# Nexenta/edge-fuse

Measured on NVIDIA H100. Metric: GiB/s hash+LZ4+dedup on 64 KiB chunks, higher is better.
Workload: dtype u8

## Files before the change

edge_fuse_b200/csrc/engine.cu:

```cuda
#include <algorithm>
#include <atomic>
#include <deque>
#include <mutex>
#include <set>
#include <shared_mutex>
#include <sched.h>
#include <string>
#include <new>
#include <unordered_set>
#include <stdio.h>
#include <stdlib.h>
#include <string.h>
#include <vector>
#include "../../include/cachemap_b200.h"
#include "../../include/uint128.h"
#include "kernels.h"
#include "common.cuh"
#include "streamgen.cuh"

static thread_local char g_err[512];

void cmb_set_error(const char *what, cudaError_t e, const char *file, int line) {
	snprintf(g_err, sizeof(g_err), "%s:%d: %s: %s", file, line, what, cudaGetErrorString(e));
}
static void set_error_msg(const char *msg) { snprintf(g_err, sizeof(g_err), "%s", msg); }

using namespace cmb;

struct cmb200_engine {
	int device = 0;
	int pshift = 16;
	uint32_t bsize = 65536;
	int accel = 12;
	uint64_t capacity = 0;
	uint32_t max_batch = 4096;
	uint32_t host_batch = 4096;
	uint32_t flags = 0;
	cudaStream_t st = nullptr, copy = nullptr;
	static constexpr int GET_LANES = 32;
	struct GetLane { std::atomic<int> busy{0}; cudaStream_t st = nullptr; int32_t *h_status = nullptr; cmb200_addr *h_addr = nullptr; };
	GetLane lane[GET_LANES];
	struct GetGate {
		std::atomic<int> active{0}, closed{0};
		void enter() {
			for (;;) {
				while (closed.load(std::memory_order_acquire)) sched_yield();
				active.fetch_add(1, std::memory_order_acq_rel);
				if (!closed.load(std::memory_order_acquire)) return;
				active.fetch_sub(1, std::memory_order_acq_rel);
			}
		}
		void leave() { active.fetch_sub(1, std::memory_order_acq_rel); }
		void close() {
			int open = 0;
			while (!closed.compare_exchange_weak(open, 1, std::memory_order_acq_rel)) { open = 0; sched_yield(); }
			while (active.load(std::memory_order_acquire)) sched_yield();
		}
		void reopen() { closed.store(0, std::memory_order_release); }
	} get_gate;
	struct GateClosed {
		GetGate &g;
		explicit GateClosed(GetGate &gate) : g(gate) { g.close(); }
		~GateClosed() { g.reopen(); }
	};
	std::atomic<uint32_t> lane_turn{0};
	static constexpr size_t GET_SMALL_MAX = 1024;
	const uint8_t *peer_base[GET_MAX_PEERS] = {};
	uint64_t peer_size[GET_MAX_PEERS] = {};
	std::atomic<uint64_t> small_get_requests{0}, small_get_hits{0}, small_get_launches{0};
	unsigned long long *d_recoff_out = nullptr;
	uint4 *d_scratch = nullptr;
	uint32_t *d_pool_bits = nullptr;
	uint32_t pool_n = 0, region_entries = 0;
	cudaEvent_t landed[2] = {nullptr, nullptr}, consumed[2] = {nullptr, nullptr};
	TableView table{};
	ArenaView arena{};
	unsigned long long *d_counters = nullptr;
	uint8_t *d_pages[2] = {nullptr, nullptr};
	uint8_t *d_stage = nullptr;
	uint64_t stage_stride = 0;
	unsigned long long *d_addr = nullptr, *d_ts = nullptr;
	uint8_t *d_valid = nullptr;
	uint32_t *d_slot = nullptr, *d_vlen = nullptr;
	int32_t *d_lens = nullptr, *d_status = nullptr;
	uint64_t *d_fps = nullptr, *d_recoff = nullptr;
	unsigned int *d_work = nullptr;
	uint32_t *d_order = nullptr;
	uint32_t *d_import_slot = nullptr;
	size_t import_slot_cap = 0;
	uint32_t *d_move_idx = nullptr;
	size_t move_idx_cap = 0;
	static constexpr size_t META_CAP = 1u << 18;
	uint8_t *h_meta = nullptr;
	unsigned long long seq = 1;
	unsigned long long seq_stride = 1;
	static constexpr int RING = 64;
	cudaEvent_t t0[RING] = {}, t1[RING] = {};
	cudaEvent_t p0[RING] = {}, p1[RING] = {};
	uint64_t pend_head = 0, pend_tail = 0;
	static constexpr int TICKETS = 8;
	cudaEvent_t ticket_ev[TICKETS] = {};
	uint64_t tickets = 0;
	cudaEvent_t meta_done = nullptr, meta_free[2] = {nullptr, nullptr};
	uint64_t ring_pos = 0;
	uint64_t meta_pos = 0;
	size_t meta_cap = 0;
	std::mutex mu;
	cmb200_stats stats{};
	struct HostTier {
		uint8_t *host = nullptr;
		uint8_t *dev = nullptr;
		uint64_t size = 0;
		uint64_t head = 0;
		std::deque<std::pair<uint64_t, uint32_t>> log;
		uint64_t demoted_records = 0, demoted_bytes = 0;
		uint64_t promoted_records = 0, promoted_bytes = 0;
		unsigned long long *d_ctr = nullptr;
		ulonglong2 *d_hot = nullptr;
		uint64_t hot_drained = 0;
		unsigned long long *d_retire = nullptr;
		size_t retire_cap = 0;
		DemoteEntry *d_moves = nullptr;
		PromoteEntry *d_promote = nullptr;
		HotLog hot() const { return HotLog{d_ctr ? d_ctr + 2 : nullptr, d_hot}; }
	} tier;
	std::atomic<bool> multi_gpu{false};
};

#define ENG_CHECK(expr)                                                 \
	do {                                                            \
		cudaError_t e_ = (expr);                                \
		if (e_ != cudaSuccess) {                                \
			cmb_set_error(#expr, e_, __FILE__, __LINE__);   \
			goto fail;                                      \
		}                                                       \
	} while (0)

static uint64_t next_pow2(uint64_t v) {
	uint64_t p = 1;
	while (p < v) p <<= 1;
	return p;
}

extern "C" const char *cmb200_last_error(void) { return g_err; }

extern "C" int cmb200_device_count(void) {
	int n = 0;
	cudaError_t e = cudaGetDeviceCount(&n);
	if (e != cudaSuccess) { cmb_set_error("cudaGetDeviceCount", e, __FILE__, __LINE__); return 0; }
	return n;
}

static int select_device(int device) {
	if (device >= 0) CMB_CHECK(cudaSetDevice(device));
	int n = 0;
	CMB_CHECK(cudaGetDeviceCount(&n));
	if (n == 0) { set_error_msg("no CUDA device"); return -1; }
	return 0;
}

extern "C" void cmb200_engine_destroy(cmb200_engine *e) {
	if (!e) return;
	cudaSetDevice(e->device);
	if (e->st) cudaStreamSynchronize(e->st);
	if (e->copy) cudaStreamSynchronize(e->copy);
	cudaFree(e->d_scratch); cudaFree(e->d_pool_bits); cudaFree(e->table.ckpt);
	cudaFree(e->table.slots); cudaFree(e->table.fp); cudaFree(e->arena.base); cudaFree(e->arena.seg); cudaFree(e->d_counters);
	cudaFree(e->d_pages[0]); cudaFree(e->d_pages[1]); cudaFree(e->d_stage);
	cudaFree(e->d_addr); cudaFree(e->d_ts); cudaFree(e->d_valid); cudaFree(e->d_slot); cudaFree(e->d_vlen);
	cudaFree(e->d_move_idx);
	if (e->h_meta) cudaFreeHost(e->h_meta);
	for (auto &ln : e->lane) {
		if (ln.st) { cudaStreamSynchronize(ln.st); cudaStreamDestroy(ln.st); }
		if (ln.h_status) cudaFreeHost(ln.h_status);
		if (ln.h_addr) cudaFreeHost(ln.h_addr);
	}
	cudaFree(e->d_recoff_out);
	for (int r = 0; r < GET_MAX_PEERS; r++) if (e->peer_base[r]) cudaIpcCloseMemHandle((void *)e->peer_base[r]);
	if (e->tier.host) cudaFreeHost(e->tier.host);
	cudaFree(e->tier.d_ctr); cudaFree(e->tier.d_retire); cudaFree(e->tier.d_moves);
	cudaFree(e->tier.d_promote); cudaFree(e->tier.d_hot);
	cudaFree(e->d_lens); cudaFree(e->d_status); cudaFree(e->d_fps); cudaFree(e->d_recoff); cudaFree(e->d_work); cudaFree(e->d_order); cudaFree(e->d_import_slot);
	for (int i = 0; i < 2; i++) {
		if (e->landed[i]) cudaEventDestroy(e->landed[i]);
		if (e->consumed[i]) cudaEventDestroy(e->consumed[i]);
	}
	for (int i = 0; i < cmb200_engine::RING; i++) {
		if (e->t0[i]) cudaEventDestroy(e->t0[i]);
		if (e->t1[i]) cudaEventDestroy(e->t1[i]);
		if (e->p0[i]) cudaEventDestroy(e->p0[i]);
		if (e->p1[i]) cudaEventDestroy(e->p1[i]);
	}
	for (int i = 0; i < cmb200_engine::TICKETS; i++) if (e->ticket_ev[i]) cudaEventDestroy(e->ticket_ev[i]);
	if (e->meta_done) cudaEventDestroy(e->meta_done);
	for (int i = 0; i < 2; i++) if (e->meta_free[i]) cudaEventDestroy(e->meta_free[i]);
	if (e->st) cudaStreamDestroy(e->st);
	if (e->copy) cudaStreamDestroy(e->copy);
	delete e;
}

extern "C" cmb200_engine *cmb200_engine_create(const cmb200_config *cfg) {
	if (!cfg || cfg->pshift < 6 || cfg->pshift > 20) { set_error_msg("bad config: pshift must be 6..20"); return nullptr; }
	if (select_device(cfg->device) != 0) return nullptr;
	cmb200_engine *e = new (std::nothrow) cmb200_engine();
	if (!e) return nullptr;
	cudaGetDevice(&e->device);
	e->pshift = cfg->pshift;
	e->bsize = 1u << cfg->pshift;
	e->accel = cfg->accel < 0 ? 1 : (cfg->accel > (1 << 20) ? (1 << 20) : cfg->accel);
	e->capacity = cfg->capacity;
	e->max_batch = cfg->max_batch ? cfg->max_batch : 4096;
	e->host_batch = e->max_batch < 4096u ? e->max_batch : 4096u;
	e->flags = cfg->flags;
	const uint64_t B = e->max_batch;
	{
		uint64_t slots = cfg->table_slots ? next_pow2(cfg->table_slots) : next_pow2(4 * (cfg->capacity ? cfg->capacity : 1024));
		if (slots < 1024) slots = 1024;
		if (slots > (1ull << 27)) slots = 1ull << 27;
		e->table.cap = slots;
		ENG_CHECK(cudaStreamCreateWithFlags(&e->st, cudaStreamNonBlocking));
		ENG_CHECK(cudaStreamCreateWithFlags(&e->copy, cudaStreamNonBlocking));
		for (auto &ln : e->lane) ENG_CHECK(cudaStreamCreateWithFlags(&ln.st, cudaStreamNonBlocking));
		for (int i = 0; i < 2; i++) {
			ENG_CHECK(cudaEventCreateWithFlags(&e->landed[i], cudaEventDisableTiming));
			ENG_CHECK(cudaEventCreateWithFlags(&e->consumed[i], cudaEventDisableTiming));
		}
		for (int i = 0; i < cmb200_engine::RING; i++) {
			ENG_CHECK(cudaEventCreate(&e->t0[i]));
			ENG_CHECK(cudaEventCreate(&e->t1[i]));
			ENG_CHECK(cudaEventCreate(&e->p0[i]));
			ENG_CHECK(cudaEventCreate(&e->p1[i]));
		}
		for (int i = 0; i < cmb200_engine::TICKETS; i++)
			ENG_CHECK(cudaEventCreateWithFlags(&e->ticket_ev[i], cudaEventDisableTiming));
		ENG_CHECK(cudaEventCreateWithFlags(&e->meta_done, cudaEventDisableTiming));
		ENG_CHECK(cudaEventCreateWithFlags(&e->meta_free[0], cudaEventDisableTiming));
		ENG_CHECK(cudaEventCreateWithFlags(&e->meta_free[1], cudaEventDisableTiming));
		ENG_CHECK(cudaMalloc(&e->table.slots, (slots + 2) * sizeof(Slot)));
		ENG_CHECK(cudaMemsetAsync(e->table.slots, 0, (slots + 2) * sizeof(Slot), e->st));
		if (e->flags & CMB200_FINGERPRINT) {
			ENG_CHECK(cudaMalloc(&e->table.fp, (slots + 2) * 16));
			ENG_CHECK(cudaMemsetAsync(e->table.fp, 0, (slots + 2) * 16, e->st));
		}
		if (get_small_supports(e->bsize)) {
			const char *ck = getenv("CMB200_CKPT");
			if (!ck || atoi(ck) != 0) {
				ENG_CHECK(cudaMalloc(&e->table.ckpt, (slots + 2) * CKPT_WORDS * 4));
				ENG_CHECK(cudaMemsetAsync(e->table.ckpt, 0, (slots + 2) * CKPT_WORDS * 4, e->st));
			}
			const int resident = get_small_residency(e->bsize);
			if (resident <= 0) { set_error_msg("k_get_small does not fit this device"); goto fail; }
			e->pool_n = (uint32_t)resident;
			e->region_entries = get_small_region_entries(e->bsize);
			ENG_CHECK(cudaMalloc(&e->d_scratch, (size_t)e->pool_n * e->region_entries * sizeof(uint4)));
			ENG_CHECK(cudaMalloc(&e->d_pool_bits, ((size_t)e->pool_n + 31) / 32 * 4));
			ENG_CHECK(cudaMemsetAsync(e->d_pool_bits, 0, ((size_t)e->pool_n + 31) / 32 * 4, e->st));
		}
		ENG_CHECK(cudaMalloc(&e->d_counters, 8 * sizeof(unsigned long long)));
		ENG_CHECK(cudaMemsetAsync(e->d_counters, 0, 8 * sizeof(unsigned long long), e->st));
		e->table.entries = e->d_counters + 0;
		e->table.tombs = e->d_counters + 1;
		e->arena.head = e->d_counters + 2;
		e->arena.garbage = e->d_counters + 3;
		e->arena.dropped = e->d_counters + 4;
		e->table.remote = e->d_counters + 5;
		e->arena.tier = e->d_counters + 6;

		{
			const uint64_t bound = (uint64_t)e->bsize + e->bsize / 255 + 16;
			const uint64_t row = (uint64_t)e->bsize + 1024 > bound ? (uint64_t)e->bsize + 1024 : bound;
			e->stage_stride = (row + 15) & ~15ull;
		}
		ENG_CHECK(cudaMalloc(&e->d_pages[0], (uint64_t)e->host_batch * e->bsize + 256));
		ENG_CHECK(cudaMalloc(&e->d_pages[1], (uint64_t)e->host_batch * e->bsize + 256));
		ENG_CHECK(cudaMalloc(&e->d_stage, (uint64_t)16384 * e->stage_stride + 256));
		const uint64_t M = cmb200_engine::META_CAP > B ? cmb200_engine::META_CAP : B;
		e->meta_cap = M;
		ENG_CHECK(cudaMalloc(&e->d_addr, 2 * M * 16));
		ENG_CHECK(cudaMalloc(&e->d_ts, 2 * M * 8));
		ENG_CHECK(cudaMalloc(&e->d_valid, 2 * M));
		ENG_CHECK(cudaMalloc(&e->d_slot, B * 4));
		ENG_CHECK(cudaMalloc(&e->d_vlen, B * 4));
		ENG_CHECK(cudaMalloc(&e->d_lens, M * 4));
		ENG_CHECK(cudaMalloc(&e->d_status, M * 4));
		ENG_CHECK(cudaMalloc(&e->d_fps, B * 16));
		ENG_CHECK(cudaMalloc(&e->d_recoff, B * 8));
		ENG_CHECK(cudaMalloc(&e->d_work, 64));
		ENG_CHECK(cudaMalloc(&e->d_order, encode_order_words((uint32_t)B) * 4));
		ENG_CHECK(cudaMallocHost(&e->h_meta, cmb200_engine::META_CAP * 33));
		for (auto &ln : e->lane) {
			ENG_CHECK(cudaMallocHost(&ln.h_status, cmb200_engine::GET_SMALL_MAX * 4));
			ENG_CHECK(cudaMallocHost(&ln.h_addr, cmb200_engine::GET_SMALL_MAX * 16));
		}
		ENG_CHECK(cudaMalloc(&e->d_recoff_out, M * 8));

		uint64_t arena = cfg->arena_bytes;
		if (!arena) {
			size_t free_b = 0, total_b = 0;
			ENG_CHECK(cudaMemGetInfo(&free_b, &total_b));
			uint64_t want = (cfg->capacity ? cfg->capacity : 1024) * (e->stage_stride + 32);
			want += want / 8;
			uint64_t lim = (uint64_t)(free_b * 0.8);
			arena = want < lim ? want : lim;
		}
		arena = (arena + 255) & ~255ull;
		ENG_CHECK(cudaMalloc(&e->arena.base, arena + 256));
		e->arena.size = arena;
		{
			const uint64_t worst = (24 + e->stage_stride + 15) & ~15ull;
			uint64_t seg = arena / (8ull * 2072ull);
			if (seg > (2ull << 20)) seg = 2ull << 20;
			if (seg < 4 * worst) seg = 0;
			const char *kb = getenv("CMB200_SEG_KB");
			if (kb && *kb) { seg = strtoull(kb, nullptr, 10) << 10; if (seg && seg < worst) seg = worst; }
			seg = (seg + 255) & ~255ull;
			e->arena.seg_bytes = (uint32_t)seg;
			ENG_CHECK(cudaMalloc(&e->arena.seg, ARENA_SEG_SLOTS * 2 * sizeof(unsigned long long)));
			ENG_CHECK(cudaMemsetAsync(e->arena.seg, 0, ARENA_SEG_SLOTS * 2 * sizeof(unsigned long long), e->st));
		}
		ENG_CHECK(cudaStreamSynchronize(e->st));
	}
	return e;
fail:
	cmb200_engine_destroy(e);
	return nullptr;
}

extern "C" void *cmb200_host_alloc(size_t bytes) {
	void *p = nullptr;
	cudaError_t er = cudaMallocHost(&p, bytes);
	if (er != cudaSuccess) { cmb_set_error("cudaMallocHost", er, __FILE__, __LINE__); return nullptr; }
	return p;
}
extern "C" void cmb200_host_free(void *p) { if (p) cudaFreeHost(p); }
extern "C" void *cmb200_dev_alloc(cmb200_engine *e, size_t bytes) {
	void *p = nullptr;
	if (e) cudaSetDevice(e->device);
	cudaError_t er = cudaMalloc(&p, bytes + 256);
	if (er != cudaSuccess) { cmb_set_error("cudaMalloc", er, __FILE__, __LINE__); return nullptr; }
	return p;
}
extern "C" void cmb200_dev_free(cmb200_engine *e, void *p) { if (e) cudaSetDevice(e->device); if (p) cudaFree(p); }
extern "C" int cmb200_memcpy_h2d(cmb200_engine *e, void *dev, const void *host, size_t bytes) {
	cudaSetDevice(e->device);
	CMB_CHECK(cudaMemcpyAsync(dev, host, bytes, cudaMemcpyHostToDevice, e->st));
	CMB_CHECK(cudaStreamSynchronize(e->st));
	return 0;
}
extern "C" int cmb200_memcpy_d2h(cmb200_engine *e, void *host, const void *dev, size_t bytes) {
	cudaSetDevice(e->device);
	CMB_CHECK(cudaMemcpyAsync(host, dev, bytes, cudaMemcpyDeviceToHost, e->st));
	CMB_CHECK(cudaStreamSynchronize(e->st));
	return 0;
}
extern "C" void *cmb200_stream(cmb200_engine *e) { return (void *)e->st; }
extern "C" int cmb200_sync(cmb200_engine *e) {
	cudaSetDevice(e->device);
	CMB_CHECK(cudaStreamSynchronize(e->copy));
	CMB_CHECK(cudaStreamSynchronize(e->st));
	return 0;
}


static void harvest_pending(cmb200_engine *e, bool wait) {
	while (e->pend_tail < e->pend_head) {
		const int k = (int)(e->pend_tail % cmb200_engine::RING);
		if (wait) cudaEventSynchronize(e->p1[k]);
		else if (cudaEventQuery(e->p1[k]) != cudaSuccess) { (void)cudaGetLastError(); break; }
		float ms = 0;
		if (cudaEventElapsedTime(&ms, e->p0[k], e->p1[k]) == cudaSuccess) {
			e->stats.encode_kernel_ns += (uint64_t)(ms * 1e6);
			e->stats.encode_kernel_launches++;
		}
		e->pend_tail++;
	}
}

struct StepRecords { uint32_t rank; unsigned long long *out; bool keep_pages; };

static int put_slice(cmb200_engine *e, size_t n, const cmb200_addr *addr, const uint8_t *valid,
    const uint8_t *pages, bool pages_on_dev, const uint64_t *ts, int32_t *lens_out, uint64_t *ticket,
    const StepRecords *recs = nullptr) {
	const size_t B = pages_on_dev ? e->max_batch : e->host_batch;
	const bool deferred = ticket != nullptr;
	const bool copy_meta = !pages_on_dev || deferred;
	const unsigned long long seq_first = e->seq;
	cmb200_addr *h_addr = (cmb200_addr *)e->h_meta;
	uint64_t *h_ts = (uint64_t *)(e->h_meta + cmb200_engine::META_CAP * 16);
	int32_t *h_lens = (int32_t *)(e->h_meta + cmb200_engine::META_CAP * 24);
	uint8_t *h_valid = e->h_meta + cmb200_engine::META_CAP * 32;
	harvest_pending(e, !deferred);
	memcpy(h_addr, addr, n * 16);
	if (ts) memcpy(h_ts, ts, n * 8);
	if (valid) memcpy(h_valid, valid, n);
	const int mb = copy_meta ? (int)(e->meta_pos++ & 1) : 0;
	unsigned long long *d_addr = e->d_addr + (size_t)mb * e->meta_cap * 2;
	unsigned long long *d_ts = e->d_ts + (size_t)mb * e->meta_cap;
	uint8_t *d_valid = e->d_valid + (size_t)mb * e->meta_cap;
	cudaStream_t ms = copy_meta ? e->copy : e->st;
	if (copy_meta) CMB_CHECK(cudaStreamWaitEvent(e->copy, e->meta_free[mb], 0));
	CMB_CHECK(cudaMemcpyAsync(d_addr, h_addr, n * 16, cudaMemcpyHostToDevice, ms));
	if (valid) CMB_CHECK(cudaMemcpyAsync(d_valid, h_valid, n, cudaMemcpyHostToDevice, ms));
	if (ts) CMB_CHECK(cudaMemcpyAsync(d_ts, h_ts, n * 8, cudaMemcpyHostToDevice, ms));
	if (copy_meta) {
		CMB_CHECK(cudaEventRecord(e->meta_done, e->copy));
		CMB_CHECK(cudaStreamWaitEvent(e->st, e->meta_done, 0));
	}
	size_t nb = 0;
	int last_buf = 0;
	for (size_t at = 0; at < n; at += B, nb++) {
		const uint32_t m = (uint32_t)((n - at < B) ? n - at : B);
		const int buf = (int)(e->ring_pos & 1);
		const uint8_t *d_in;
		if (pages_on_dev) {
			d_in = pages + at * e->bsize;
		} else {
			e->ring_pos++;
			last_buf = buf;
			CMB_CHECK(cudaStreamWaitEvent(e->copy, e->consumed[buf], 0));
			CMB_CHECK(cudaMemcpyAsync(e->d_pages[buf], pages + at * e->bsize, (size_t)m * e->bsize,
			    cudaMemcpyHostToDevice, e->copy));
			CMB_CHECK(cudaEventRecord(e->landed[buf], e->copy));
			CMB_CHECK(cudaStreamWaitEvent(e->st, e->landed[buf], 0));
			d_in = e->d_pages[buf];
		}
		if (launch_upsert(e->table, d_addr + 2 * at, valid ? d_valid + at : nullptr, m, e->seq, e->seq_stride, e->d_slot, e->st)) return -1;
		EncodeJob job{};
		job.pages = d_in; job.page_stride = e->bsize; job.nbytes = e->bsize; job.n = m;
		job.accel = (uint32_t)e->accel;
		job.stage = e->d_stage; job.stage_stride = e->stage_stride;
		job.lens = e->d_lens + at;
		job.rec_out = e->d_recoff_out + at;
		job.fps = (e->flags & CMB200_FINGERPRINT) ? e->d_fps : nullptr;
		job.work = e->d_work;
		job.order = e->d_order;
		job.slot_idx = e->d_slot;
		job.addr = d_addr + 2 * at;
		job.ts = ts ? d_ts + at : nullptr;
		job.seq0 = e->seq; job.seq_stride = e->seq_stride;
		job.table = e->table; job.arena = e->arena;
		cudaEvent_t ev0, ev1;
		if (deferred) {
			if (e->pend_head - e->pend_tail >= (uint64_t)cmb200_engine::RING) harvest_pending(e, true);
			ev0 = e->p0[e->pend_head % cmb200_engine::RING]; ev1 = e->p1[e->pend_head % cmb200_engine::RING];
			e->pend_head++;
		} else {
			ev0 = e->t0[nb % e->RING]; ev1 = e->t1[nb % e->RING];
		}
		CMB_CHECK(cudaEventRecord(ev0, e->st));
		const int encode_kernels = launch_encode(job, e->st);
		if (encode_kernels < 0) return -1;
		CMB_CHECK(cudaEventRecord(ev1, e->st));
		if (!pages_on_dev) CMB_CHECK(cudaEventRecord(e->consumed[buf], e->st));
		e->seq += (unsigned long long)m * e->seq_stride;
		e->stats.kernel_launches += 1 + encode_kernels;
	}
	e->stats.put_chunks += n;
	if (recs && recs->out) {
		if (launch_pack_records(d_addr, e->d_lens, e->d_recoff_out, (uint32_t)n, seq_first, e->seq_stride, recs->rank, recs->out, e->st)) return -1;
		e->stats.kernel_launches++;
	}
	if (copy_meta) CMB_CHECK(cudaEventRecord(e->meta_free[mb], e->st));
	if (deferred) {
		if (lens_out) CMB_CHECK(cudaMemcpyAsync(lens_out, e->d_lens, n * 4, cudaMemcpyDeviceToHost, e->st));
		CMB_CHECK(cudaEventRecord(e->ticket_ev[e->tickets % cmb200_engine::TICKETS], e->st));
		*ticket = ++e->tickets;
		CMB_CHECK(cudaEventSynchronize(e->meta_done));
		if (nb && !pages_on_dev && !(recs && recs->keep_pages)) CMB_CHECK(cudaEventSynchronize(e->landed[last_buf]));
		harvest_pending(e, false);
		return 0;
	}
	if (lens_out) CMB_CHECK(cudaMemcpyAsync(h_lens, e->d_lens, n * 4, cudaMemcpyDeviceToHost, e->st));
	CMB_CHECK(cudaStreamSynchronize(e->st));
	if (lens_out) memcpy(lens_out, h_lens, n * 4);
	for (size_t k = 0; k < nb && k < (size_t)e->RING; k++) {
		float ms = 0;
		CMB_CHECK(cudaEventElapsedTime(&ms, e->t0[k], e->t1[k]));
		e->stats.encode_kernel_ns += (uint64_t)(ms * 1e6);
		e->stats.encode_kernel_launches++;
	}
	return 0;
}

static int check_dev_pages(const void *pages, const char *what) {
	if (reinterpret_cast<uintptr_t>(pages) & 15u) {
		snprintf(g_err, sizeof(g_err), "%s: device pages must be 16-byte aligned", what);
		return -1;
	}
	return 0;
}

static int multi_gpu_call(cmb200_engine *e, const char *what) {
	if (e->tier.host) {
		snprintf(g_err, sizeof(g_err), "%s: not available on an engine with a host tier", what);
		return -1;
	}
	e->multi_gpu = true;
	return 0;
}

static int put_impl(cmb200_engine *e, size_t n, const cmb200_addr *addr, const uint8_t *valid,
    const uint8_t *pages, bool pages_on_dev, const uint64_t *ts, int32_t *lens_out, uint64_t *ticket) {
	std::lock_guard<std::mutex> g(e->mu);
	CMB_CHECK(cudaSetDevice(e->device));
	if (ticket) *ticket = e->tickets;
	for (size_t at = 0; at < n; at += cmb200_engine::META_CAP) {
		size_t m = n - at < cmb200_engine::META_CAP ? n - at : cmb200_engine::META_CAP;
		const bool last = at + m == n;
		if (put_slice(e, m, addr + at, valid ? valid + at : nullptr, pages + at * e->bsize, pages_on_dev,
			ts ? ts + at : nullptr, lens_out ? lens_out + at : nullptr, last ? ticket : nullptr)) return -1;
	}
	return 0;
}

extern "C" int cmb200_put_batch(cmb200_engine *e, size_t n, const cmb200_addr *addr, const uint8_t *valid,
    const void *pages_host, const uint64_t *ts, int32_t *lens_out) {
	return put_impl(e, n, addr, valid, (const uint8_t *)pages_host, false, ts, lens_out, nullptr);
}
extern "C" int cmb200_put_batch_async(cmb200_engine *e, size_t n, const cmb200_addr *addr, const uint8_t *valid,
    const void *pages_host, const uint64_t *ts, int32_t *lens_out, uint64_t *ticket) {
	uint64_t t = 0;
	const int rc = put_impl(e, n, addr, valid, (const uint8_t *)pages_host, false, ts, lens_out, &t);
	if (ticket) *ticket = t;
	return rc;
}
extern "C" int cmb200_put_step(cmb200_engine *e, size_t n, const cmb200_addr *addr, const uint8_t *valid,
    const void *pages, int pages_on_dev, const uint64_t *ts, uint32_t rank, void *records_dev_out,
    int32_t *lens_out, uint64_t *ticket) {
	if (multi_gpu_call(e, "cmb200_put_step")) return -1;
	if (n > cmb200_engine::META_CAP) { set_error_msg("cmb200_put_step: more than 262144 chunks in one step"); return -1; }
	if (pages_on_dev == 1 && check_dev_pages(pages, "cmb200_put_step")) return -1;
	std::lock_guard<std::mutex> g(e->mu);
	CMB_CHECK(cudaSetDevice(e->device));
	uint64_t t = e->tickets;
	StepRecords r{rank, (unsigned long long *)records_dev_out, pages_on_dev == 2};
	const int rc = n ? put_slice(e, n, addr, valid, (const uint8_t *)pages, pages_on_dev == 1, ts, lens_out, &t, &r) : 0;
	if (ticket) *ticket = t;
	return rc;
}

extern "C" int cmb200_import_records_dev(cmb200_engine *e, size_t n_total, const void *records_dev, uint32_t my_rank) {
	std::lock_guard<std::mutex> g(e->mu);
	if (multi_gpu_call(e, "cmb200_import_records_dev")) return -1;
	CMB_CHECK(cudaSetDevice(e->device));
	if (n_total == 0) return 0;
	if (n_total > 0xffffffffull) { set_error_msg("cmb200_import_records_dev: too many records"); return -1; }
	if (n_total > e->import_slot_cap) {
		CMB_CHECK(cudaStreamSynchronize(e->st));
		if (e->d_import_slot) cudaFree(e->d_import_slot);
		e->d_import_slot = nullptr; e->import_slot_cap = 0;
		CMB_CHECK(cudaMalloc(&e->d_import_slot, n_total * sizeof(uint32_t)));
		e->import_slot_cap = n_total;
	}
	if (launch_import_records(e->table, e->arena, (const unsigned long long *)records_dev, (uint32_t)n_total, my_rank,
		e->d_import_slot, e->st)) return -1;
	e->stats.kernel_launches += 2;
	return 0;
}

extern "C" int cmb200_wait(cmb200_engine *e, uint64_t ticket) {
	cudaEvent_t ev = nullptr;
	{
		std::lock_guard<std::mutex> g(e->mu);
		if (ticket == 0 || ticket > e->tickets) return 0;
		ev = e->ticket_ev[(ticket - 1) % cmb200_engine::TICKETS];
		if (cudaSetDevice(e->device) != cudaSuccess) return -1;
	}
	CMB_CHECK(cudaEventSynchronize(ev));
	return 0;
}
extern "C" int cmb200_put_batch_dev(cmb200_engine *e, size_t n, const cmb200_addr *addr, const uint8_t *valid,
    const void *pages_dev, const uint64_t *ts, int32_t *lens_out) {
	if (check_dev_pages(pages_dev, "cmb200_put_batch_dev")) return -1;
	return put_impl(e, n, addr, valid, (const uint8_t *)pages_dev, true, ts, lens_out, nullptr);
}


static int get_slice(cmb200_engine *e, size_t n, const cmb200_addr *addr, const uint8_t *valid,
    uint8_t *pages_out, bool out_on_dev, int32_t *status_out) {
	const size_t B = out_on_dev ? e->max_batch : e->host_batch;
	cmb200_addr *h_addr = (cmb200_addr *)e->h_meta;
	int32_t *h_status = (int32_t *)(e->h_meta + cmb200_engine::META_CAP * 28);
	uint8_t *h_valid = e->h_meta + cmb200_engine::META_CAP * 32;
	memcpy(h_addr, addr, n * 16);
	if (valid) memcpy(h_valid, valid, n);
	CMB_CHECK(cudaMemcpyAsync(e->d_addr, h_addr, n * 16, cudaMemcpyHostToDevice, e->st));
	if (valid) CMB_CHECK(cudaMemcpyAsync(e->d_valid, h_valid, n, cudaMemcpyHostToDevice, e->st));
	size_t nb = 0;
	for (size_t at = 0; at < n; at += B, nb++) {
		const uint32_t m = (uint32_t)((n - at < B) ? n - at : B);
		const int buf = (int)(nb & 1);
		uint8_t *d_out = out_on_dev ? pages_out + at * e->bsize : e->d_pages[buf];
		if (!out_on_dev) CMB_CHECK(cudaStreamWaitEvent(e->st, e->consumed[buf], 0));
		if (launch_lookup(e->table, e->d_addr + 2 * at, valid ? e->d_valid + at : nullptr, m, e->d_status + at, e->d_recoff,
			e->d_vlen, nullptr, e->st)) return -1;
		DecodeJob job{};
		job.n = m; job.nbytes = e->bsize; job.pages = d_out; job.status = e->d_status + at;
		job.rec_off = e->d_recoff; job.vlen = e->d_vlen; job.arena = e->arena.base;
		job.host = e->tier.dev; job.host_hits = e->tier.d_ctr + 1;
		job.hot = e->tier.hot(); job.addr = e->d_addr + 2 * at;
		CMB_CHECK(cudaEventRecord(e->t0[nb % e->RING], e->st));
		if (launch_decode(job, e->st)) return -1;
		CMB_CHECK(cudaEventRecord(e->t1[nb % e->RING], e->st));
		if (!out_on_dev) {
			CMB_CHECK(cudaEventRecord(e->landed[buf], e->st));
			CMB_CHECK(cudaStreamWaitEvent(e->copy, e->landed[buf], 0));
			CMB_CHECK(cudaMemcpyAsync(pages_out + at * e->bsize, d_out, (size_t)m * e->bsize,
			    cudaMemcpyDeviceToHost, e->copy));
			CMB_CHECK(cudaEventRecord(e->consumed[buf], e->copy));
		}
		e->stats.kernel_launches += 2;
	}
	CMB_CHECK(cudaMemcpyAsync(h_status, e->d_status, n * 4, cudaMemcpyDeviceToHost, e->st));
	CMB_CHECK(cudaStreamSynchronize(e->st));
	CMB_CHECK(cudaStreamSynchronize(e->copy));
	memcpy(status_out, h_status, n * 4);
	for (size_t k = 0; k < nb && k < (size_t)e->RING; k++) {
		float ms = 0;
		CMB_CHECK(cudaEventElapsedTime(&ms, e->t0[k], e->t1[k]));
		e->stats.decode_kernel_ns += (uint64_t)(ms * 1e6);
		e->stats.decode_kernel_launches++;
	}
	for (size_t i = 0; i < n; i++) {
		if (status_out[i] != CMB200_INVALID) e->stats.get_requests++;
		if (status_out[i] == CMB200_HIT) e->stats.get_hits++;
	}
	return 0;
}

static int get_impl(cmb200_engine *e, size_t n, const cmb200_addr *addr, const uint8_t *valid,
    uint8_t *pages_out, bool out_on_dev, int32_t *status_out) {
	std::lock_guard<std::mutex> g(e->mu);
	CMB_CHECK(cudaSetDevice(e->device));
	for (size_t at = 0; at < n; at += cmb200_engine::META_CAP) {
		size_t m = n - at < cmb200_engine::META_CAP ? n - at : cmb200_engine::META_CAP;
		if (get_slice(e, m, addr + at, valid ? valid + at : nullptr, pages_out + at * e->bsize, out_on_dev,
			status_out + at)) return -1;
	}
	return 0;
}

extern "C" int cmb200_get_batch(cmb200_engine *e, size_t n, const cmb200_addr *addr, const uint8_t *valid,
    void *pages_out_host, int32_t *status_out) {
	return get_impl(e, n, addr, valid, (uint8_t *)pages_out_host, false, status_out);
}
static int lookup_chunk(cmb200_engine *e, const cmb200_addr *addr, uint32_t m, int32_t *status, uint64_t *loc,
    uint32_t *vlen) {
	CMB_CHECK(cudaMemcpyAsync(e->d_addr, addr, (size_t)m * 16, cudaMemcpyHostToDevice, e->st));
	if (launch_lookup(e->table, e->d_addr, nullptr, m, e->d_status, e->d_recoff, e->d_vlen, nullptr, e->st)) return -1;
	CMB_CHECK(cudaMemcpyAsync(status, e->d_status, (size_t)m * 4, cudaMemcpyDeviceToHost, e->st));
	CMB_CHECK(cudaMemcpyAsync(loc, e->d_recoff, (size_t)m * 8, cudaMemcpyDeviceToHost, e->st));
	if (vlen) CMB_CHECK(cudaMemcpyAsync(vlen, e->d_vlen, (size_t)m * 4, cudaMemcpyDeviceToHost, e->st));
	CMB_CHECK(cudaStreamSynchronize(e->st));
	return 0;
}

extern "C" int cmb200_locate_batch(cmb200_engine *e, size_t n, const cmb200_addr *addr, int32_t *status_out,
    uint64_t *owner_out) {
	std::lock_guard<std::mutex> g(e->mu);
	CMB_CHECK(cudaSetDevice(e->device));
	for (size_t at = 0; at < n; at += e->max_batch) {
		uint32_t m = (uint32_t)((n - at < e->max_batch) ? n - at : e->max_batch);
		if (lookup_chunk(e, addr + at, m, status_out + at, owner_out + at, nullptr)) return -1;
		e->stats.kernel_launches++;
	}
	return 0;
}
extern "C" int cmb200_get_batch_dev(cmb200_engine *e, size_t n, const cmb200_addr *addr, const uint8_t *valid,
    void *pages_out_dev, int32_t *status_out) {
	return get_impl(e, n, addr, valid, (uint8_t *)pages_out_dev, true, status_out);
}


extern "C" int cmb200_set_stream_order(cmb200_engine *e, uint64_t next_seq, uint64_t stride) {
	std::lock_guard<std::mutex> g(e->mu);
	if (multi_gpu_call(e, "cmb200_set_stream_order")) return -1;
	if (stride == 0) { set_error_msg("stream order: stride must be >= 1"); return -1; }
	e->seq = next_seq; e->seq_stride = stride;
	return 0;
}


static const int32_t SMALL_PENDING = -1;

extern "C" int cmb200_get_small_begin(cmb200_engine *e, size_t n, const cmb200_addr *addr, void *pages_out, cmb200_small_ticket *t) {
	if (!t) return -1;
	t->lane = -1; t->n = 0; t->status = nullptr;
	if (n == 0) return 0;
	if (n > cmb200_engine::GET_SMALL_MAX) { set_error_msg("cmb200_get_small_begin: more than 1024 requests"); return -1; }
	if (!get_small_supports(e->bsize)) { set_error_msg("cmb200_get_small: page size not supported by the fused kernel"); return -2; }
	e->get_gate.enter();
	cmb200_engine::GetLane *ln = nullptr;
	int li = -1;
	const uint32_t first = e->lane_turn.fetch_add(1, std::memory_order_relaxed);
	for (uint64_t spins = 0; !ln; spins++) {
		for (int k = 0; k < cmb200_engine::GET_LANES && !ln; k++) {
			const int c = (int)((first + k) % cmb200_engine::GET_LANES);
			int idle = 0;
			if (e->lane[c].busy.compare_exchange_strong(idle, 1, std::memory_order_acq_rel)) { ln = &e->lane[c]; li = c; }
		}
		if (!ln) sched_yield();
	}
	if (cudaSetDevice(e->device) != cudaSuccess) { ln->busy.store(0, std::memory_order_release); e->get_gate.leave(); return -1; }
	memcpy(ln->h_addr, addr, n * 16);
	volatile int32_t *hs = ln->h_status;
	for (size_t i = 0; i < n; i++) hs[i] = SMALL_PENDING;
	GetJob job{};
	job.table = e->table; job.arena = e->arena.base; job.arena_size = e->arena.size;
	job.host = e->tier.dev; job.host_size = e->tier.size; job.host_hits = e->tier.d_ctr + 1;
	job.addr = (const unsigned long long *)ln->h_addr; job.valid = nullptr; job.n = (uint32_t)n; job.nbytes = e->bsize;
	job.out = (uint8_t *)pages_out;
	job.status = ln->h_status;
	for (int r = 0; r < GET_MAX_PEERS; r++) { job.peer[r] = e->peer_base[r]; job.peer_size[r] = e->peer_size[r]; }
	job.scratch = e->d_scratch; job.region_entries = e->region_entries; job.pool_bits = e->d_pool_bits; job.pool_n = e->pool_n;
	job.hot = e->tier.hot();
	if (launch_get_small(job, e->device, ln->st)) { ln->busy.store(0, std::memory_order_release); e->get_gate.leave(); return -1; }
	t->lane = li; t->n = (uint32_t)n; t->status = ln->h_status;
	return 0;
}

extern "C" int cmb200_get_small_end(cmb200_engine *e, cmb200_small_ticket *t, int32_t *status_out) {
	if (!t || t->lane < 0) return 0;
	cmb200_engine::GetLane *ln = &e->lane[t->lane];
	volatile int32_t *hs = ln->h_status;
	int rc = 0;
	uint32_t done = 0;
	for (uint64_t spins = 0; done < t->n;) {
		if (hs[done] != SMALL_PENDING) { done++; continue; }
#if defined(__x86_64__)
		__builtin_ia32_pause();
#endif
		if (++spins > 20000) {
			if (cudaSetDevice(e->device) != cudaSuccess || cudaStreamSynchronize(ln->st) != cudaSuccess) {
				cmb_set_error("cudaStreamSynchronize(small get)", cudaGetLastError(), __FILE__, __LINE__);
				rc = -1; break;
			}
			spins = 0;
			if (hs[done] == SMALL_PENDING) { set_error_msg("cmb200_get_small: kernel finished without an answer"); rc = -1; break; }
		}
	}
	__atomic_thread_fence(__ATOMIC_ACQUIRE);
	if (rc == 0) {
		uint64_t rq = 0, ht = 0;
		for (uint32_t i = 0; i < t->n; i++) {
			const int32_t st = hs[i];
			if (status_out) status_out[i] = st;
			if (st != CMB200_INVALID) rq++;
			if (st == CMB200_HIT) ht++;
		}
		e->small_get_launches++;
		e->small_get_requests += rq; e->small_get_hits += ht;
	}
	t->lane = -1;
	ln->busy.store(0, std::memory_order_release);
	e->get_gate.leave();
	return rc;
}

extern "C" int cmb200_get_small(cmb200_engine *e, size_t n, const cmb200_addr *addr, void *pages_out, int32_t *status_out) {
	for (size_t at = 0; at < n; at += cmb200_engine::GET_SMALL_MAX) {
		const size_t m = n - at < cmb200_engine::GET_SMALL_MAX ? n - at : cmb200_engine::GET_SMALL_MAX;
		cmb200_small_ticket t;
		const int rc = cmb200_get_small_begin(e, m, addr + at, (uint8_t *)pages_out + at * e->bsize, &t);
		if (rc) return rc;
		if (cmb200_get_small_end(e, &t, status_out + at)) return -1;
	}
	return 0;
}


extern "C" int cmb200_close_peers(cmb200_engine *e) {
	cmb200_engine::GateClosed g(e->get_gate);
	CMB_CHECK(cudaSetDevice(e->device));
	for (int r = 0; r < GET_MAX_PEERS; r++) {
		if (e->peer_base[r]) cudaIpcCloseMemHandle((void *)e->peer_base[r]);
		e->peer_base[r] = nullptr; e->peer_size[r] = 0;
	}
	return 0;
}

extern "C" int cmb200_arena_ipc_handle(cmb200_engine *e, void *handle64, uint64_t *arena_bytes_out) {
	{
		std::lock_guard<std::mutex> g(e->mu);
		if (multi_gpu_call(e, "cmb200_arena_ipc_handle")) return -1;
	}
	CMB_CHECK(cudaSetDevice(e->device));
	cudaIpcMemHandle_t h;
	static_assert(sizeof(h) == 64, "cudaIpcMemHandle_t is 64 bytes");
	CMB_CHECK(cudaIpcGetMemHandle(&h, e->arena.base));
	memcpy(handle64, &h, 64);
	if (arena_bytes_out) *arena_bytes_out = e->arena.size;
	return 0;
}

extern "C" int cmb200_open_peer(cmb200_engine *e, uint32_t rank, const void *handle64, uint64_t arena_bytes) {
	{
		std::lock_guard<std::mutex> g(e->mu);
		if (multi_gpu_call(e, "cmb200_open_peer")) return -1;
	}
	if (rank >= GET_MAX_PEERS) { set_error_msg("cmb200_open_peer: rank out of range"); return -1; }
	cmb200_engine::GateClosed g(e->get_gate);
	CMB_CHECK(cudaSetDevice(e->device));
	cudaIpcMemHandle_t h;
	memcpy(&h, handle64, 64);
	void *p = nullptr;
	CMB_CHECK(cudaIpcOpenMemHandle(&p, h, cudaIpcMemLazyEnablePeerAccess));
	if (e->peer_base[rank]) cudaIpcCloseMemHandle((void *)e->peer_base[rank]);
	e->peer_base[rank] = (const uint8_t *)p;
	e->peer_size[rank] = arena_bytes;
	return 0;
}


extern "C" int cmb200_unset_batch(cmb200_engine *e, size_t n, const cmb200_addr *addr) {
	std::lock_guard<std::mutex> g(e->mu);
	CMB_CHECK(cudaSetDevice(e->device));
	for (size_t at = 0; at < n; at += e->max_batch) {
		uint32_t m = (uint32_t)((n - at < e->max_batch) ? n - at : e->max_batch);
		CMB_CHECK(cudaMemcpyAsync(e->d_addr, addr + at, (size_t)m * 16, cudaMemcpyHostToDevice, e->st));
		if (launch_unset(e->table, e->arena, e->d_addr, m, e->st)) return -1;
		e->stats.kernel_launches++;
	}
	CMB_CHECK(cudaStreamSynchronize(e->st));
	return 0;
}

static int read_counters(cmb200_engine *e, unsigned long long out[8]) {
	CMB_CHECK(cudaSetDevice(e->device));
	CMB_CHECK(cudaMemcpyAsync(out, e->d_counters, 8 * sizeof(unsigned long long), cudaMemcpyDeviceToHost, e->st));
	CMB_CHECK(cudaStreamSynchronize(e->st));
	return 0;
}

extern "C" uint64_t cmb200_entries(cmb200_engine *e) {
	std::lock_guard<std::mutex> g(e->mu);
	unsigned long long c[8];
	if (read_counters(e, c)) return 0;
	return c[0];
}

extern "C" int cmb200_get_stats(cmb200_engine *e, cmb200_stats *out) {
	std::lock_guard<std::mutex> g(e->mu);
	unsigned long long c[8];
	if (read_counters(e, c)) return -1;
	harvest_pending(e, true);
	*out = e->stats;
	out->get_requests += e->small_get_requests.load(); out->get_hits += e->small_get_hits.load();
	out->kernel_launches += e->small_get_launches.load();
	out->entries = c[0]; out->tombstones = c[1];
	out->arena_used = c[2] < e->arena.size ? c[2] : e->arena.size;
	out->arena_garbage = c[3];
	out->dropped_puts = c[4]; out->remote_entries = c[5];
	out->table_slots = e->table.cap; out->arena_bytes = e->arena.size;
	return 0;
}

extern "C" int cmb200_sample(cmb200_engine *e, size_t n, const uint64_t *r, cmb200_addr *addr_out,
    uint64_t *ts_out, int32_t *ok_out) {
	std::lock_guard<std::mutex> g(e->mu);
	CMB_CHECK(cudaSetDevice(e->device));
	for (size_t at = 0; at < n; at += e->max_batch) {
		const uint32_t m = (uint32_t)((n - at < e->max_batch) ? n - at : e->max_batch);
		CMB_CHECK(cudaMemcpyAsync(e->d_recoff, r + at, (size_t)m * 8, cudaMemcpyHostToDevice, e->st));
		if (launch_sample(e->table, (const unsigned long long *)e->d_recoff, m, e->d_addr, e->d_ts, e->d_status, e->st)) return -1;
		CMB_CHECK(cudaMemcpyAsync(addr_out + at, e->d_addr, (size_t)m * 16, cudaMemcpyDeviceToHost, e->st));
		CMB_CHECK(cudaMemcpyAsync(ts_out + at, e->d_ts, (size_t)m * 8, cudaMemcpyDeviceToHost, e->st));
		CMB_CHECK(cudaMemcpyAsync(ok_out + at, e->d_status, (size_t)m * 4, cudaMemcpyDeviceToHost, e->st));
		CMB_CHECK(cudaStreamSynchronize(e->st));
		e->stats.kernel_launches++;
	}
	return 0;
}

extern "C" int cmb200_read_records(cmb200_engine *e, size_t n, const cmb200_addr *addr, void *out_host,
    size_t stride, int32_t *len_out) {
	std::lock_guard<std::mutex> g(e->mu);
	CMB_CHECK(cudaSetDevice(e->device));
	std::vector<int32_t> st(e->max_batch);
	std::vector<uint64_t> off(e->max_batch);
	std::vector<uint32_t> vl(e->max_batch);
	for (size_t at = 0; at < n; at += e->max_batch) {
		uint32_t m = (uint32_t)((n - at < e->max_batch) ? n - at : e->max_batch);
		if (lookup_chunk(e, addr + at, m, st.data(), off.data(), vl.data())) return -1;
		for (uint32_t i = 0; i < m; i++) {
			if (st[i] != ST_HIT) { len_out[at + i] = -1; continue; }
			uint32_t clen = vl[i] - 1;
			size_t total = 24 + (clen ? clen : e->bsize);
			if (total > stride) { set_error_msg("cmb200_read_records: stride too small"); return -1; }
			if (off[i] & REC_HOST) memcpy((uint8_t *)out_host + (at + i) * stride, e->tier.host + (off[i] & ~REC_HOST), total);
			else CMB_CHECK(cudaMemcpyAsync((uint8_t *)out_host + (at + i) * stride, e->arena.base + off[i], total,
			    cudaMemcpyDeviceToHost, e->st));
			len_out[at + i] = (int32_t)total;
		}
		CMB_CHECK(cudaStreamSynchronize(e->st));
	}
	return 0;
}

extern "C" int cmb200_read_fingerprints(cmb200_engine *e, size_t n, const cmb200_addr *addr, uint64_t *fp_out,
    int32_t *ok_out) {
	std::lock_guard<std::mutex> g(e->mu);
	CMB_CHECK(cudaSetDevice(e->device));
	if (!e->table.fp) { set_error_msg("engine created without CMB200_FINGERPRINT"); return -1; }
	for (size_t at = 0; at < n; at += e->max_batch) {
		uint32_t m = (uint32_t)((n - at < e->max_batch) ? n - at : e->max_batch);
		CMB_CHECK(cudaMemcpyAsync(e->d_addr, addr + at, (size_t)m * 16, cudaMemcpyHostToDevice, e->st));
		if (launch_read_fp(e->table, e->d_addr, m, e->d_fps, e->d_status, e->st)) return -1;
		CMB_CHECK(cudaMemcpyAsync(fp_out + 2 * at, e->d_fps, (size_t)m * 16, cudaMemcpyDeviceToHost, e->st));
		CMB_CHECK(cudaMemcpyAsync(ok_out + at, e->d_status, (size_t)m * 4, cudaMemcpyDeviceToHost, e->st));
		CMB_CHECK(cudaStreamSynchronize(e->st));
	}
	return 0;
}

struct DevBuf {
	void *p = nullptr;
	~DevBuf() { if (p) cudaFree(p); }
	int alloc(size_t bytes) { CMB_CHECK(cudaMalloc(&p, bytes + 256)); return 0; }
	template <class T> T *as() { return (T *)p; }
};

extern "C" int cmb200_read_checkpoints(cmb200_engine *e, size_t n, const cmb200_addr *addr, uint32_t *words_out,
    int32_t *ok_out) {
	std::lock_guard<std::mutex> g(e->mu);
	CMB_CHECK(cudaSetDevice(e->device));
	if (!e->table.ckpt) {
		memset(words_out, 0, n * CKPT_WORDS * 4);
		for (size_t i = 0; i < n; i++) ok_out[i] = -1;
		return 0;
	}
	DevBuf d_words;
	if (n && d_words.alloc((size_t)e->max_batch * CKPT_WORDS * 4)) return -1;
	for (size_t at = 0; at < n; at += e->max_batch) {
		uint32_t m = (uint32_t)((n - at < e->max_batch) ? n - at : e->max_batch);
		CMB_CHECK(cudaMemcpyAsync(e->d_addr, addr + at, (size_t)m * 16, cudaMemcpyHostToDevice, e->st));
		if (launch_read_ckpt(e->table, e->d_addr, m, d_words.as<uint32_t>(), e->d_status, e->st)) return -1;
		CMB_CHECK(cudaMemcpyAsync(words_out + at * CKPT_WORDS, d_words.p, (size_t)m * CKPT_WORDS * 4, cudaMemcpyDeviceToHost, e->st));
		CMB_CHECK(cudaMemcpyAsync(ok_out + at, e->d_status, (size_t)m * 4, cudaMemcpyDeviceToHost, e->st));
		CMB_CHECK(cudaStreamSynchronize(e->st));
	}
	return 0;
}

static int live_records(cmb200_engine *e, bool arena_only, std::vector<ExportEntry> &list, unsigned long long c[8]) {
	if (read_counters(e, c)) return -1;
	const unsigned long long cap_out = c[0] + 16;
	DevBuf d_list, d_count;
	if (d_list.alloc(cap_out * sizeof(ExportEntry)) || d_count.alloc(8)) return -1;
	CMB_CHECK(cudaMemsetAsync(d_count.p, 0, 8, e->st));
	if (launch_export_list(e->table, e->bsize, d_list.as<ExportEntry>(), d_count.as<unsigned long long>(), cap_out,
		arena_only, e->st)) return -1;
	unsigned long long count = 0;
	CMB_CHECK(cudaMemcpyAsync(&count, d_count.p, 8, cudaMemcpyDeviceToHost, e->st));
	CMB_CHECK(cudaStreamSynchronize(e->st));
	const int over = count > cap_out;
	if (over) count = cap_out;
	list.resize(count);
	if (count) CMB_CHECK(cudaMemcpy(list.data(), d_list.p, count * sizeof(ExportEntry), cudaMemcpyDeviceToHost));
	std::sort(list.begin(), list.end(), [](const ExportEntry &a, const ExportEntry &b) { return a.rec_off < b.rec_off; });
	return over;
}

struct SnapHeader {
	char magic[8];
	uint32_t version, pshift;
	uint64_t records, bytes;
	uint32_t flags, pad[7];
};
static_assert(sizeof(SnapHeader) == 64, "snapshot header");
struct SnapRecord { uint64_t ts, fp_hi, fp_lo; uint32_t len, zero; };
static_assert(sizeof(SnapRecord) == 32, "snapshot record header");
static const size_t SNAP_WINDOW = 64u << 20;

static int save_engine(cmb200_engine *e, FILE *f, uint8_t *win, uint64_t *records, uint64_t *bytes) {
	unsigned long long c[8];
	std::vector<ExportEntry> list;
	if (live_records(e, false, list, c) < 0) return -1;
	*records += list.size();
	for (const ExportEntry &x : list) *bytes += x.len;

	bool ok = true;
	static const uint8_t zeros[16] = {0};
	size_t k = 0;
	while (ok && k < list.size()) {
		if (list[k].rec_off & REC_HOST) {
			const ExportEntry &x = list[k++];
			SnapRecord r{x.ts, x.fp_hi, x.fp_lo, x.len, 0};
			const size_t padn = (16 - (x.len & 15)) & 15;
			ok = fwrite(&r, sizeof(r), 1, f) == 1 && fwrite(e->tier.host + (x.rec_off & ~REC_HOST), x.len, 1, f) == 1 &&
			    (padn == 0 || fwrite(zeros, padn, 1, f) == 1);
			continue;
		}
		const unsigned long long w0 = list[k].rec_off;
		unsigned long long w1 = w0 + SNAP_WINDOW;
		if (w1 > e->arena.size + 256) w1 = e->arena.size + 256;
		if (cudaMemcpyAsync(win, e->arena.base + w0, (size_t)(w1 - w0), cudaMemcpyDeviceToHost, e->st) != cudaSuccess ||
		    cudaStreamSynchronize(e->st) != cudaSuccess) { ok = false; break; }
		for (; k < list.size() && list[k].rec_off + list[k].len <= w1; k++) {
			const ExportEntry &x = list[k];
			SnapRecord r{x.ts, x.fp_hi, x.fp_lo, x.len, 0};
			const size_t padn = (16 - (x.len & 15)) & 15;
			ok = ok && fwrite(&r, sizeof(r), 1, f) == 1 && fwrite(win + (x.rec_off - w0), x.len, 1, f) == 1 &&
			    (padn == 0 || fwrite(zeros, padn, 1, f) == 1);
		}
	}
	return ok ? 0 : -2;
}

extern "C" int cmb200_save_set(cmb200_engine *const *engines, int g, const char *path, uint64_t *records_out) {
	if (g < 1 || !engines) { set_error_msg("cmb200_save_set: no engines"); return -1; }
	for (int i = 1; i < g; i++)
		if (engines[i]->pshift != engines[0]->pshift) { set_error_msg("cmb200_save_set: engines of different page sizes"); return -1; }
	std::string tmp = std::string(path) + ".tmp";
	FILE *f = fopen(tmp.c_str(), "wb");
	if (!f) { set_error_msg("cmb200_save: cannot create the snapshot file"); return -1; }
	uint8_t *win = nullptr;
	if (cudaMallocHost(&win, SNAP_WINDOW) != cudaSuccess) { fclose(f); remove(tmp.c_str()); set_error_msg("cmb200_save: no page-locked window"); return -1; }
	SnapHeader h{};
	memcpy(h.magic, "CMB200S1", 8);
	h.version = 1; h.pshift = (uint32_t)engines[0]->pshift; h.flags = engines[0]->table.fp ? 1u : 0u;
	bool ok = fwrite(&h, sizeof(h), 1, f) == 1;
	int rc = 0;
	for (int i = 0; i < g && ok && rc == 0; i++) {
		std::lock_guard<std::mutex> lk(engines[i]->mu);
		rc = save_engine(engines[i], f, win, &h.records, &h.bytes);
	}
	cudaFreeHost(win);
	ok = ok && rc != -2 && fseek(f, 0, SEEK_SET) == 0 && fwrite(&h, sizeof(h), 1, f) == 1;
	ok = ok && fflush(f) == 0;
	ok = (fclose(f) == 0) && ok;
	if (rc == -1 || !ok || rename(tmp.c_str(), path) != 0) {
		remove(tmp.c_str());
		if (rc != -1) set_error_msg("cmb200_save: write failed");
		return -1;
	}
	if (records_out) *records_out = h.records;
	return 0;
}

extern "C" int cmb200_save(cmb200_engine *e, const char *path, uint64_t *records_out) {
	return cmb200_save_set(&e, 1, path, records_out);
}

static int demote_arena_all(cmb200_engine *e);

struct LoadBatch {
	cmb200_engine *e = nullptr;
	uint8_t *blob = nullptr;
	size_t cap = 0, B = 0, used = 0, m = 0;
	std::vector<unsigned long long> off, ts, fps;
	std::vector<cmb200_addr> addr;
	unsigned long long *d_off = nullptr;
	uint64_t *d_fp = nullptr;
	int setup(cmb200_engine *eng) {
		e = eng;
		CMB_CHECK(cudaSetDevice(e->device));
		cap = (size_t)e->host_batch * e->bsize;
		B = e->max_batch < cmb200_engine::META_CAP ? e->max_batch : cmb200_engine::META_CAP;
		off.resize(B); ts.resize(B); fps.resize(2 * B); addr.resize(B);
		CMB_CHECK(cudaMallocHost(&blob, cap));
		CMB_CHECK(cudaMalloc(&d_off, B * 8));
		CMB_CHECK(cudaMalloc(&d_fp, B * 16));
		return 0;
	}
	void release() {
		if (!e) return;
		cudaSetDevice(e->device);
		if (blob) cudaFreeHost(blob);
		if (d_off) cudaFree(d_off);
		if (d_fp) cudaFree(d_fp);
	}
};

static long long load_flush(LoadBatch &b, bool with_fp) {
	if (b.m == 0) return 0;
	cmb200_engine *e = b.e;
	std::lock_guard<std::mutex> g(e->mu);
	CMB_CHECK(cudaSetDevice(e->device));
	const size_t m = b.m;
	if (e->tier.host) {
		unsigned long long c[8];
		if (read_counters(e, c)) return -1;
		if (c[2] + b.used > e->arena.size && demote_arena_all(e)) return -1;
	}
	CMB_CHECK(cudaMemcpyAsync(e->d_pages[0], b.blob, b.used, cudaMemcpyHostToDevice, e->st));
	CMB_CHECK(cudaMemcpyAsync(e->d_addr, b.addr.data(), m * 16, cudaMemcpyHostToDevice, e->st));
	CMB_CHECK(cudaMemcpyAsync(e->d_ts, b.ts.data(), m * 8, cudaMemcpyHostToDevice, e->st));
	CMB_CHECK(cudaMemcpyAsync(b.d_off, b.off.data(), m * 8, cudaMemcpyHostToDevice, e->st));
	CMB_CHECK(cudaMemcpyAsync(b.d_fp, b.fps.data(), m * 16, cudaMemcpyHostToDevice, e->st));
	if (launch_upsert(e->table, e->d_addr, nullptr, (uint32_t)m, e->seq, e->seq_stride, e->d_slot, e->st)) return -1;
	EncodeJob job{};
	job.n = (uint32_t)m; job.nbytes = e->bsize;
	job.slot_idx = e->d_slot; job.addr = e->d_addr; job.ts = e->d_ts;
	job.seq0 = e->seq; job.seq_stride = e->seq_stride;
	job.table = e->table; job.arena = e->arena;
	if (launch_restore(job, e->d_pages[0], b.d_off, with_fp ? b.d_fp : nullptr, e->bsize, e->st)) return -1;
	CMB_CHECK(cudaStreamSynchronize(e->st));
	e->seq += (unsigned long long)m * e->seq_stride;
	e->stats.kernel_launches += 2;
	b.m = 0; b.used = 0;
	return (long long)m;
}

extern "C" int cmb200_load_set(cmb200_engine *const *engines, int g, const char *path, uint64_t *records_out) {
	if (records_out) *records_out = 0;
	if (g < 1 || !engines) { set_error_msg("cmb200_load_set: no engines"); return -1; }
	FILE *f = fopen(path, "rb");
	if (!f) { set_error_msg("cmb200_load: no snapshot file"); return -1; }
	SnapHeader h{};
	if (fread(&h, sizeof(h), 1, f) != 1 || memcmp(h.magic, "CMB200S1", 8) != 0 || h.version != 1) {
		fclose(f); set_error_msg("cmb200_load: not a snapshot of this library"); return -1;
	}
	for (int i = 0; i < g; i++)
		if ((int)h.pshift != engines[i]->pshift) { fclose(f); set_error_msg("cmb200_load: snapshot has another page size"); return -1; }
	const uint32_t bsize = engines[0]->bsize;
	std::vector<LoadBatch> bs(g);
	int rc = 0;
	for (int i = 0; i < g && rc == 0; i++)
		if (bs[i].setup(engines[i])) { rc = -1; set_error_msg("cmb200_load: no staging buffers"); }
	uint64_t done = 0, loaded = 0;
	while (rc == 0 && done < h.records) {
		SnapRecord r;
		cmb200_addr a;
		if (fread(&r, sizeof(r), 1, f) != 1 || r.len < 24 || r.len > 24u + bsize + 1024u || fread(&a, 16, 1, f) != 1) {
			rc = -1; set_error_msg("cmb200_load: truncated or corrupt snapshot"); break;
		}
		uint64_t key;
		FNV_hash(&a, 16, &key);
		LoadBatch &b = bs[cmb200_owner(key, g)];
		const size_t padded = ((size_t)r.len + 15) & ~(size_t)15;
		if (padded > b.cap) { rc = -1; set_error_msg("cmb200_load: record larger than the staging buffer"); break; }
		if (b.m == b.B || b.used + padded > b.cap) {
			const long long got = load_flush(b, h.flags & 1u);
			if (got < 0) { rc = -1; break; }
			loaded += (uint64_t)got;
		}
		uint8_t *rec = b.blob + b.used;
		memcpy(rec, &a, 16);
		if (fread(rec + 16, padded - 16, 1, f) != 1) { rc = -1; set_error_msg("cmb200_load: truncated or corrupt snapshot"); break; }
		{
			int32_t clen;
			memcpy(&clen, rec + 16, 4);
			if (clen < 0 || (uint32_t)clen > bsize + 1024u || r.len != 24u + (clen ? (uint32_t)clen : bsize)) {
				rc = -1; set_error_msg("cmb200_load: truncated or corrupt snapshot"); break;
			}
		}
		b.addr[b.m] = a;
		b.off[b.m] = b.used; b.ts[b.m] = r.ts; b.fps[2 * b.m] = r.fp_hi; b.fps[2 * b.m + 1] = r.fp_lo;
		b.used += padded; b.m++;
		done++;
	}
	for (int i = 0; i < g && rc == 0; i++) {
		const long long got = load_flush(bs[i], h.flags & 1u);
		if (got < 0) rc = -1;
		else loaded += (uint64_t)got;
	}
	for (LoadBatch &b : bs) b.release();
	fclose(f);
	if (records_out) *records_out = loaded;
	return rc;
}

extern "C" int cmb200_load(cmb200_engine *e, const char *path, uint64_t *records_out) {
	return cmb200_load_set(&e, 1, path, records_out);
}


extern "C" int cmb200_move_pages(cmb200_engine *e, size_t n, void *dst_dev, const uint32_t *dst_idx, const void *src_dev,
    const uint32_t *src_idx) {
	if (n == 0) return 0;
	if (check_dev_pages(dst_dev, "cmb200_move_pages") || check_dev_pages(src_dev, "cmb200_move_pages")) return -1;
	if (n > 0xffffffffu) { set_error_msg("cmb200_move_pages: too many pages"); return -1; }
	std::lock_guard<std::mutex> g(e->mu);
	CMB_CHECK(cudaSetDevice(e->device));
	if ((dst_idx || src_idx) && n > e->move_idx_cap) {
		CMB_CHECK(cudaStreamSynchronize(e->st));
		cudaFree(e->d_move_idx);
		e->d_move_idx = nullptr;
		e->move_idx_cap = 0;
		CMB_CHECK(cudaMalloc(&e->d_move_idx, n * 8));
		e->move_idx_cap = n;
	}
	uint32_t *d_dst_idx = dst_idx ? e->d_move_idx : nullptr;
	uint32_t *d_src_idx = src_idx ? e->d_move_idx + e->move_idx_cap : nullptr;
	if (dst_idx) CMB_CHECK(cudaMemcpyAsync(d_dst_idx, dst_idx, n * 4, cudaMemcpyHostToDevice, e->st));
	if (src_idx) CMB_CHECK(cudaMemcpyAsync(d_src_idx, src_idx, n * 4, cudaMemcpyHostToDevice, e->st));
	if (launch_move_pages(dst_dev, d_dst_idx, src_dev, d_src_idx, (uint32_t)n, e->bsize, e->st)) return -1;
	e->stats.kernel_launches++;
	CMB_CHECK(cudaStreamSynchronize(e->st));
	return 0;
}

extern "C" int cmb200_copy_peer(cmb200_engine *dst_e, void *dst_dev, cmb200_engine *src_e, const void *src_dev, size_t bytes) {
	if (bytes == 0) return 0;
	std::lock_guard<std::mutex> g(src_e->mu);
	CMB_CHECK(cudaSetDevice(src_e->device));
	CMB_CHECK(cudaMemcpyPeerAsync(dst_dev, dst_e->device, src_dev, src_e->device, bytes, src_e->st));
	CMB_CHECK(cudaStreamSynchronize(src_e->st));
	return 0;
}

static int compact_locked(cmb200_engine *e, uint64_t *reclaimed_out) {
	cmb200_engine::GateClosed gg(e->get_gate);
	harvest_pending(e, true);
	unsigned long long c[8];
	std::vector<ExportEntry> list;
	const int listed = live_records(e, true, list, c);
	if (listed < 0) return -1;
	if (listed > 0) { set_error_msg("cmb200_compact: the store changed under the compaction"); return -1; }
	const unsigned long long head_before = c[2];
	const size_t count = list.size();
	DevBuf d_moves;
	std::vector<MoveEntry> moves(count);
	unsigned long long at = 0;
	for (size_t i = 0; i < count; i++) {
		moves[i] = MoveEntry{list[i].rec_off, at, list[i].len, list[i].slot};
		at += ((unsigned long long)list[i].len + 15ull) & ~15ull;
	}
	if (count && d_moves.alloc(count * sizeof(MoveEntry))) return -1;
	if (count) CMB_CHECK(cudaMemcpyAsync(d_moves.p, moves.data(), count * sizeof(MoveEntry), cudaMemcpyHostToDevice, e->st));
	const unsigned long long bounce_cap = (unsigned long long)e->host_batch * e->bsize;
	size_t k = 0;
	while (k < count) {
		size_t j = k;
		while (j < count && moves[j].new_off + (((unsigned long long)moves[j].len + 15ull) & ~15ull) - moves[k].new_off <= bounce_cap) j++;
		if (j == k) { set_error_msg("cmb200_compact: record larger than the bounce buffer"); return -1; }
		if (launch_compact_window(e->table, e->arena, d_moves.as<MoveEntry>() + k, (uint32_t)(j - k), e->d_pages[0], e->st)) return -1;
		e->stats.kernel_launches += 2;
		k = j;
	}
	unsigned long long fresh[2] = {at, 0};
	CMB_CHECK(cudaMemcpyAsync(e->d_counters + 2, fresh, 16, cudaMemcpyHostToDevice, e->st));
	CMB_CHECK(cudaMemsetAsync(e->arena.seg, 0, ARENA_SEG_SLOTS * 2 * sizeof(unsigned long long), e->st));
	CMB_CHECK(cudaStreamSynchronize(e->st));
	if (reclaimed_out) *reclaimed_out = head_before > at ? head_before - at : 0;
	if (c[1] > e->table.cap / 8) {
		TableView fresh = e->table;
		fresh.slots = nullptr; fresh.fp = nullptr; fresh.ckpt = nullptr;
		if (cudaMalloc(&fresh.slots, (e->table.cap + 2) * sizeof(Slot)) == cudaSuccess &&
		    (!e->table.fp || cudaMalloc(&fresh.fp, (e->table.cap + 2) * 16) == cudaSuccess)) {
			CMB_CHECK(cudaMemsetAsync(fresh.slots, 0, (e->table.cap + 2) * sizeof(Slot), e->st));
			if (fresh.fp) CMB_CHECK(cudaMemsetAsync(fresh.fp, 0, (e->table.cap + 2) * 16, e->st));
			const size_t ck_bytes = (e->table.cap + 2) * CKPT_WORDS * 4;
			if (e->table.ckpt && cudaMalloc(&fresh.ckpt, ck_bytes) != cudaSuccess) {
				(void)cudaGetLastError();
				fresh.ckpt = nullptr;
			}
			if (fresh.ckpt) CMB_CHECK(cudaMemsetAsync(fresh.ckpt, 0, ck_bytes, e->st));
			if (launch_rehash(e->table, fresh, e->st)) return -1;
			if (e->table.ckpt && !fresh.ckpt) CMB_CHECK(cudaMemsetAsync(e->table.ckpt, 0, ck_bytes, e->st));
			CMB_CHECK(cudaMemsetAsync(e->d_counters + 1, 0, sizeof(unsigned long long), e->st));
			CMB_CHECK(cudaStreamSynchronize(e->st));
			cudaFree(e->table.slots); cudaFree(e->table.fp);
			e->table.slots = fresh.slots; e->table.fp = fresh.fp;
			if (fresh.ckpt) { cudaFree(e->table.ckpt); e->table.ckpt = fresh.ckpt; }
			e->stats.kernel_launches++;
		} else {
			(void)cudaGetLastError();
			cudaFree(fresh.slots);
		}
	}
	return 0;
}

extern "C" int cmb200_compact(cmb200_engine *e, uint64_t *reclaimed_out) {
	std::lock_guard<std::mutex> g(e->mu);
	return compact_locked(e, reclaimed_out);
}


extern "C" int cmb200_host_tier_enable(cmb200_engine *e, uint64_t bytes) {
	std::lock_guard<std::mutex> g(e->mu);
	if (e->tier.host) { set_error_msg("cmb200_host_tier_enable: the engine already has a host tier"); return -1; }
	if (e->multi_gpu) { set_error_msg("cmb200_host_tier_enable: not available after a multi-GPU call"); return -1; }
	if (e->seq != 1) { set_error_msg("cmb200_host_tier_enable: must be called before the first put"); return -1; }
	bytes = (bytes + 4095) & ~4095ull;
	if (bytes < 4ull * e->stage_stride) { set_error_msg("cmb200_host_tier_enable: fewer bytes than four worst-case records"); return -1; }
	CMB_CHECK(cudaSetDevice(e->device));
	cmb200_engine::HostTier &t = e->tier;
	if (cudaMalloc(&t.d_ctr, 3 * sizeof(unsigned long long)) != cudaSuccess ||
	    cudaMalloc(&t.d_moves, (size_t)e->max_batch * sizeof(DemoteEntry)) != cudaSuccess ||
	    cudaMalloc(&t.d_promote, (size_t)e->max_batch * sizeof(PromoteEntry)) != cudaSuccess ||
	    cudaMalloc(&t.d_hot, HOT_LOG_N * sizeof(ulonglong2)) != cudaSuccess ||
	    cudaMemset(t.d_ctr, 0, 3 * sizeof(unsigned long long)) != cudaSuccess ||
	    cudaMemset(t.d_hot, 0, HOT_LOG_N * sizeof(ulonglong2)) != cudaSuccess ||
	    cudaHostAlloc(&t.host, bytes, cudaHostAllocMapped) != cudaSuccess ||
	    cudaHostGetDevicePointer(&t.dev, t.host, 0) != cudaSuccess) {
		cmb_set_error("cmb200_host_tier_enable", cudaGetLastError(), __FILE__, __LINE__);
		if (t.host) cudaFreeHost(t.host);
		cudaFree(t.d_ctr); cudaFree(t.d_moves); cudaFree(t.d_promote); cudaFree(t.d_hot);
		t = cmb200_engine::HostTier{};
		return -1;
	}
	t.size = bytes;
	return 0;
}

static int demote_group(cmb200_engine *e, const std::vector<DemoteEntry> &grp,
    const std::vector<std::pair<uint64_t, uint32_t>> &placed, uint64_t start, uint64_t end) {
	cmb200_engine::HostTier &t = e->tier;
	uint8_t *bounce = e->d_pages[0];
	const uint32_t n = (uint32_t)grp.size();
	CMB_CHECK(cudaMemcpyAsync(t.d_moves, grp.data(), n * sizeof(DemoteEntry), cudaMemcpyHostToDevice, e->st));
	if (launch_demote_gather(e->arena, t.d_moves, n, bounce, e->st)) return -1;
	std::vector<unsigned long long> ret;
	while (!t.log.empty() && t.log.front().first + t.size < end) {
		const uint64_t p = t.log.front().first, at = p % t.size;
		const unsigned long long *pre = reinterpret_cast<const unsigned long long *>(t.host + at);
		ret.insert(ret.end(), {pre[0], pre[1], REC_HOST | at, t.log.front().second});
		t.log.pop_front();
	}
	const bool overwrite = end > t.size;
	if (overwrite) e->get_gate.close();
	int rc = 0;
	const size_t nr = ret.size() / 4;
	if (nr > t.retire_cap) {
		if (cudaStreamSynchronize(e->st) != cudaSuccess) rc = -1;
		cudaFree(t.d_retire);
		t.d_retire = nullptr; t.retire_cap = 0;
		if (rc == 0 && cudaMalloc(&t.d_retire, nr * 32) == cudaSuccess) t.retire_cap = nr;
		else rc = -1;
	}
	const uint64_t a0 = start % t.size, bytes = end - start, first = std::min(bytes, t.size - a0);
	if (rc == 0 && nr) {
		rc = cudaMemcpyAsync(t.d_retire, ret.data(), nr * 32, cudaMemcpyHostToDevice, e->st) != cudaSuccess ||
		    launch_tier_retire(e->table, e->arena, t.d_retire, (uint32_t)nr, t.d_ctr, e->st) ? -1 : 0;
		e->stats.kernel_launches++;
	}
	if (rc == 0 && (cudaMemcpyAsync(t.host + a0, bounce, first, cudaMemcpyDeviceToHost, e->st) != cudaSuccess ||
	    (bytes > first && cudaMemcpyAsync(t.host, bounce + first, bytes - first, cudaMemcpyDeviceToHost, e->st) != cudaSuccess)))
		rc = -1;
	if (rc == 0 && launch_demote_publish(e->table, e->arena, t.d_moves, n, e->st)) rc = -1;
	if (cudaStreamSynchronize(e->st) != cudaSuccess) rc = -1;
	if (overwrite) e->get_gate.reopen();
	if (rc) { cmb_set_error("host tier demotion", cudaGetLastError(), __FILE__, __LINE__); return -1; }
	t.log.insert(t.log.end(), placed.begin(), placed.end());
	t.head = end;
	t.demoted_records += n;
	for (const DemoteEntry &d : grp) t.demoted_bytes += d.len;
	e->stats.kernel_launches += 2;
	return 0;
}

static int demote_records(cmb200_engine *e, const std::vector<std::pair<unsigned long long, uint32_t>> &recs) {
	cmb200_engine::HostTier &t = e->tier;
	const uint64_t cap = std::min<uint64_t>(t.size, (uint64_t)e->host_batch * e->bsize);
	size_t k = 0;
	std::vector<DemoteEntry> grp;
	std::vector<std::pair<uint64_t, uint32_t>> placed;
	while (k < recs.size()) {
		grp.clear(); placed.clear();
		const uint64_t start = t.head;
		uint64_t pos = start;
		while (k < recs.size() && grp.size() < e->max_batch) {
			const uint32_t len = recs[k].second, need = (len + 15u) & ~15u;
			uint64_t p = pos;
			if (p % t.size + need > t.size) p += t.size - p % t.size;
			if (p + need - start > cap) break;
			grp.push_back(DemoteEntry{recs[k].first, p % t.size, p - start, len, 0});
			placed.emplace_back(p, need);
			pos = p + need;
			k++;
		}
		if (grp.empty()) { set_error_msg("cmb200_demote_batch: record larger than the bounce buffer"); return -1; }
		if (demote_group(e, grp, placed, start, pos)) return -1;
	}
	return 0;
}

extern "C" int cmb200_demote_batch(cmb200_engine *e, size_t n, const cmb200_addr *addr, uint64_t *demoted_out) {
	std::lock_guard<std::mutex> g(e->mu);
	if (demoted_out) *demoted_out = 0;
	if (!e->tier.host) { set_error_msg("cmb200_demote_batch: the engine has no host tier"); return -1; }
	CMB_CHECK(cudaSetDevice(e->device));
	harvest_pending(e, true);
	std::vector<int32_t> st(e->max_batch);
	std::vector<uint64_t> off(e->max_batch);
	std::vector<uint32_t> vl(e->max_batch);
	std::vector<std::pair<unsigned long long, uint32_t>> recs;
	uint64_t done = 0;
	for (size_t at = 0; at < n; at += e->max_batch) {
		const uint32_t m = (uint32_t)((n - at < e->max_batch) ? n - at : e->max_batch);
		if (lookup_chunk(e, addr + at, m, st.data(), off.data(), vl.data())) return -1;
		e->stats.kernel_launches++;
		recs.clear();
		std::unordered_set<uint64_t> seen;
		for (uint32_t i = 0; i < m; i++) {
			if (st[i] != ST_HIT || (off[i] & REC_HOST) || !seen.insert(off[i]).second) continue;
			const uint32_t clen = vl[i] - 1u;
			recs.emplace_back(off[i], 24u + (clen ? clen : e->bsize));
		}
		if (demote_records(e, recs)) return -1;
		done += recs.size();
	}
	if (demoted_out) *demoted_out = done;
	return 0;
}

static int demote_arena_all(cmb200_engine *e) {
	unsigned long long c[8];
	std::vector<ExportEntry> list;
	if (live_records(e, true, list, c) < 0) return -1;
	std::vector<std::pair<unsigned long long, uint32_t>> recs;
	for (const ExportEntry &x : list) recs.emplace_back(x.rec_off, x.len);
	if (demote_records(e, recs)) return -1;
	return compact_locked(e, nullptr);
}

extern "C" int cmb200_promote_batch(cmb200_engine *e, size_t n, const cmb200_addr *addr, uint64_t *promoted_out) {
	std::lock_guard<std::mutex> g(e->mu);
	if (promoted_out) *promoted_out = 0;
	cmb200_engine::HostTier &t = e->tier;
	if (!t.host) { set_error_msg("cmb200_promote_batch: the engine has no host tier"); return -1; }
	CMB_CHECK(cudaSetDevice(e->device));
	harvest_pending(e, true);
	unsigned long long c[8];
	if (read_counters(e, c)) return -1;
	unsigned long long head = c[2];
	std::vector<int32_t> st(e->max_batch);
	std::vector<uint64_t> off(e->max_batch);
	std::vector<uint32_t> vl(e->max_batch);
	std::vector<PromoteEntry> plan;
	uint64_t done = 0;
	bool full = false;
	for (size_t at = 0; at < n && !full; at += e->max_batch) {
		const uint32_t m = (uint32_t)((n - at < e->max_batch) ? n - at : e->max_batch);
		if (lookup_chunk(e, addr + at, m, st.data(), off.data(), vl.data())) return -1;
		e->stats.kernel_launches++;
		plan.clear();
		std::unordered_set<uint64_t> seen;
		for (uint32_t i = 0; i < m; i++) {
			if (st[i] != ST_HIT || !(off[i] & REC_HOST) || !seen.insert(off[i]).second) continue;
			const uint32_t clen = vl[i] - 1u, len = 24u + (clen ? clen : e->bsize), need = (len + 15u) & ~15u;
			if (head + need > e->arena.size) { full = true; break; }
			plan.push_back(PromoteEntry{off[i] & ~REC_HOST, head, len, 0});
			head += need;
		}
		if (plan.empty()) continue;
		CMB_CHECK(cudaMemcpyAsync(e->d_counters + 2, &head, 8, cudaMemcpyHostToDevice, e->st));
		CMB_CHECK(cudaMemcpyAsync(t.d_promote, plan.data(), plan.size() * sizeof(PromoteEntry), cudaMemcpyHostToDevice, e->st));
		if (launch_promote(e->table, e->arena, t.d_promote, (uint32_t)plan.size(), t.dev, e->st)) return -1;
		CMB_CHECK(cudaStreamSynchronize(e->st));
		e->stats.kernel_launches++;
		done += plan.size();
		t.promoted_records += plan.size();
		for (const PromoteEntry &p : plan) t.promoted_bytes += p.len;
	}
	if (promoted_out) *promoted_out = done;
	return 0;
}

extern "C" int cmb200_host_tier_hot(cmb200_engine *e, size_t max, cmb200_addr *addr_out, size_t *n_out, uint64_t *lost_out) {
	std::lock_guard<std::mutex> g(e->mu);
	*n_out = 0;
	if (lost_out) *lost_out = 0;
	cmb200_engine::HostTier &t = e->tier;
	if (!t.host) return 0;
	CMB_CHECK(cudaSetDevice(e->device));
	unsigned long long head = 0;
	std::vector<ulonglong2> ring(HOT_LOG_N);
	CMB_CHECK(cudaMemcpyAsync(&head, t.d_ctr + 2, 8, cudaMemcpyDeviceToHost, e->st));
	CMB_CHECK(cudaMemcpyAsync(ring.data(), t.d_hot, HOT_LOG_N * sizeof(ulonglong2), cudaMemcpyDeviceToHost, e->st));
	CMB_CHECK(cudaStreamSynchronize(e->st));
	const uint64_t since = head - t.hot_drained;
	const uint64_t from = since > HOT_LOG_N ? head - HOT_LOG_N : t.hot_drained;
	if (lost_out) *lost_out = since > HOT_LOG_N ? since - HOT_LOG_N : 0;
	t.hot_drained = head;
	std::set<std::pair<uint64_t, uint64_t>> seen;
	size_t k = 0;
	for (uint64_t p = head; p > from && k < max; p--) {
		const ulonglong2 a = ring[(p - 1) % HOT_LOG_N];
		if (!seen.insert({a.x, a.y}).second) continue;
		addr_out[k].u = a.x; addr_out[k].l = a.y;
		k++;
	}
	*n_out = k;
	return 0;
}

extern "C" int cmb200_host_tier_stats(cmb200_engine *e, struct cmb200_host_tier_stats *out) {
	std::lock_guard<std::mutex> g(e->mu);
	memset(out, 0, sizeof(*out));
	const cmb200_engine::HostTier &t = e->tier;
	if (!t.host) return 0;
	unsigned long long c[8], d[2];
	if (read_counters(e, c)) return -1;
	CMB_CHECK(cudaMemcpy(d, t.d_ctr, sizeof(d), cudaMemcpyDeviceToHost));
	out->bytes = t.size;
	out->used = t.log.empty() ? 0 : t.head - t.log.front().first;
	out->records = c[7]; out->garbage = c[6];
	out->demoted_records = t.demoted_records; out->demoted_bytes = t.demoted_bytes;
	out->retired_records = d[0]; out->hits = d[1];
	out->promoted_records = t.promoted_records; out->promoted_bytes = t.promoted_bytes;
	return 0;
}


extern "C" int cmb200_compose_keys(int device, size_t n, const uint64_t *offset, const uint64_t *nhid,
    const uint32_t *genid, int pshift, cmb200_addr *addr_out, uint8_t *valid_out, uint64_t *key_out) {
	if (select_device(device)) return -1;
	DevBuf d_off, d_nh, d_g, d_addr, d_valid, d_key;
	if (d_off.alloc(n * 8) || d_nh.alloc(n * 8) || d_g.alloc(n * 4) || d_addr.alloc(n * 16) || d_valid.alloc(n) || d_key.alloc(n * 8)) return -1;
	CMB_CHECK(cudaMemcpy(d_off.p, offset, n * 8, cudaMemcpyHostToDevice));
	CMB_CHECK(cudaMemcpy(d_nh.p, nhid, n * 8, cudaMemcpyHostToDevice));
	CMB_CHECK(cudaMemcpy(d_g.p, genid, n * 4, cudaMemcpyHostToDevice));
	if (launch_compose(d_off.as<uint64_t>(), d_nh.as<uint64_t>(), d_g.as<uint32_t>(), pshift, (uint32_t)n,
		d_addr.as<unsigned long long>(), d_valid.as<uint8_t>(), d_key.as<unsigned long long>(), 0)) return -1;
	CMB_CHECK(cudaMemcpy(addr_out, d_addr.p, n * 16, cudaMemcpyDeviceToHost));
	CMB_CHECK(cudaMemcpy(valid_out, d_valid.p, n, cudaMemcpyDeviceToHost));
	CMB_CHECK(cudaMemcpy(key_out, d_key.p, n * 8, cudaMemcpyDeviceToHost));
	return 0;
}

extern "C" int cmb200_lz4_encode_batch(int device, const void *pages_host, size_t n, uint32_t nbytes,
    size_t stride, int accel, void *blocks_out_host, size_t out_stride, int32_t *lens_out, uint64_t *fp_out) {
	if (select_device(device)) return -1;
	if (stride % 16 || stride < nbytes) { set_error_msg("encode_batch: stride must be a multiple of 16 and >= nbytes"); return -1; }
	size_t bound = (size_t)nbytes + nbytes / 255 + 16;
	size_t sstride = (bound + 15) & ~(size_t)15;
	if (out_stride < bound) { set_error_msg("encode_batch: out_stride below LZ4_compressBound"); return -1; }
	DevBuf d_in, d_stage, d_lens, d_fps, d_work, d_order;
	if (d_in.alloc(n * stride) || d_stage.alloc(n * sstride) || d_lens.alloc(n * 4) || d_fps.alloc(n * 16) || d_work.alloc(64) ||
	    d_order.alloc(encode_order_words((uint32_t)n) * 4)) return -1;
	CMB_CHECK(cudaMemcpy(d_in.p, pages_host, n * stride, cudaMemcpyHostToDevice));
	EncodeJob job{};
	job.pages = d_in.as<uint8_t>(); job.page_stride = stride; job.nbytes = nbytes; job.n = (uint32_t)n;
	job.accel = accel < 0 ? 1u : (uint32_t)(accel > (1 << 20) ? (1 << 20) : accel);
	if (accel == 0) job.accel = 1;
	job.stage = d_stage.as<uint8_t>(); job.stage_stride = sstride;
	job.lens = d_lens.as<int32_t>();
	job.fps = fp_out ? d_fps.as<uint64_t>() : nullptr;
	job.work = d_work.as<unsigned int>();
	job.order = d_order.as<uint32_t>();
	if (launch_encode(job, 0) < 0) return -1;
	CMB_CHECK(cudaMemcpy(lens_out, d_lens.p, n * 4, cudaMemcpyDeviceToHost));
	if (fp_out) CMB_CHECK(cudaMemcpy(fp_out, d_fps.p, n * 16, cudaMemcpyDeviceToHost));
	CMB_CHECK(cudaMemcpy2D(blocks_out_host, out_stride, d_stage.p, sstride, bound < out_stride ? bound : out_stride, n,
	    cudaMemcpyDeviceToHost));
	return 0;
}

extern "C" int cmb200_lz4_decode_batch(int device, const void *blocks_host, size_t in_stride, const int32_t *lens,
    size_t n, uint32_t nbytes, void *pages_out_host, int32_t *consumed_out) {
	if (select_device(device)) return -1;
	DevBuf d_blk, d_lens, d_out, d_used;
	if (d_blk.alloc(n * in_stride) || d_lens.alloc(n * 4) || d_out.alloc(n * (size_t)nbytes) || d_used.alloc(n * 4)) return -1;
	CMB_CHECK(cudaMemcpy(d_blk.p, blocks_host, n * in_stride, cudaMemcpyHostToDevice));
	CMB_CHECK(cudaMemcpy(d_lens.p, lens, n * 4, cudaMemcpyHostToDevice));
	CMB_CHECK(cudaMemset(d_out.p, 0, n * (size_t)nbytes));
	DecodeJob job{};
	job.n = (uint32_t)n; job.nbytes = nbytes; job.pages = d_out.as<uint8_t>(); job.status = d_used.as<int32_t>();
	job.blocks = d_blk.as<uint8_t>(); job.block_stride = in_stride; job.lens = d_lens.as<int32_t>();
	if (launch_decode(job, 0)) return -1;
	CMB_CHECK(cudaMemcpy(consumed_out, d_used.p, n * 4, cudaMemcpyDeviceToHost));
	CMB_CHECK(cudaMemcpy(pages_out_host, d_out.p, n * (size_t)nbytes, cudaMemcpyDeviceToHost));
	return 0;
}

extern "C" int cmb200_fingerprint_batch(int device, const void *pages_host, size_t n, uint32_t nbytes,
    size_t stride, uint64_t *fp_out) {
	if (select_device(device)) return -1;
	if (stride % 16) { set_error_msg("fingerprint_batch: stride must be a multiple of 16"); return -1; }
	DevBuf d_in, d_fps;
	if (d_in.alloc(n * stride) || d_fps.alloc(n * 16)) return -1;
	CMB_CHECK(cudaMemcpy(d_in.p, pages_host, n * stride, cudaMemcpyHostToDevice));
	if (launch_fingerprint(d_in.as<uint8_t>(), stride, nbytes, (uint32_t)n, d_fps.as<uint64_t>(), 0)) return -1;
	CMB_CHECK(cudaMemcpy(fp_out, d_fps.p, n * 16, cudaMemcpyDeviceToHost));
	return 0;
}

extern "C" int cmb200_fingerprint_dev(cmb200_engine *e, size_t n, const void *pages_dev, uint64_t *fp_out_host) {
	std::lock_guard<std::mutex> g(e->mu);
	CMB_CHECK(cudaSetDevice(e->device));
	DevBuf d_fps;
	if (d_fps.alloc(n * 16)) return -1;
	CMB_CHECK(cudaEventRecord(e->t0[0], e->st));
	if (launch_fingerprint((const uint8_t *)pages_dev, e->bsize, e->bsize, (uint32_t)n, d_fps.as<uint64_t>(), e->st)) return -1;
	CMB_CHECK(cudaEventRecord(e->t1[0], e->st));
	CMB_CHECK(cudaMemcpyAsync(fp_out_host, d_fps.p, n * 16, cudaMemcpyDeviceToHost, e->st));
	CMB_CHECK(cudaStreamSynchronize(e->st));
	float ms = 0;
	CMB_CHECK(cudaEventElapsedTime(&ms, e->t0[0], e->t1[0]));
	e->stats.fingerprint_kernel_ns += (uint64_t)(ms * 1e6);
	e->stats.kernel_launches++;
	return 0;
}


extern "C" void cmb200_gen_chunk_host(uint64_t seed, uint64_t cid, uint32_t bsize, void *out) {
	uint64_t *w = (uint64_t *)out;
	for (uint32_t i = 0; i < bsize / 8; i++) w[i] = sg_chunk_word(seed, cid, bsize, i);
}

extern "C" int cmb200_gen_chunks_dev(cmb200_engine *e, uint64_t seed, const uint64_t *cids_host, size_t n, void *out_dev) {
	std::lock_guard<std::mutex> g(e->mu);
	CMB_CHECK(cudaSetDevice(e->device));
	DevBuf d_c;
	if (d_c.alloc(n * 8)) return -1;
	CMB_CHECK(cudaMemcpyAsync(d_c.p, cids_host, n * 8, cudaMemcpyHostToDevice, e->st));
	if (launch_streamgen(d_c.as<uint64_t>(), (uint32_t)n, seed, e->bsize, (uint8_t *)out_dev, e->st)) return -1;
	CMB_CHECK(cudaStreamSynchronize(e->st));
	return 0;
}

extern "C" uint64_t cmb200_gen_stream_ids(uint64_t seed2, size_t n, double dup, uint64_t first_cid, uint64_t *cid_out) {
	uint64_t state = seed2, distinct = 0;
	for (size_t k = 0; k < n; k++) {
		state += SG_GOLDEN;
		uint64_t r = sg_mix(state);
		bool repeat = distinct > 0 && (double)(r >> 11) * (1.0 / 9007199254740992.0) < dup;
		if (repeat) {
			state += SG_GOLDEN;
			cid_out[k] = first_cid + sg_mix(state) % distinct;
		} else {
			cid_out[k] = first_cid + distinct++;
		}
	}
	return distinct;
}

extern "C" void cmb200_gen_addr(uint64_t seed, uint64_t cid, int pshift, uint64_t *offset_out, uint64_t *nhid_out) {
	*offset_out = sg_offset(cid, pshift);
	*nhid_out = sg_nhid(seed, cid);
}
```

edge_fuse_b200/csrc/kernels.cu:

```cuda
#include "kernels.h"
#include "common.cuh"
#include "fingerprint.cuh"
#include "lz4_encode.cuh"
#include "lz4_encode_ring.cuh"
#include <type_traits>
#include "lz4_decode.cuh"
#include "lz4_decode_cta.cuh"
#include "streamgen.cuh"

namespace cmb {


__host__ __device__ __forceinline__ unsigned long long fnv_addr(unsigned long long u, unsigned long long l) {
	unsigned long long h = 14695981039346656037ULL;
#pragma unroll
	for (int i = 0; i < 8; i++) { h = (h ^ ((u >> (8 * i)) & 0xFF)) * 0x100000001b3ULL; }
#pragma unroll
	for (int i = 0; i < 8; i++) { h = (h ^ ((l >> (8 * i)) & 0xFF)) * 0x100000001b3ULL; }
	return h;
}

__device__ __forceinline__ uint64_t home_slot(unsigned long long key, uint64_t cap) {
	unsigned long long z = key;
	z = (z ^ (z >> 32)) * 0xD6E8FEB86659FD93ULL;
	z ^= z >> 32;
	return z & (cap - 1);
}

__device__ __forceinline__ unsigned long long ld_key(const Slot *s) {
	return *reinterpret_cast<const volatile unsigned long long *>(&s->key);
}

__device__ uint32_t table_find_or_claim(const TableView &t, unsigned long long key) {
	if (key == KEY_EMPTY) return (uint32_t)t.cap;
	if (key == KEY_TOMB) return (uint32_t)t.cap + 1;
	for (int attempt = 0; attempt < 64; attempt++) {
		uint64_t i = home_slot(key, t.cap);
		uint64_t tomb = ~0ull;
		bool retry = false;
		for (uint64_t n = 0; n < t.cap; n++, i = (i + 1) & (t.cap - 1)) {
			unsigned long long cur = ld_key(&t.slots[i]);
			if (cur == key) return (uint32_t)i;
			if (cur == KEY_TOMB) { if (tomb == ~0ull) tomb = i; continue; }
			if (cur == KEY_EMPTY) {
				if (tomb != ~0ull) {
					unsigned long long old = atomicCAS(&t.slots[tomb].key, KEY_TOMB, key);
					if (old == KEY_TOMB) { atomicAdd(t.tombs, (unsigned long long)-1ll); return (uint32_t)tomb; }
					if (old == key) return (uint32_t)tomb;
					retry = true;
					break;
				}
				unsigned long long old = atomicCAS(&t.slots[i].key, KEY_EMPTY, key);
				if (old == KEY_EMPTY || old == key) return (uint32_t)i;
			}
		}
		if (retry) continue;
		if (tomb != ~0ull) {
			unsigned long long old = atomicCAS(&t.slots[tomb].key, KEY_TOMB, key);
			if (old == KEY_TOMB) { atomicAdd(t.tombs, (unsigned long long)-1ll); return (uint32_t)tomb; }
			if (old == key) return (uint32_t)tomb;
			continue;
		}
		break;
	}
	return 0xffffffffu;
}

__device__ uint32_t table_find(const TableView &t, unsigned long long key) {
	if (key == KEY_EMPTY) return (uint32_t)t.cap;
	if (key == KEY_TOMB) return (uint32_t)t.cap + 1;
	uint64_t i = home_slot(key, t.cap);
	for (uint64_t n = 0; n < t.cap; n++, i = (i + 1) & (t.cap - 1)) {
		unsigned long long cur = ld_key(&t.slots[i]);
		if (cur == key) return (uint32_t)i;
		if (cur == KEY_EMPTY) break;
	}
	return 0xffffffffu;
}

__global__ void k_compose(const uint64_t *offset, const uint64_t *nhid, const uint32_t *genid, int pshift,
    uint32_t n, unsigned long long *addr, uint8_t *valid, unsigned long long *key) {
	uint32_t i = blockIdx.x * blockDim.x + threadIdx.x;
	if (i >= n) return;
	unsigned long long page = offset[i] >> pshift;
	bool ok = (page >> 44) == 0;
	unsigned long long l = page | ((unsigned long long)genid[i] << 44);
	unsigned long long u = nhid[i];
	addr[2 * i] = u;
	addr[2 * i + 1] = l;
	valid[i] = ok;
	if (key) key[i] = fnv_addr(u, l);
}

__global__ void k_upsert(TableView t, const unsigned long long *addr, const uint8_t *valid, uint32_t n,
    unsigned long long seq0, unsigned long long seq_stride, uint32_t *slot_idx) {
	uint32_t i = blockIdx.x * blockDim.x + threadIdx.x;
	if (i >= n) return;
	uint32_t idx = 0xffffffffu;
	if (!valid || valid[i]) {
		unsigned long long key = fnv_addr(addr[2 * i], addr[2 * i + 1]);
		idx = table_find_or_claim(t, key);
		if (idx != 0xffffffffu) atomicMax(&t.slots[idx].seq, seq0 + seq_stride * i);
	}
	slot_idx[i] = idx;
}

__global__ void k_lookup(TableView t, const unsigned long long *addr, const uint8_t *valid, uint32_t n,
    int32_t *status, uint64_t *rec_off, uint32_t *vlen, unsigned long long *ts_out) {
	uint32_t i = blockIdx.x * blockDim.x + threadIdx.x;
	if (i >= n) return;
	int32_t st = ST_MISS;
	uint64_t off = 0;
	uint32_t vl = 0;
	unsigned long long ts = 0;
	if (valid && !valid[i]) {
		st = ST_INVALID;
	} else {
		unsigned long long u = addr[2 * i], l = addr[2 * i + 1];
		uint32_t idx = table_find(t, fnv_addr(u, l));
		if (idx != 0xffffffffu) {
			const Slot &s = t.slots[idx];
			if (s.vlen != 0) {
				if (s.addr_u == u && s.addr_l == l) {
					st = ST_HIT; off = s.rec_off; vl = s.vlen; ts = s.ts;
				} else {
					st = ST_BAD_ENTRY;
				}
			} else if (s.owner != 0 && s.addr_u == u && s.addr_l == l) {
				st = ST_REMOTE; off = s.owner - 1;
			}
		}
	}
	status[i] = st;
	if (rec_off) rec_off[i] = off;
	if (vlen) vlen[i] = vl;
	if (ts_out) ts_out[i] = ts;
}

__device__ __forceinline__ void slot_release(const ArenaView &a, const Slot &s) {
	if (s.rec_off & REC_HOST) {
		atomicAdd(a.tier, (unsigned long long)s.alloc);
		atomicAdd(a.tier + 1, (unsigned long long)-1ll);
	} else {
		atomicAdd(a.garbage, (unsigned long long)s.alloc);
	}
}

__device__ __forceinline__ void hot_log(const HotLog &h, unsigned long long u, unsigned long long l) {
	const unsigned long long k = atomicAdd(h.head, 1ull);
	h.ring[k % HOT_LOG_N] = make_ulonglong2(u, l);
}

__global__ void k_unset(TableView t, ArenaView a, const unsigned long long *addr, uint32_t n) {
	uint32_t i = blockIdx.x * blockDim.x + threadIdx.x;
	if (i >= n) return;
	uint32_t idx = table_find(t, fnv_addr(addr[2 * i], addr[2 * i + 1]));
	if (idx == 0xffffffffu) return;
	Slot &s = t.slots[idx];
	uint32_t old = atomicExch(&s.vlen, 0u);
	if (old == 0) return;
	atomicAdd(t.entries, (unsigned long long)-1ll);
	slot_release(a, s);
	s.alloc = 0;
	s.owner = 0;
	if (idx < t.cap) {
		s.key = KEY_TOMB;
		atomicAdd(t.tombs, 1ull);
	}
}

constexpr uint32_t SAMPLE_WALK = 128, SAMPLE_REDRAWS = 8;
__device__ __forceinline__ bool slot_live(const Slot &s) { return s.vlen != 0; }
__global__ void k_sample(TableView t, const unsigned long long *r, uint32_t n, unsigned long long *addr_out,
    unsigned long long *ts_out, int32_t *ok) {
	uint32_t i = blockIdx.x * blockDim.x + threadIdx.x;
	if (i >= n) return;
	unsigned long long draw = r[i];
	int32_t found = -1;
	for (uint32_t a = 0; a < SAMPLE_REDRAWS && found < 0; a++) {
		const uint64_t start = home_slot(draw, t.cap);
		for (uint32_t k = 0; k < SAMPLE_WALK; k++) {
			const uint64_t j = (start + k) % (t.cap + 2);
			const Slot &s = t.slots[j];
			if (slot_live(s)) {
				addr_out[2 * i] = s.addr_u; addr_out[2 * i + 1] = s.addr_l; ts_out[i] = s.ts;
				found = 1;
				break;
			}
		}
		draw = draw * 0x9E3779B97F4A7C15ULL + 0xD1B54A32D192ED03ULL;
	}
	ok[i] = found;
}
__global__ void __launch_bounds__(256) k_sample_scan(TableView t, const unsigned long long *r, uint32_t n,
    unsigned long long *addr_out, unsigned long long *ts_out, int32_t *ok) {
	__shared__ unsigned long long first;
	for (uint32_t i = blockIdx.x; i < n; i += gridDim.x) {
		if (ok[i] >= 0) continue;
		const uint64_t total = t.cap + 2, start = home_slot(r[i], t.cap);
		if (threadIdx.x == 0) first = ~0ull;
		__syncthreads();
		for (uint64_t base = 0; base < total; base += blockDim.x) {
			const uint64_t k = base + threadIdx.x;
			if (k < total && slot_live(t.slots[(start + k) % total])) atomicMin(&first, (unsigned long long)k);
			__syncthreads();
			if (first != ~0ull) break;
			__syncthreads();
		}
		if (threadIdx.x == 0) {
			if (first != ~0ull) {
				const Slot &s = t.slots[(start + first) % total];
				addr_out[2 * i] = s.addr_u; addr_out[2 * i + 1] = s.addr_l; ts_out[i] = s.ts;
				ok[i] = 1;
			} else {
				ok[i] = 0;
			}
		}
		__syncthreads();
	}
}


__device__ __forceinline__ void slot_publish(const EncodeJob &job, Slot &s, uint32_t i, uint32_t idx, unsigned long long off,
    uint32_t need, uint32_t clen, unsigned long long au, unsigned long long al, uint64_t fp_hi, uint64_t fp_lo) {
	if (job.table.ckpt) *reinterpret_cast<volatile uint32_t *>(&job.table.ckpt[(size_t)idx * CKPT_WORDS]) = 0u;
	if (s.owner) { atomicAdd(job.table.remote, (unsigned long long)-1ll); s.owner = 0; }
	else if (s.alloc) slot_release(job.arena, s);
	s.addr_u = au; s.addr_l = al;
	s.ts = job.ts ? job.ts[i] : 0;
	if (job.table.fp) { job.table.fp[2 * (size_t)idx] = fp_hi; job.table.fp[2 * (size_t)idx + 1] = fp_lo; }
	s.alloc = need;
	*reinterpret_cast<volatile unsigned long long *>(&s.rec_off) = off;
	__threadfence();
	if (s.vlen == 0) atomicAdd(job.table.entries, 1ull);
	*reinterpret_cast<volatile uint32_t *>(&s.vlen) = clen + 1u;
	if (job.rec_out) job.rec_out[i] = off;
}

__device__ __forceinline__ void ckpt_store(const EncodeJob &job, uint32_t idx, unsigned long long off, uint32_t clen,
    uint32_t ck, int lane) {
	if (!job.table.ckpt) return;
	uint32_t *w = job.table.ckpt + (size_t)idx * CKPT_WORDS;
	__syncwarp();
	if (lane >= 1 && lane < (int)CKPT_WORDS) *reinterpret_cast<volatile uint32_t *>(w + lane) = ck;
	__threadfence();
	__syncwarp();
	if (lane == 0) *reinterpret_cast<volatile uint32_t *>(w) = ckpt_tag(off, clen);
}

__device__ __forceinline__ void ckpt_retag(const TableView &t, uint32_t idx, unsigned long long old_loc,
    unsigned long long new_loc, uint32_t clen) {
	if (!t.ckpt) return;
	uint32_t *w = t.ckpt + (size_t)idx * CKPT_WORDS;
	if (*reinterpret_cast<volatile uint32_t *>(w) == ckpt_tag(old_loc, clen)) {
		__threadfence();
		*reinterpret_cast<volatile uint32_t *>(w) = ckpt_tag(new_loc, clen);
	}
}

__device__ unsigned long long commit_record(const EncodeJob &job, uint32_t i, uint32_t idx, const uint8_t *payload,
    uint32_t plen, int32_t clen, bool payload_ro, uint64_t fp_hi, uint64_t fp_lo, int lane) {
	Slot &s = job.table.slots[idx];
	const uint32_t need = (24u + plen + 15u) & ~15u;
	unsigned long long off = 0;
	int ok = 1;
	if (lane == 0) {
		off = atomicAdd(job.arena.head, (unsigned long long)need);
		if (off + need > job.arena.size) {
			atomicAdd(job.arena.dropped, 1ull);
			ok = 0;
		}
	}
	ok = __shfl_sync(CMB_FULL, ok, 0);
	if (!ok) { if (lane == 0 && job.rec_out) job.rec_out[i] = ~0ull; return ~0ull; }
	off = __shfl_sync(CMB_FULL, off, 0);
	uint8_t *rec = job.arena.base + off;
	const unsigned long long au = job.addr[2 * i], al = job.addr[2 * i + 1];
	if (lane < 6) {
		uint32_t w;
		switch (lane) {
		case 0: w = (uint32_t)au; break;
		case 1: w = (uint32_t)(au >> 32); break;
		case 2: w = (uint32_t)al; break;
		case 3: w = (uint32_t)(al >> 32); break;
		case 4: w = (uint32_t)clen; break;
		default: w = 0; break;
		}
		reinterpret_cast<uint32_t *>(rec)[lane] = w;
	}
	if (payload_ro) warp_copy_ro(rec + 24, payload, plen, lane);
	else warp_copy_rw(rec + 24, payload, plen, lane);
	__threadfence();
	__syncwarp();
	if (lane == 0) slot_publish(job, s, i, idx, off, need, (uint32_t)clen, au, al, fp_hi, fp_lo);
	return off;
}

__device__ uint32_t commit_direct(const EncodeJob &job, uint32_t i, uint32_t idx, unsigned long long base,
    uint32_t clen, uint64_t fp_hi, uint64_t fp_lo, int lane) {
	Slot &s = job.table.slots[idx];
	const uint32_t need = (24u + clen + 15u) & ~15u;
	uint8_t *r = job.arena.base + base;
	const unsigned long long au = job.addr[2 * i], al = job.addr[2 * i + 1];
	if (lane < 6) {
		const uint32_t w = lane == 0 ? (uint32_t)au : lane == 1 ? (uint32_t)(au >> 32) : lane == 2 ? (uint32_t)al
		    : lane == 3 ? (uint32_t)(al >> 32) : lane == 4 ? clen : 0u;
		reinterpret_cast<uint32_t *>(r)[lane] = w;
	}
	__threadfence();
	__syncwarp();
	if (lane == 0) slot_publish(job, s, i, idx, base, need, clen, au, al, fp_hi, fp_lo);
	return need;
}

constexpr uint32_t COST_WARPS = 8, COST_TAB = 2048, COST_POS = 125;
constexpr float COST_LIT = 1.0f / 14.0f;
constexpr float COST_FULL = 160.0f;
#ifdef CMB_ENC_TIMELINE
__device__ unsigned long long *g_enc_timeline;
__device__ __forceinline__ unsigned long long enc_clock() {
	unsigned long long t;
	asm volatile("mov.u64 %0, %%globaltimer;" : "=l"(t));
	return t;
}
#endif
__global__ void __launch_bounds__(COST_WARPS * 32, 4) k_cost(EncodeJob job) {
	__shared__ __align__(16) uint32_t smp[COST_WARPS][256 + 4];
	__shared__ uint16_t tab[COST_WARPS][COST_TAB];
	const int lane = threadIdx.x & 31, warp = threadIdx.x >> 5;
	uint32_t *s = smp[warp];
	uint16_t *h = tab[warp];
	const uint8_t *sb = reinterpret_cast<const uint8_t *>(s);
	const uint32_t o0 = ((uint32_t)lane & 3u) * 32u;
	const uint32_t win_stride = (job.nbytes / 8u) & ~15u;
	for (uint32_t i = blockIdx.x * COST_WARPS + warp; i < job.n; i += gridDim.x * COST_WARPS) {
		const uint4 *src = reinterpret_cast<const uint4 *>(job.pages + (size_t)i * job.page_stride + (lane >> 2) * win_stride + o0);
		const uint4 a = __ldg(src), c = __ldg(src + 1);
		bool live = true;
		if (job.slot_idx) {
			const uint32_t idx = job.slot_idx[i];
			live = idx != 0xffffffffu && job.table.slots[idx].seq == job.seq0 + job.seq_stride * i;
		}
		uint32_t bucket = 0;
		[[maybe_unused]] uint32_t est = 0;
		if (live) {
			const uint32_t w[9] = {a.x, a.y, a.z, a.w, c.x, c.y, c.z, c.w, __shfl_down_sync(CMB_FULL, a.x, 1)};
			__syncwarp();
			reinterpret_cast<uint4 *>(s)[2 * lane] = a;
			reinterpret_cast<uint4 *>(s)[2 * lane + 1] = c;
#pragma unroll
			for (uint32_t k = 0; k < 32; k++) {
				if (o0 + k >= COST_POS) break;
				const uint32_t g = __funnelshift_r(w[k >> 2], w[(k >> 2) + 1], (k & 3u) * 8u);
				h[(g * 2654435761u) >> 21] = (uint16_t)((uint32_t)lane * 32u + k);
			}
			__syncwarp();
			uint32_t starts = 0, lits = 0;
#pragma unroll
			for (uint32_t k = 0; k < 32; k++) {
				if (o0 + k >= COST_POS) break;
				const uint32_t p = (uint32_t)lane * 32u + k;
				const uint32_t g = __funnelshift_r(w[k >> 2], w[(k >> 2) + 1], (k & 3u) * 8u);
				const uint32_t q = h[(g * 2654435761u) >> 21] & 1023u;
				const bool m = q != p && (q & 127u) < COST_POS && __funnelshift_r(s[q >> 2], s[(q >> 2) + 1], (q & 3u) * 8u) == g;
				const bool cont = m && o0 + k > 0u && (q & 127u) > 0u && sb[p - 1] == sb[q - 1];
				starts += m && !cont;
				lits += !m;
			}
#pragma unroll
			for (int d = 16; d > 0; d >>= 1) {
				starts += __shfl_xor_sync(CMB_FULL, starts, d);
				lits += __shfl_xor_sync(CMB_FULL, lits, d);
			}
			const float cost = (float)starts + COST_LIT * (float)lits / (float)job.accel;
			bucket = min(ENC_BUCKETS - 1u, (uint32_t)(cost * ((float)ENC_BUCKETS / COST_FULL)));
			est = starts << 16 | lits;
		}
		if (lane == 0) {
			const uint32_t pos = atomicAdd(&job.work[1 + bucket], 1u);
			job.order[(size_t)bucket * job.n + pos] = i;
#ifdef CMB_ENC_TIMELINE
			if (g_enc_timeline) g_enc_timeline[4 * (size_t)i + 3] = (unsigned long long)bucket << 32 | est;
#endif
		}
	}
}

__device__ __noinline__ uint32_t enc_ticket_chunk(const unsigned int *work, const uint32_t *order, uint32_t n, uint32_t t, int lane) {
	uint32_t cum = lane < (int)ENC_BUCKETS ? work[ENC_BUCKETS - lane] : 0u;
#pragma unroll
	for (int d = 1; d < (int)ENC_BUCKETS; d <<= 1) {
		const uint32_t v = __shfl_up_sync(CMB_FULL, cum, d);
		if (lane >= d) cum += v;
	}
	const int k = __ffs(__ballot_sync(CMB_FULL, lane < (int)ENC_BUCKETS && t < cum)) - 1;
	const uint32_t before = __shfl_sync(CMB_FULL, cum, (k + 31) & 31);
	return order[(size_t)(ENC_BUCKETS - 1 - k) * n + (t - (k ? before : 0u))];
}

constexpr int ENC_PLAIN_WARPS = 7, ENC_PLAIN_CTAS = 2, ENC_RING_WARPS = 13;
template <bool WIDE, int ENC>
__global__ void __launch_bounds__(ENC == 1 ? ENC_RING_WARPS * 32 : ENC_PLAIN_WARPS * 32, ENC == 1 ? 1 : ENC_PLAIN_CTAS) k_encode(EncodeJob job) {
	extern __shared__ __align__(128) uint8_t smem[];
	const int lane = threadIdx.x & 31, warp = threadIdx.x >> 5;
	const uint32_t nwarps = blockDim.x >> 5;
	uint8_t *wsm = smem + (size_t)warp * LZ4_TABLE_BYTES;
	PageRing ring;
	if (ENC == 1)
		ring_setup(ring, smem + (size_t)nwarps * LZ4_TABLE_BYTES + (size_t)warp * RING_ALLOC,
		    smem + (size_t)nwarps * (LZ4_TABLE_BYTES + RING_ALLOC) + (size_t)warp * RING_MBAR_BYTES, lane);
	const uint32_t gw = blockIdx.x * (blockDim.x >> 5) + warp;
	const bool direct = job.slot_idx != nullptr && job.arena.seg_bytes != 0u && job.accel != 0u && gw < ARENA_SEG_SLOTS;
	const uint32_t worst = (uint32_t)((24u + job.stage_stride + 15u) & ~15ull);
	unsigned long long seg_cur = 0, seg_end = 0;
	if (direct && lane == 0) { seg_cur = job.arena.seg[2 * gw]; seg_end = job.arena.seg[2 * gw + 1]; }
#ifdef CMB_ENC_TIMELINE
	uint32_t prev = ~0u;
#endif
	for (;;) {
		uint32_t i = 0;
		if (lane == 0) i = atomicAdd(job.work, 1u);
		i = __shfl_sync(CMB_FULL, i, 0);
		if (i < job.n && job.order) i = enc_ticket_chunk(job.work, job.order, job.n, i, lane);
#ifdef CMB_ENC_TIMELINE
		if (lane == 0 && g_enc_timeline) {
			const unsigned long long t = enc_clock();
			if (prev != ~0u) g_enc_timeline[4 * (size_t)prev + 2] = t;
			if (i < job.n) { g_enc_timeline[4 * (size_t)i] = gw; g_enc_timeline[4 * (size_t)i + 1] = t; }
			prev = i;
		}
#endif
		if (i >= job.n) break;
		const bool store = job.slot_idx != nullptr;
		uint32_t idx = 0;
		if (store) {
			idx = job.slot_idx[i];
			bool live = idx != 0xffffffffu && job.table.slots[idx].seq == job.seq0 + job.seq_stride * i;
			if (!live) { if (lane == 0) job.lens[i] = -1; continue; }
		}
		const uint8_t *src = job.pages + (size_t)i * job.page_stride;
		uint64_t fp_hi = 0, fp_lo = 0;
		if (job.accel == 0) {
			if (job.fps) {
				warp_fingerprint128(src, job.nbytes, lane, fp_hi, fp_lo);
				if (lane == 0) { job.fps[2 * (size_t)i] = fp_hi; job.fps[2 * (size_t)i + 1] = fp_lo; }
			}
			if (lane == 0) job.lens[i] = 0;
			if (store) commit_record(job, i, idx, src, job.nbytes, 0, true, fp_hi, fp_lo, lane);
			continue;
		}
		uint8_t *dst = job.stage + (size_t)(store ? gw : i) * job.stage_stride;
		unsigned long long base = 0;
		int in_arena = 0;
		if (direct) {
			if (lane == 0) {
				if (seg_cur + worst > seg_end) {
					if (seg_end > seg_cur) atomicAdd(job.arena.garbage, seg_end - seg_cur);
					const unsigned long long off = atomicAdd(job.arena.head, (unsigned long long)job.arena.seg_bytes);
					if (off + job.arena.seg_bytes <= job.arena.size) { seg_cur = off; seg_end = off + job.arena.seg_bytes; }
					else { seg_cur = seg_end = 0; }
				}
				in_arena = seg_cur + worst <= seg_end;
				base = seg_cur;
			}
			in_arena = __shfl_sync(CMB_FULL, in_arena, 0);
			base = __shfl_sync(CMB_FULL, base, 0);
			if (in_arena) dst = job.arena.base + base + 24;
		}
		uint32_t clen, ck = 0xffffffffu;
#ifdef CMB_ENC_PHASES
		if (lane == 0) s_enc_phase_row[warp] = g_enc_phases && gw % 4u == 0u ? g_enc_phases + 2u * ENC_PH_N * (size_t)i : nullptr;
		__syncwarp();
#endif
		if (job.fps) {
			clen = lz4_encode_lean<WIDE, true, ENC == 1>(src, job.nbytes, dst, job.accel, wsm, ring, lane, fp_hi, fp_lo, ck);
			if (lane == 0) { job.fps[2 * (size_t)i] = fp_hi; job.fps[2 * (size_t)i + 1] = fp_lo; }
		} else {
			clen = lz4_encode_lean<WIDE, false, ENC == 1>(src, job.nbytes, dst, job.accel, wsm, ring, lane, fp_hi, fp_lo, ck);
		}
		const bool raw = store && clen > job.nbytes + 1024u;
		if (lane == 0) job.lens[i] = raw ? 0 : (int32_t)clen;
		if (raw) {
			__syncwarp();
			commit_record(job, i, idx, src, job.nbytes, 0, true, fp_hi, fp_lo, lane);
		} else if (store) {
			__syncwarp();
			if (in_arena) {
				const uint32_t used = commit_direct(job, i, idx, base, clen, fp_hi, fp_lo, lane);
				if (lane == 0) seg_cur += used;
				ckpt_store(job, idx, base, clen, ck, lane);
			} else {
				const unsigned long long at = commit_record(job, i, idx, dst, clen, (int32_t)clen, false, fp_hi, fp_lo, lane);
				if (at != ~0ull) ckpt_store(job, idx, at, clen, ck, lane);
			}
		}
	}
	if (direct && lane == 0) { job.arena.seg[2 * gw] = seg_cur; job.arena.seg[2 * gw + 1] = seg_end; }
}

static int g_sm_count = 0;
int sm_count() {
	if (!g_sm_count) {
		int dev = 0;
		cudaGetDevice(&dev);
		cudaDeviceGetAttribute(&g_sm_count, cudaDevAttrMultiProcessorCount, dev);
		if (g_sm_count <= 0) g_sm_count = 132;
	}
	return g_sm_count;
}

static int launch_encode_kernel(const EncodeJob &job, bool ring, cudaStream_t st) {
	const bool wide = job.nbytes >= LZ4_NARROW_LIMIT;
	void (*const kern)(EncodeJob) = ring ? (wide ? k_encode<true, 1> : k_encode<false, 1>)
	                                     : (wide ? k_encode<true, 0> : k_encode<false, 0>);
	const int warps = ring ? ENC_RING_WARPS : ENC_PLAIN_WARPS, ctas_per_sm = ring ? 1 : ENC_PLAIN_CTAS;
	const size_t smem = (size_t)warps * (ring ? RING_WARP_SMEM : LZ4_TABLE_BYTES);
	CMB_CHECK(cudaFuncSetAttribute(kern, cudaFuncAttributeMaxDynamicSharedMemorySize, (int)smem));
	uint32_t grid = (uint32_t)(sm_count() * ctas_per_sm);
	uint32_t need = (job.n + warps - 1) / warps;
	if (grid > need) grid = need;
	kern<<<grid, warps * 32, smem, st>>>(job);
	CMB_CHECK(cudaGetLastError());
	return 0;
}

int launch_encode(const EncodeJob &job_in, cudaStream_t st) {
	if (job_in.n == 0) return 0;
	EncodeJob job = job_in;
	const bool ring = job.accel >= 1 && job.accel <= RING_MAX_ACCEL && job.nbytes < (1u << 24);
	const uint32_t resident = (uint32_t)sm_count() * (ring ? ENC_RING_WARPS : ENC_PLAIN_CTAS * ENC_PLAIN_WARPS);
	if (job.n <= resident || job.accel == 0 || job.nbytes < 1024u) job.order = nullptr;
	CMB_CHECK(cudaMemsetAsync(job.work, 0, (job.order ? 1 + ENC_BUCKETS : 1) * sizeof(unsigned int), st));
	if (job.order) {
		k_cost<<<(job.n + COST_WARPS - 1) / COST_WARPS, COST_WARPS * 32, 0, st>>>(job);
		CMB_CHECK(cudaGetLastError());
	}
	if (launch_encode_kernel(job, ring, st) != 0) return -1;
	return job.order ? 2 : 1;
}

#ifdef CMB_ENC_TIMELINE
extern "C" int cmb200_enc_timeline(void *buf) {
	return cudaMemcpyToSymbol(g_enc_timeline, &buf, sizeof(buf)) == cudaSuccess ? 0 : -1;
}
#endif
#ifdef CMB_ENC_PHASES
extern "C" int cmb200_enc_phases(void *buf, uint32_t *nphases) {
	if (nphases) *nphases = ENC_PH_N;
	return cudaMemcpyToSymbol(g_enc_phases, &buf, sizeof(buf)) == cudaSuccess ? 0 : -1;
}
#endif


__global__ void __launch_bounds__(256, 8) k_decode(DecodeJob job) {
	const int lane = threadIdx.x & 31;
	const uint32_t i = blockIdx.x * (blockDim.x >> 5) + (threadIdx.x >> 5);
	if (i >= job.n) return;
	uint8_t *out = job.pages + (size_t)i * job.nbytes;
	if (job.rec_off) {
		if (job.status[i] != ST_HIT) return;
		const unsigned long long off = job.rec_off[i];
		const uint8_t *rec = (off & REC_HOST) ? job.host + (off & ~REC_HOST) : job.arena + off;
		if ((off & REC_HOST) && lane == 0) {
			atomicAdd(job.host_hits, 1ull);
			hot_log(job.hot, job.addr[2 * (size_t)i], job.addr[2 * (size_t)i + 1]);
		}
		uint32_t clen = job.vlen[i] - 1u;
		if (clen == 0) {
			warp_copy_ro(out, rec + 24, job.nbytes, lane);
			return;
		}
		int used = lz4_decode_warp(rec + 24, clen, out, job.nbytes, lane);
		if (used != (int)clen && lane == 0) job.status[i] = ST_BAD_DECODE;
	} else {
		int used = lz4_decode_warp(job.blocks + (size_t)i * job.block_stride, (uint32_t)job.lens[i], out,
		    job.nbytes, lane);
		if (lane == 0) job.status[i] = used;
	}
}

int launch_decode(const DecodeJob &job, cudaStream_t st) {
	if (job.n == 0) return 0;
	const int warps = 8;
	k_decode<<<(job.n + warps - 1) / warps, warps * 32, 0, st>>>(job);
	CMB_CHECK(cudaGetLastError());
	return 0;
}


constexpr uint32_t GS_THREADS = DC_THREADS;
constexpr uint32_t GS_CTRL = 128 + 1152;
static_assert(sizeof(DecodeCta) <= 1152, "decoder state fits its slot");
constexpr uint32_t GS_MAX_PAGE = 65536;
constexpr uint32_t GS_PAIR_MAX_PAGE = 131072;
struct GetShared {
	unsigned long long bar;
	unsigned long long off;
	int32_t st;
	uint32_t clen;
	uint32_t owner;
	uint32_t idx;
	uint32_t region;
	uint32_t sections;
	uint32_t ck[CKPT_WORDS];
};
static_assert(sizeof(GetShared) <= 128, "control block");
__host__ __device__ inline uint32_t gs_recbuf(uint32_t nbytes) { return (24u + nbytes + 1024u + 31u) & ~15u; }
bool get_small_supports(uint32_t nbytes) { return nbytes >= 64u && nbytes <= GS_PAIR_MAX_PAGE && (nbytes & 15u) == 0; }
size_t get_small_smem(uint32_t nbytes) {
	return nbytes > GS_MAX_PAGE ? GS_CTRL + gs_recbuf(nbytes) : GS_CTRL + gs_recbuf(nbytes) + nbytes;
}
uint32_t get_small_region_entries(uint32_t nbytes) { return dc_region(nbytes); }

__device__ __forceinline__ unsigned long long ldv64(const unsigned long long *p) { return *reinterpret_cast<const volatile unsigned long long *>(p); }
__device__ __forceinline__ uint32_t ldv32(const uint32_t *p) { return *reinterpret_cast<const volatile uint32_t *>(p); }

__device__ void gs_lookup(const GetJob &job, unsigned long long u, unsigned long long l, GetShared *sh) {
	int32_t st = ST_MISS;
	uint32_t clen = 0, owner = 0;
	unsigned long long off = 0;
	const uint32_t idx = table_find(job.table, fnv_addr(u, l));
	if (idx != 0xffffffffu) {
		const Slot *s = &job.table.slots[idx];
		const uint32_t vlen = ldv32(&s->vlen);
		const unsigned long long au = ldv64(&s->addr_u), al = ldv64(&s->addr_l);
		if (vlen != 0u) {
			if (au == u && al == l) { st = ST_HIT; __threadfence(); off = ldv64(&s->rec_off); clen = vlen - 1u; }
			else st = ST_BAD_ENTRY;
		} else {
			const unsigned long long ow = ldv64(&s->owner);
			if (ow != 0ull && au == u && al == l) {
				st = ST_REMOTE; owner = (uint32_t)ow;
				__threadfence();
				off = ldv64(&s->rec_off);
				const uint32_t len1 = ldv32(&s->alloc);
				clen = len1 ? len1 - 1u : 0xffffffffu;
			}
		}
	}
	sh->st = st; sh->clen = clen; sh->off = off; sh->owner = owner; sh->idx = idx;
}

__device__ uint32_t gs_region_take(const GetJob &job) {
	uint32_t smid;
	asm volatile("mov.u32 %0, %%smid;" : "=r"(smid));
	const uint32_t words = (job.pool_n + 31u) / 32u;
	for (uint32_t probe = 0; probe < (1u << 22); probe++) {
		const uint32_t w = (smid + probe) % words;
		const uint32_t live = w + 1u == words && (job.pool_n & 31u) ? (1u << (job.pool_n & 31u)) - 1u : 0xffffffffu;
		const uint32_t vacant = ~ldv32(&job.pool_bits[w]) & live;
		if (!vacant) continue;
		const uint32_t b = (uint32_t)__ffs(vacant) - 1u;
		if (!((atomicOr(&job.pool_bits[w], 1u << b) >> b) & 1u)) return w * 32u + b;
	}
	return 0xffffffffu;
}
__device__ void gs_region_give(const GetJob &job, uint32_t r) { atomicAnd(&job.pool_bits[r / 32u], ~(1u << (r & 31u))); }

__device__ void gs_sections(const GetJob &job, GetShared *sh, DecodeCta *dc, uint32_t clen, bool local) {
	const uint32_t n = job.nbytes, S = n / DC_CHAINS;
	bool use = false;
	if (local && job.table.ckpt) {
		const uint32_t *ck = job.table.ckpt + (size_t)sh->idx * CKPT_WORDS;
		const uint32_t want = ckpt_tag(sh->off, clen);
		if (ldv32(ck) == want) {
			__threadfence();
			for (uint32_t k = 1; k < CKPT_WORDS; k++) sh->ck[k] = ldv32(ck + k);
			__threadfence();
			use = ldv32(ck) == want;
		}
	}
	for (uint32_t c = 0; c < DC_CHAINS; c++) { dc->ip0[c] = 0xffffffffu; dc->op0[c] = 0; dc->op_end[c] = 0; dc->cnt[c] = 0; dc->ip1[c] = 0; dc->op1[c] = 0; }
	dc->err = 0;
	dc->ip0[0] = 0; dc->op0[0] = 0;
	uint32_t prev = 0;
	if (use) {
		for (uint32_t k = 1; k < DC_CHAINS; k++) {
			const uint32_t v = sh->ck[k];
			if (v == 0xffffffffu) continue;
			const uint32_t ip = v >> CKPT_POS_BITS, op = k * S + (v & ((1u << CKPT_POS_BITS) - 1u));
			if (ip >= clen || op >= n || op >= (k + 1u) * S || ip <= dc->ip0[prev]) { use = false; break; }
			dc->ip0[k] = ip; dc->op0[k] = op;
			dc->op_end[prev] = op;
			prev = k;
		}
	}
	if (!use) {
		for (uint32_t c = 1; c < DC_CHAINS; c++) dc->ip0[c] = 0xffffffffu;
		prev = 0;
	}
	dc->op_end[prev] = n;
// ... 289 lines not shown
	if (job.n == 0) return 0;
	const size_t smem = get_small_smem(job.nbytes);
	constexpr int MAX_DEV = 64;
	const int dev = device >= 0 && device < MAX_DEV ? device : 0;
	if (job.nbytes > GS_MAX_PAGE) {
		static size_t configured_pair[MAX_DEV] = {};
		if (smem > configured_pair[dev]) {
			CMB_CHECK(cudaFuncSetAttribute(k_get_small_pair, cudaFuncAttributeMaxDynamicSharedMemorySize, (int)smem));
			configured_pair[dev] = smem;
		}
		k_get_small_pair<<<2u * job.n, GS_THREADS, smem, st>>>(job);
		CMB_CHECK(cudaGetLastError());
		return 0;
	}
	static size_t configured[MAX_DEV] = {};
	if (smem > configured[dev]) {
		CMB_CHECK(cudaFuncSetAttribute(k_get_small, cudaFuncAttributeMaxDynamicSharedMemorySize, (int)smem));
		configured[dev] = smem;
	}
	k_get_small<<<job.n, GS_THREADS, smem, st>>>(job);
	CMB_CHECK(cudaGetLastError());
	return 0;
}

int get_small_residency(uint32_t nbytes) {
	const size_t smem = get_small_smem(nbytes);
	if (nbytes > GS_MAX_PAGE) {
		if (cudaFuncSetAttribute(k_get_small_pair, cudaFuncAttributeMaxDynamicSharedMemorySize, (int)smem) != cudaSuccess) return -1;
		cudaLaunchConfig_t cfg = {};
		cfg.gridDim = dim3(2u * (uint32_t)sm_count());
		cfg.blockDim = dim3(GS_THREADS);
		cfg.dynamicSmemBytes = smem;
		int clusters = 0;
		if (cudaOccupancyMaxActiveClusters(&clusters, k_get_small_pair, &cfg) != cudaSuccess) return -1;
		return clusters;
	}
	if (cudaFuncSetAttribute(k_get_small, cudaFuncAttributeMaxDynamicSharedMemorySize, (int)smem) != cudaSuccess) return -1;
	int per_sm = 0;
	if (cudaOccupancyMaxActiveBlocksPerMultiprocessor(&per_sm, k_get_small, (int)GS_THREADS, smem) != cudaSuccess) return -1;
	return per_sm * sm_count();
}


__global__ void __launch_bounds__(256) k_fingerprint(const uint8_t *pages, uint64_t stride, uint32_t nbytes,
    uint32_t n, uint64_t *fps) {
	const int lane = threadIdx.x & 31;
	const uint32_t i = blockIdx.x * (blockDim.x >> 5) + (threadIdx.x >> 5);
	if (i >= n) return;
	uint64_t hi, lo;
	warp_fingerprint128(pages + (size_t)i * stride, nbytes, lane, hi, lo);
	if (lane == 0) { fps[2 * (size_t)i] = hi; fps[2 * (size_t)i + 1] = lo; }
}

int launch_fingerprint(const uint8_t *pages, uint64_t stride, uint32_t nbytes, uint32_t n, uint64_t *fps,
    cudaStream_t st) {
	if (n == 0) return 0;
	const int warps = 8;
	k_fingerprint<<<(n + warps - 1) / warps, warps * 32, 0, st>>>(pages, stride, nbytes, n, fps);
	CMB_CHECK(cudaGetLastError());
	return 0;
}

__global__ void k_streamgen(const uint64_t *cids, uint32_t n, uint64_t seed, uint32_t bsize, uint8_t *out) {
	const uint32_t words = bsize / 8;
	const uint64_t total = (uint64_t)n * words;
	for (uint64_t g = (uint64_t)blockIdx.x * blockDim.x + threadIdx.x; g < total;
	     g += (uint64_t)gridDim.x * blockDim.x) {
		uint32_t c = (uint32_t)(g / words), w = (uint32_t)(g % words);
		reinterpret_cast<uint64_t *>(out)[g] = sg_chunk_word(seed, cids[c], bsize, w);
	}
}

int launch_streamgen(const uint64_t *cids, uint32_t n, uint64_t seed, uint32_t bsize, uint8_t *out,
    cudaStream_t st) {
	if (n == 0) return 0;
	k_streamgen<<<sm_count() * 8, 256, 0, st>>>(cids, n, seed, bsize, out);
	CMB_CHECK(cudaGetLastError());
	return 0;
}

#define GRID1D(n) (((n) + 255u) / 256u), 256

int launch_compose(const uint64_t *offset, const uint64_t *nhid, const uint32_t *genid, int pshift,
    uint32_t n, unsigned long long *addr, uint8_t *valid, unsigned long long *key, cudaStream_t st) {
	if (n == 0) return 0;
	k_compose<<<GRID1D(n), 0, st>>>(offset, nhid, genid, pshift, n, addr, valid, key);
	CMB_CHECK(cudaGetLastError());
	return 0;
}
__global__ void k_pack_records(const unsigned long long *addr, const int32_t *lens, const unsigned long long *rec_off,
    uint32_t n, unsigned long long seq0, unsigned long long stride, uint32_t rank, unsigned long long *out) {
	uint32_t i = blockIdx.x * blockDim.x + threadIdx.x;
	if (i >= n) return;
	ulonglong2 a = *reinterpret_cast<const ulonglong2 *>(addr + 2 * (size_t)i);
	ulonglong2 b;
	b.x = seq0 + stride * i;
	int32_t len = lens[i];
	unsigned long long off = (len >= 0 && rec_off) ? rec_off[i] : 0ull;
	if (off == ~0ull) { len = -1; off = 0; }
	b.y = xrec_tail(rank, off, len);
	reinterpret_cast<ulonglong2 *>(out)[2 * (size_t)i] = a;
	reinterpret_cast<ulonglong2 *>(out)[2 * (size_t)i + 1] = b;
}
int launch_pack_records(const unsigned long long *addr, const int32_t *lens, const unsigned long long *rec_off, uint32_t n,
    unsigned long long seq0, unsigned long long stride, uint32_t rank, unsigned long long *out, cudaStream_t st) {
	if (n == 0) return 0;
	k_pack_records<<<GRID1D(n), 0, st>>>(addr, lens, rec_off, n, seq0, stride, rank, out);
	CMB_CHECK(cudaGetLastError());
	return 0;
}
__global__ void k_import_claim_rec(TableView t, const unsigned long long *rec, uint32_t n, uint32_t my_rank,
    uint32_t *slot_idx) {
	uint32_t i = blockIdx.x * blockDim.x + threadIdx.x;
	if (i >= n) return;
	const unsigned long long tail = rec[4 * (size_t)i + 3];
	uint32_t idx = 0xffffffffu;
	if (xrec_owner(tail) != my_rank && xrec_len1(tail) != 0u) {
		idx = table_find_or_claim(t, fnv_addr(rec[4 * (size_t)i], rec[4 * (size_t)i + 1]));
		if (idx != 0xffffffffu) atomicMax(&t.slots[idx].seq, rec[4 * (size_t)i + 2]);
	}
	slot_idx[i] = idx;
}
__global__ void k_import_apply_rec(TableView t, ArenaView a, const unsigned long long *rec, uint32_t n,
    const uint32_t *slot_idx) {
	uint32_t i = blockIdx.x * blockDim.x + threadIdx.x;
	if (i >= n) return;
	uint32_t idx = slot_idx[i];
	if (idx == 0xffffffffu) return;
	Slot &s = t.slots[idx];
	if (s.seq != rec[4 * (size_t)i + 2]) return;
	if (s.vlen) {
		atomicAdd(t.entries, (unsigned long long)-1ll);
		atomicAdd(a.garbage, (unsigned long long)s.alloc);
		s.vlen = 0; s.alloc = 0;
	}
	if (s.owner == 0) atomicAdd(t.remote, 1ull);
	const unsigned long long tail = rec[4 * (size_t)i + 3];
	s.addr_u = rec[4 * (size_t)i]; s.addr_l = rec[4 * (size_t)i + 1];
	s.rec_off = xrec_off(tail); s.alloc = xrec_len1(tail);
	__threadfence();
	s.owner = (unsigned long long)xrec_owner(tail) + 1;
}
int launch_import_records(TableView t, ArenaView a, const unsigned long long *rec, uint32_t n, uint32_t my_rank,
    uint32_t *slot_idx, cudaStream_t st) {
	if (n == 0) return 0;
	k_import_claim_rec<<<GRID1D(n), 0, st>>>(t, rec, n, my_rank, slot_idx);
	CMB_CHECK(cudaGetLastError());
	k_import_apply_rec<<<GRID1D(n), 0, st>>>(t, a, rec, n, slot_idx);
	CMB_CHECK(cudaGetLastError());
	return 0;
}

int launch_upsert(TableView t, const unsigned long long *addr, const uint8_t *valid, uint32_t n,
    unsigned long long seq0, unsigned long long seq_stride, uint32_t *slot_idx, cudaStream_t st) {
	if (n == 0) return 0;
	k_upsert<<<GRID1D(n), 0, st>>>(t, addr, valid, n, seq0, seq_stride, slot_idx);
	CMB_CHECK(cudaGetLastError());
	return 0;
}
int launch_lookup(TableView t, const unsigned long long *addr, const uint8_t *valid, uint32_t n,
    int32_t *status, uint64_t *rec_off, uint32_t *vlen, unsigned long long *ts_out, cudaStream_t st) {
	if (n == 0) return 0;
	k_lookup<<<GRID1D(n), 0, st>>>(t, addr, valid, n, status, rec_off, vlen, ts_out);
	CMB_CHECK(cudaGetLastError());
	return 0;
}
int launch_unset(TableView t, ArenaView a, const unsigned long long *addr, uint32_t n, cudaStream_t st) {
	if (n == 0) return 0;
	k_unset<<<GRID1D(n), 0, st>>>(t, a, addr, n);
	CMB_CHECK(cudaGetLastError());
	return 0;
}
__global__ void k_read_fp(TableView t, const unsigned long long *addr, uint32_t n, uint64_t *fp_out, int32_t *ok) {
	uint32_t i = blockIdx.x * blockDim.x + threadIdx.x;
	if (i >= n) return;
	unsigned long long u = addr[2 * i], l = addr[2 * i + 1];
	uint32_t idx = table_find(t, fnv_addr(u, l));
	int32_t found = 0;
	if (idx != 0xffffffffu && t.slots[idx].vlen != 0 && t.slots[idx].addr_u == u && t.slots[idx].addr_l == l) {
		fp_out[2 * i] = t.fp[2 * (size_t)idx]; fp_out[2 * i + 1] = t.fp[2 * (size_t)idx + 1];
		found = 1;
	}
	ok[i] = found;
}
int launch_read_fp(TableView t, const unsigned long long *addr, uint32_t n, uint64_t *fp_out, int32_t *ok,
    cudaStream_t st) {
	if (n == 0) return 0;
	k_read_fp<<<GRID1D(n), 0, st>>>(t, addr, n, fp_out, ok);
	CMB_CHECK(cudaGetLastError());
	return 0;
}
__global__ void k_read_ckpt(TableView t, const unsigned long long *addr, uint32_t n, uint32_t *words_out, int32_t *ok) {
	uint32_t i = blockIdx.x * blockDim.x + threadIdx.x;
	if (i >= n) return;
	unsigned long long u = addr[2 * i], l = addr[2 * i + 1];
	uint32_t idx = table_find(t, fnv_addr(u, l));
	int32_t found = -1;
	uint32_t *w = words_out + (size_t)i * CKPT_WORDS;
	for (uint32_t k = 0; k < CKPT_WORDS; k++) w[k] = 0;
	if (idx != 0xffffffffu) {
		const Slot &s = t.slots[idx];
		if (s.vlen != 0 && s.owner == 0 && s.addr_u == u && s.addr_l == l) {
			for (uint32_t k = 0; k < CKPT_WORDS; k++) w[k] = t.ckpt[(size_t)idx * CKPT_WORDS + k];
			found = w[0] == ckpt_tag(s.rec_off, s.vlen - 1u) ? 1 : 0;
		}
	}
	ok[i] = found;
}
int launch_read_ckpt(TableView t, const unsigned long long *addr, uint32_t n, uint32_t *words_out, int32_t *ok,
    cudaStream_t st) {
	if (n == 0) return 0;
	k_read_ckpt<<<GRID1D(n), 0, st>>>(t, addr, n, words_out, ok);
	CMB_CHECK(cudaGetLastError());
	return 0;
}
__global__ void k_export_list(TableView t, uint32_t bsize, ExportEntry *out, unsigned long long *count,
    unsigned long long max_out, bool arena_only) {
	const uint64_t i = (uint64_t)blockIdx.x * blockDim.x + threadIdx.x;
	if (i >= t.cap + 2) return;
	const Slot &s = t.slots[i];
	if (s.vlen == 0 || s.owner != 0) return;
	if (arena_only && (s.rec_off & REC_HOST)) return;
	if (i < t.cap && (s.key == KEY_EMPTY || s.key == KEY_TOMB)) return;
	const unsigned long long j = atomicAdd(count, 1ull);
	if (j >= max_out) return;
	ExportEntry e;
	e.rec_off = s.rec_off; e.ts = s.ts;
	e.fp_hi = t.fp ? t.fp[2 * i] : 0ull; e.fp_lo = t.fp ? t.fp[2 * i + 1] : 0ull;
	e.len = 24u + (s.vlen > 1u ? s.vlen - 1u : bsize);
	e.slot = (uint32_t)i;
	out[j] = e;
}
int launch_export_list(TableView t, uint32_t bsize, ExportEntry *out, unsigned long long *count,
    unsigned long long max_out, bool arena_only, cudaStream_t st) {
	const uint64_t n = t.cap + 2;
	k_export_list<<<(unsigned)((n + 255) / 256), 256, 0, st>>>(t, bsize, out, count, max_out, arena_only);
	CMB_CHECK(cudaGetLastError());
	return 0;
}

constexpr uint32_t RESTORE_WARPS = 8, RESTORE_WIN = 1024;
__device__ bool restore_ckpt_walk(const uint8_t *blk, uint32_t clen, uint32_t n, uint8_t *win, int lane, uint32_t &ck) {
	const uint32_t S = n / CKPT_WORDS;
	uint32_t ip = 0, op = 0, k = 1, wb = 0, we = 0;
	ck = 0xffffffffu;
	auto at = [&](uint32_t p) -> uint32_t {
		if (p >= we) {
			__syncwarp();
			wb = p; we = min(p + RESTORE_WIN, clen);
			for (uint32_t q = wb + (uint32_t)lane; q < we; q += 32u) win[q - wb] = blk[q];
			__syncwarp();
		}
		return win[p - wb];
	};
	for (;;) {
		for (; k < CKPT_WORDS && op >= k * S; k++)
			if ((uint32_t)lane == k) ck = op - k * S < S ? (ip << CKPT_POS_BITS) | (op - k * S) : 0xffffffffu;
		if (ip >= clen) return false;
		const uint32_t tok = at(ip++);
		uint32_t lit = tok >> 4;
		if (lit == 15u) {
			uint32_t b;
			do {
				if (ip >= clen) return false;
				b = at(ip++);
				lit += b;
			} while (b == 255u && lit <= n);
		}
		if (lit > n - op || lit > clen - ip) return false;
		ip += lit; op += lit;
		if (ip == clen) break;
		if (clen - ip < 2u) return false;
		ip += 2;
		uint32_t mlen = tok & 15u;
		if (mlen == 15u) {
			uint32_t b;
			do {
				if (ip >= clen) return false;
				b = at(ip++);
				mlen += b;
			} while (b == 255u && mlen <= n);
		}
		if (mlen + 4u > n - op) return false;
		op += mlen + 4u;
	}
	if (op != n) return false;
	for (; k < CKPT_WORDS; k++) if ((uint32_t)lane == k) ck = 0xffffffffu;
	return true;
}

__global__ void __launch_bounds__(RESTORE_WARPS * 32) k_restore(EncodeJob job, const uint8_t *blob, const unsigned long long *off,
    const uint64_t *fps, uint32_t bsize) {
	__shared__ uint8_t win[RESTORE_WARPS][RESTORE_WIN];
	const int lane = threadIdx.x & 31;
	const uint32_t i = (blockIdx.x * blockDim.x + threadIdx.x) >> 5;
	if (i >= job.n) return;
	const uint32_t idx = job.slot_idx[i];
	if (idx == 0xffffffffu || job.table.slots[idx].seq != job.seq0 + job.seq_stride * i) return;
	const uint8_t *rec = blob + off[i];
	const int32_t clen = *reinterpret_cast<const int32_t *>(rec + 16);
	const uint32_t plen = clen > 0 ? (uint32_t)clen : bsize;
	const unsigned long long at =
	    commit_record(job, i, idx, rec + 24, plen, clen, true, fps ? fps[2 * i] : 0ull, fps ? fps[2 * i + 1] : 0ull, lane);
	if (at == ~0ull || clen <= 0 || !job.table.ckpt) return;
	uint32_t ck;
	if (restore_ckpt_walk(rec + 24, (uint32_t)clen, bsize, win[threadIdx.x >> 5], lane, ck))
		ckpt_store(job, idx, at, (uint32_t)clen, ck, lane);
}
int launch_restore(const EncodeJob &job, const uint8_t *blob, const unsigned long long *off,
// ... 197 lines not shown
```

edge_fuse_b200/csrc/kernels.h:

```cpp
#pragma once
#include <cuda_runtime.h>
#include <stdint.h>

namespace cmb {

struct Slot {
	unsigned long long key;
	unsigned long long addr_u;
	unsigned long long addr_l;
	unsigned long long rec_off;
	uint32_t vlen;
	uint32_t alloc;
	unsigned long long ts;
	unsigned long long seq;
	unsigned long long owner;
};
static_assert(sizeof(Slot) == 64, "slot layout");

constexpr unsigned long long KEY_EMPTY = 0ull;
constexpr unsigned long long KEY_TOMB = ~0ull;

constexpr unsigned long long REC_HOST = 1ull << 63;

constexpr uint32_t HOT_LOG_N = 4096;
struct HotLog {
	unsigned long long *head;
	ulonglong2 *ring;
};

struct TableView {
	Slot *slots;
	uint64_t cap;
	unsigned long long *entries;
	unsigned long long *tombs;
	unsigned long long *remote;
	uint64_t *fp;
	uint32_t *ckpt;
};

constexpr uint32_t CKPT_WORDS = 16;
constexpr uint32_t CKPT_POS_BITS = 13;
__host__ __device__ inline uint32_t ckpt_tag(unsigned long long rec_off, uint32_t clen) {
	return 0x80000000u | ((uint32_t)(rec_off >> 33) & 0x40000000u) |
	    (((uint32_t)(rec_off >> 4) ^ (clen * 0x9E3779B1u)) & 0x3fffffffu);
}

#define ARENA_SEG_SLOTS 4096u

struct ArenaView {
	uint8_t *base;
	uint64_t size;
	unsigned long long *head;
	unsigned long long *garbage;
	unsigned long long *dropped;
	unsigned long long *tier;
	unsigned long long *seg;
	uint32_t seg_bytes;
};

enum LookupStatus : int32_t {
	ST_MISS = 0,
	ST_HIT = 1,
	ST_INVALID = 2,
	ST_BAD_ENTRY = 3,
	ST_BAD_DECODE = 4,
	ST_REMOTE = 5,
};

struct EncodeJob {
	const uint8_t *pages;
	uint64_t page_stride;
	uint32_t nbytes;
	uint32_t n;
	uint32_t accel;
	uint8_t *stage;
	uint64_t stage_stride;
	int32_t *lens;
	unsigned long long *rec_out;
	uint64_t *fps;
	unsigned int *work;
	uint32_t *order;
	const uint32_t *slot_idx;
	const unsigned long long *addr;
	const unsigned long long *ts;
	unsigned long long seq0;
	unsigned long long seq_stride;
	TableView table;
	ArenaView arena;
};

constexpr uint32_t ENC_BUCKETS = 8;
inline size_t encode_order_words(uint32_t n) { return (size_t)ENC_BUCKETS * n; }
int launch_encode(const EncodeJob &job, cudaStream_t st);

struct DecodeJob {
	uint32_t n;
	uint32_t nbytes;
	uint8_t *pages;
	int32_t *status;
	const uint8_t *blocks;
	uint64_t block_stride;
	const int32_t *lens;
	const uint64_t *rec_off;
	const uint32_t *vlen;
	const uint8_t *arena;
	const uint8_t *host;
	unsigned long long *host_hits;
	HotLog hot;
	const unsigned long long *addr;
};
int launch_decode(const DecodeJob &job, cudaStream_t st);

#define GET_MAX_PEERS 16
struct GetJob {
	TableView table;
	const uint8_t *arena;
	uint64_t arena_size;
	const uint8_t *host;
	uint64_t host_size;
	unsigned long long *host_hits;
	const unsigned long long *addr;
	const uint8_t *valid;
	uint32_t n;
	uint32_t nbytes;
	uint8_t *out;
	int32_t *status;
	const uint8_t *peer[GET_MAX_PEERS];
	uint64_t peer_size[GET_MAX_PEERS];
	uint4 *scratch;
	uint32_t region_entries;
	uint32_t *pool_bits;
	uint32_t pool_n;
	HotLog hot;
};
bool get_small_supports(uint32_t nbytes);
size_t get_small_smem(uint32_t nbytes);
uint32_t get_small_region_entries(uint32_t nbytes);
int get_small_residency(uint32_t nbytes);
int launch_get_small(const GetJob &job, int device, cudaStream_t st);

int launch_fingerprint(const uint8_t *pages, uint64_t stride, uint32_t nbytes, uint32_t n,
    uint64_t *fps, cudaStream_t st);

int launch_compose(const uint64_t *offset, const uint64_t *nhid, const uint32_t *genid, int pshift,
    uint32_t n, unsigned long long *addr, uint8_t *valid, unsigned long long *key, cudaStream_t st);

int launch_upsert(TableView t, const unsigned long long *addr, const uint8_t *valid, uint32_t n,
    unsigned long long seq0, unsigned long long seq_stride, uint32_t *slot_idx, cudaStream_t st);

#define XREC_LEN_BITS 22
#define XREC_OFF_BITS 34
__host__ __device__ inline unsigned long long xrec_tail(uint32_t owner, unsigned long long rec_off, int32_t len) {
	return ((unsigned long long)owner << 56) | (((rec_off >> 4) & ((1ull << XREC_OFF_BITS) - 1)) << XREC_LEN_BITS) |
	    (unsigned long long)(len < 0 ? 0u : (uint32_t)len + 1u);
}
__host__ __device__ inline uint32_t xrec_owner(unsigned long long tail) { return (uint32_t)(tail >> 56); }
__host__ __device__ inline unsigned long long xrec_off(unsigned long long tail) {
	return ((tail >> XREC_LEN_BITS) & ((1ull << XREC_OFF_BITS) - 1)) << 4;
}
__host__ __device__ inline uint32_t xrec_len1(unsigned long long tail) { return (uint32_t)(tail & ((1u << XREC_LEN_BITS) - 1)); }
int launch_pack_records(const unsigned long long *addr, const int32_t *lens, const unsigned long long *rec_off, uint32_t n,
    unsigned long long seq0, unsigned long long stride, uint32_t rank, unsigned long long *out, cudaStream_t st);
int launch_import_records(TableView t, ArenaView a, const unsigned long long *rec, uint32_t n, uint32_t my_rank,
    uint32_t *slot_idx, cudaStream_t st);

int launch_lookup(TableView t, const unsigned long long *addr, const uint8_t *valid, uint32_t n,
    int32_t *status, uint64_t *rec_off, uint32_t *vlen, unsigned long long *ts_out, cudaStream_t st);

int launch_unset(TableView t, ArenaView a, const unsigned long long *addr, uint32_t n, cudaStream_t st);

int launch_sample(TableView t, const unsigned long long *r, uint32_t n, unsigned long long *addr_out,
    unsigned long long *ts_out, int32_t *ok, cudaStream_t st);

int launch_read_fp(TableView t, const unsigned long long *addr, uint32_t n, uint64_t *fp_out, int32_t *ok,
    cudaStream_t st);
int launch_read_ckpt(TableView t, const unsigned long long *addr, uint32_t n, uint32_t *words_out, int32_t *ok,
    cudaStream_t st);

int launch_streamgen(const uint64_t *cids, uint32_t n, uint64_t seed, uint32_t bsize, uint8_t *out,
    cudaStream_t st);

struct ExportEntry {
	unsigned long long rec_off;
	unsigned long long ts;
	unsigned long long fp_hi, fp_lo;
	uint32_t len;
	uint32_t slot;
};
static_assert(sizeof(ExportEntry) == 40, "export entry layout");
int launch_export_list(TableView t, uint32_t bsize, ExportEntry *out, unsigned long long *count,
    unsigned long long max_out, bool arena_only, cudaStream_t st);
int launch_restore(const EncodeJob &job, const uint8_t *blob, const unsigned long long *off,
    const uint64_t *fps, uint32_t bsize, cudaStream_t st);

struct MoveEntry { unsigned long long old_off, new_off; uint32_t len, slot; };
static_assert(sizeof(MoveEntry) == 24, "move entry layout");
int launch_compact_window(TableView t, ArenaView a, const MoveEntry *moves, uint32_t n, uint8_t *bounce,
    cudaStream_t st);

struct DemoteEntry { unsigned long long old_off, host_off, bounce_off; uint32_t len, pad; };
static_assert(sizeof(DemoteEntry) == 32, "demote entry layout");
int launch_demote_gather(ArenaView a, const DemoteEntry *d, uint32_t n, uint8_t *bounce, cudaStream_t st);
int launch_demote_publish(TableView t, ArenaView a, const DemoteEntry *d, uint32_t n, cudaStream_t st);
struct PromoteEntry { unsigned long long host_off, new_off; uint32_t len, pad; };
static_assert(sizeof(PromoteEntry) == 24, "promote entry layout");
int launch_promote(TableView t, ArenaView a, const PromoteEntry *p, uint32_t n, const uint8_t *host, cudaStream_t st);
int launch_tier_retire(TableView t, ArenaView a, const unsigned long long *rec, uint32_t n,
    unsigned long long *retired, cudaStream_t st);

int launch_rehash(TableView from, TableView to, cudaStream_t st);

int launch_move_pages(void *dst, const uint32_t *dst_idx, const void *src, const uint32_t *src_idx, uint32_t n,
    uint32_t nbytes, cudaStream_t st);

int sm_count();

}
```

Measured before the change: 138.2.

## Chain device-resident put steps so next encode job starts inside running kernel

Adds a device-pages put_step path that runs upsert and encode prep on a high-priority prep stream and double-buffers per-step metadata (slots, lens, order, liveness). A small arm kernel publishes the next step's EncodeJob descriptor so the running encode kernel can continue into it, with conflict detection against the in-flight sequence range. Liveness is precomputed by a separate k_live kernel instead of table lookups inside encode, and the work memset becomes a tiny zero kernel. The aim is to hide launch gaps and per-step prep latency between consecutive batches, at the cost of extra synchronisation complexity and possible correctness risks if conflicts are misdetected.

```diff
diff --git a/edge_fuse_b200/csrc/engine.cu b/edge_fuse_b200/csrc/engine.cu
--- a/edge_fuse_b200/csrc/engine.cu
+++ b/edge_fuse_b200/csrc/engine.cu
@@ -26,6 +26,20 @@
 static void set_error_msg(const char *msg) { snprintf(g_err, sizeof(g_err), "%s", msg); }
 
 using namespace cmb;
+
+struct CallLock {
+	std::mutex m;
+	uint64_t calls = 0;
+	void lock() { m.lock(); calls++; }
+	void unlock() { m.unlock(); }
+};
+
+struct StepDesc {
+	EncodeJob job;
+	unsigned int work[ENC_WORK_WORDS];
+	unsigned int armed;
+	unsigned int conflict;
+};
 
 struct cmb200_engine {
 	int device = 0;
@@ -86,6 +100,13 @@
 	uint64_t *d_fps = nullptr, *d_recoff = nullptr;
 	unsigned int *d_work = nullptr;
 	uint32_t *d_order = nullptr;
+	uint8_t *d_live = nullptr;
+	StepDesc *d_desc = nullptr;
+	cudaStream_t prep = nullptr;
+	cudaEvent_t prep_done = nullptr, tail = nullptr;
+	uint64_t step_no = 0;
+	uint64_t step_call = 0;
+	unsigned long long step_seq_lo = 0, step_seq_hi = 0;
 	uint32_t *d_import_slot = nullptr;
 	size_t import_slot_cap = 0;
 	uint32_t *d_move_idx = nullptr;
@@ -105,7 +126,7 @@
 	uint64_t ring_pos = 0;
 	uint64_t meta_pos = 0;
 	size_t meta_cap = 0;
-	std::mutex mu;
+	CallLock mu;
 	cmb200_stats stats{};
 	struct HostTier {
 		uint8_t *host = nullptr;
@@ -164,6 +185,7 @@
 	cudaSetDevice(e->device);
 	if (e->st) cudaStreamSynchronize(e->st);
 	if (e->copy) cudaStreamSynchronize(e->copy);
+	if (e->prep) cudaStreamSynchronize(e->prep);
 	cudaFree(e->d_scratch); cudaFree(e->d_pool_bits); cudaFree(e->table.ckpt);
 	cudaFree(e->table.slots); cudaFree(e->table.fp); cudaFree(e->arena.base); cudaFree(e->arena.seg); cudaFree(e->d_counters);
 	cudaFree(e->d_pages[0]); cudaFree(e->d_pages[1]); cudaFree(e->d_stage);
@@ -181,6 +203,9 @@
 	cudaFree(e->tier.d_ctr); cudaFree(e->tier.d_retire); cudaFree(e->tier.d_moves);
 	cudaFree(e->tier.d_promote); cudaFree(e->tier.d_hot);
 	cudaFree(e->d_lens); cudaFree(e->d_status); cudaFree(e->d_fps); cudaFree(e->d_recoff); cudaFree(e->d_work); cudaFree(e->d_order); cudaFree(e->d_import_slot);
+	cudaFree(e->d_live); cudaFree(e->d_desc);
+	if (e->prep_done) cudaEventDestroy(e->prep_done);
+	if (e->tail) cudaEventDestroy(e->tail);
 	for (int i = 0; i < 2; i++) {
 		if (e->landed[i]) cudaEventDestroy(e->landed[i]);
 		if (e->consumed[i]) cudaEventDestroy(e->consumed[i]);
@@ -196,6 +221,7 @@
 	for (int i = 0; i < 2; i++) if (e->meta_free[i]) cudaEventDestroy(e->meta_free[i]);
 	if (e->st) cudaStreamDestroy(e->st);
 	if (e->copy) cudaStreamDestroy(e->copy);
+	if (e->prep) cudaStreamDestroy(e->prep);
 	delete e;
 }
 
@@ -220,6 +246,13 @@
 		e->table.cap = slots;
 		ENG_CHECK(cudaStreamCreateWithFlags(&e->st, cudaStreamNonBlocking));
 		ENG_CHECK(cudaStreamCreateWithFlags(&e->copy, cudaStreamNonBlocking));
+		{
+			int least = 0, greatest = 0;
+			ENG_CHECK(cudaDeviceGetStreamPriorityRange(&least, &greatest));
+			ENG_CHECK(cudaStreamCreateWithPriority(&e->prep, cudaStreamNonBlocking, greatest));
+		}
+		ENG_CHECK(cudaEventCreateWithFlags(&e->prep_done, cudaEventDisableTiming));
+		ENG_CHECK(cudaEventCreateWithFlags(&e->tail, cudaEventDisableTiming));
 		for (auto &ln : e->lane) ENG_CHECK(cudaStreamCreateWithFlags(&ln.st, cudaStreamNonBlocking));
 		for (int i = 0; i < 2; i++) {
 			ENG_CHECK(cudaEventCreateWithFlags(&e->landed[i], cudaEventDisableTiming));
@@ -279,20 +312,23 @@
 		ENG_CHECK(cudaMalloc(&e->d_addr, 2 * M * 16));
 		ENG_CHECK(cudaMalloc(&e->d_ts, 2 * M * 8));
 		ENG_CHECK(cudaMalloc(&e->d_valid, 2 * M));
-		ENG_CHECK(cudaMalloc(&e->d_slot, B * 4));
+		ENG_CHECK(cudaMalloc(&e->d_slot, 2 * B * 4));
 		ENG_CHECK(cudaMalloc(&e->d_vlen, B * 4));
-		ENG_CHECK(cudaMalloc(&e->d_lens, M * 4));
+		ENG_CHECK(cudaMalloc(&e->d_lens, 2 * M * 4));
 		ENG_CHECK(cudaMalloc(&e->d_status, M * 4));
 		ENG_CHECK(cudaMalloc(&e->d_fps, B * 16));
 		ENG_CHECK(cudaMalloc(&e->d_recoff, B * 8));
 		ENG_CHECK(cudaMalloc(&e->d_work, 64));
-		ENG_CHECK(cudaMalloc(&e->d_order, encode_order_words((uint32_t)B) * 4));
+		ENG_CHECK(cudaMalloc(&e->d_order, 2 * encode_order_words((uint32_t)B) * 4));
+		ENG_CHECK(cudaMalloc(&e->d_live, 2 * B));
+		ENG_CHECK(cudaMalloc(&e->d_desc, 2 * sizeof(StepDesc)));
+		ENG_CHECK(cudaMemsetAsync(e->d_desc, 0, 2 * sizeof(StepDesc), e->st));
 		ENG_CHECK(cudaMallocHost(&e->h_meta, cmb200_engine::META_CAP * 33));
 		for (auto &ln : e->lane) {
 			ENG_CHECK(cudaMallocHost(&ln.h_status, cmb200_engine::GET_SMALL_MAX * 4));
 			ENG_CHECK(cudaMallocHost(&ln.h_addr, cmb200_engine::GET_SMALL_MAX * 16));
 		}
-		ENG_CHECK(cudaMalloc(&e->d_recoff_out, M * 8));
+		ENG_CHECK(cudaMalloc(&e->d_recoff_out, 2 * M * 8));
 
 		uint64_t arena = cfg->arena_bytes;
 		if (!arena) {
@@ -398,6 +434,11 @@
 	unsigned long long *d_ts = e->d_ts + (size_t)mb * e->meta_cap;
 	uint8_t *d_valid = e->d_valid + (size_t)mb * e->meta_cap;
 	cudaStream_t ms = copy_meta ? e->copy : e->st;
+	uint32_t *d_slot = e->d_slot + (size_t)mb * e->max_batch;
+	uint8_t *d_live = e->d_live + (size_t)mb * e->max_batch;
+	int32_t *d_lens = e->d_lens + (size_t)mb * e->meta_cap;
+	unsigned long long *d_recoff_out = e->d_recoff_out + (size_t)mb * e->meta_cap;
+	uint32_t *d_order = e->d_order + (size_t)mb * encode_order_words(e->max_batch);
 	if (copy_meta) CMB_CHECK(cudaStreamWaitEvent(e->copy, e->meta_free[mb], 0));
 	CMB_CHECK(cudaMemcpyAsync(d_addr, h_addr, n * 16, cudaMemcpyHostToDevice, ms));
 	if (valid) CMB_CHECK(cudaMemcpyAsync(d_valid, h_valid, n, cudaMemcpyHostToDevice, ms));
@@ -424,17 +465,18 @@
 			CMB_CHECK(cudaStreamWaitEvent(e->st, e->landed[buf], 0));
 			d_in = e->d_pages[buf];
 		}
-		if (launch_upsert(e->table, d_addr + 2 * at, valid ? d_valid + at : nullptr, m, e->seq, e->seq_stride, e->d_slot, e->st)) return -1;
+		if (launch_upsert(e->table, d_addr + 2 * at, valid ? d_valid + at : nullptr, m, e->seq, e->seq_stride, d_slot, e->st)) return -1;
 		EncodeJob job{};
 		job.pages = d_in; job.page_stride = e->bsize; job.nbytes = e->bsize; job.n = m;
 		job.accel = (uint32_t)e->accel;
 		job.stage = e->d_stage; job.stage_stride = e->stage_stride;
-		job.lens = e->d_lens + at;
-		job.rec_out = e->d_recoff_out + at;
+		job.lens = d_lens + at;
+		job.rec_out = d_recoff_out + at;
 		job.fps = (e->flags & CMB200_FINGERPRINT) ? e->d_fps : nullptr;
 		job.work = e->d_work;
-		job.order = e->d_order;
-		job.slot_idx = e->d_slot;
+		job.order = d_order;
+		job.slot_idx = d_slot;
+		job.live = d_live;
 		job.addr = d_addr + 2 * at;
 		job.ts = ts ? d_ts + at : nullptr;
 		job.seq0 = e->seq; job.seq_stride = e->seq_stride;
@@ -457,12 +499,12 @@
 	}
 	e->stats.put_chunks += n;
 	if (recs && recs->out) {
-		if (launch_pack_records(d_addr, e->d_lens, e->d_recoff_out, (uint32_t)n, seq_first, e->seq_stride, recs->rank, recs->out, e->st)) return -1;
+		if (launch_pack_records(d_addr, d_lens, d_recoff_out, (uint32_t)n, seq_first, e->seq_stride, recs->rank, recs->out, e->st)) return -1;
 		e->stats.kernel_launches++;
 	}
 	if (copy_meta) CMB_CHECK(cudaEventRecord(e->meta_free[mb], e->st));
 	if (deferred) {
-		if (lens_out) CMB_CHECK(cudaMemcpyAsync(lens_out, e->d_lens, n * 4, cudaMemcpyDeviceToHost, e->st));
+		if (lens_out) CMB_CHECK(cudaMemcpyAsync(lens_out, d_lens, n * 4, cudaMemcpyDeviceToHost, e->st));
 		CMB_CHECK(cudaEventRecord(e->ticket_ev[e->tickets % cmb200_engine::TICKETS], e->st));
 		*ticket = ++e->tickets;
 		CMB_CHECK(cudaEventSynchronize(e->meta_done));
@@ -470,7 +512,7 @@
 		harvest_pending(e, false);
 		return 0;
 	}
-	if (lens_out) CMB_CHECK(cudaMemcpyAsync(h_lens, e->d_lens, n * 4, cudaMemcpyDeviceToHost, e->st));
+	if (lens_out) CMB_CHECK(cudaMemcpyAsync(h_lens, d_lens, n * 4, cudaMemcpyDeviceToHost, e->st));
 	CMB_CHECK(cudaStreamSynchronize(e->st));
 	if (lens_out) memcpy(lens_out, h_lens, n * 4);
 	for (size_t k = 0; k < nb && k < (size_t)e->RING; k++) {
@@ -482,6 +524,83 @@
 	return 0;
 }
 
+static int put_step_dev(cmb200_engine *e, size_t n, const cmb200_addr *addr, const uint8_t *valid,
+    const uint8_t *pages, const uint64_t *ts, int32_t *lens_out, uint64_t *ticket, const StepRecords &recs) {
+	const bool chain = e->step_no > 0 && e->mu.calls == e->step_call + 1;
+	const unsigned long long seq0 = e->seq;
+	cmb200_addr *h_addr = (cmb200_addr *)e->h_meta;
+	uint64_t *h_ts = (uint64_t *)(e->h_meta + cmb200_engine::META_CAP * 16);
+	uint8_t *h_valid = e->h_meta + cmb200_engine::META_CAP * 32;
+	harvest_pending(e, false);
+	memcpy(h_addr, addr, n * 16);
+	if (ts) memcpy(h_ts, ts, n * 8);
+	if (valid) memcpy(h_valid, valid, n);
+	const int mb = (int)(e->meta_pos++ & 1);
+	const size_t M = e->meta_cap, B = e->max_batch;
+	unsigned long long *d_addr = e->d_addr + (size_t)mb * M * 2;
+	unsigned long long *d_ts = e->d_ts + (size_t)mb * M;
+	uint8_t *d_valid = e->d_valid + (size_t)mb * M;
+	StepDesc *desc = e->d_desc + mb;
+	CMB_CHECK(cudaStreamWaitEvent(e->copy, e->meta_free[mb], 0));
+	CMB_CHECK(cudaMemcpyAsync(d_addr, h_addr, n * 16, cudaMemcpyHostToDevice, e->copy));
+	if (valid) CMB_CHECK(cudaMemcpyAsync(d_valid, h_valid, n, cudaMemcpyHostToDevice, e->copy));
+	if (ts) CMB_CHECK(cudaMemcpyAsync(d_ts, h_ts, n * 8, cudaMemcpyHostToDevice, e->copy));
+	CMB_CHECK(cudaEventRecord(e->meta_done, e->copy));
+	if (!chain) {
+		CMB_CHECK(cudaEventRecord(e->tail, e->st));
+		CMB_CHECK(cudaStreamWaitEvent(e->prep, e->tail, 0));
+	}
+	CMB_CHECK(cudaStreamWaitEvent(e->prep, e->meta_done, 0));
+	if (launch_zero(&desc->conflict, 1, e->prep)) return -1;
+	EncodeJob job{};
+	job.pages = pages; job.page_stride = e->bsize; job.nbytes = e->bsize; job.n = (uint32_t)n;
+	job.accel = (uint32_t)e->accel;
+	job.stage = e->d_stage; job.stage_stride = e->stage_stride;
+	job.lens = e->d_lens + (size_t)mb * M;
+	job.rec_out = e->d_recoff_out + (size_t)mb * M;
+	job.fps = (e->flags & CMB200_FINGERPRINT) ? e->d_fps : nullptr;
+	job.work = desc->work;
+	job.order = e->d_order + (size_t)mb * encode_order_words((uint32_t)B);
+	job.live = e->d_live + (size_t)mb * B;
+	job.addr = d_addr;
+	job.ts = ts ? d_ts : nullptr;
+	job.seq0 = seq0; job.seq_stride = e->seq_stride;
+	job.table = e->table; job.arena = e->arena;
+	job.next = &e->d_desc[mb ^ 1].job; job.armed = &e->d_desc[mb ^ 1].armed; job.stamp = (unsigned int)(e->step_no + 2);
+	uint32_t *d_slot = e->d_slot + (size_t)mb * B;
+	job.slot_idx = d_slot;
+	if (launch_upsert(e->table, d_addr, valid ? d_valid : nullptr, (uint32_t)n, seq0, e->seq_stride, d_slot, e->prep,
+		chain ? e->step_seq_lo : 0, chain ? e->step_seq_hi : 0, &desc->conflict)) return -1;
+	const int prep_kernels = launch_encode_prep(job, e->prep);
+	if (prep_kernels < 0) return -1;
+	if (chain && launch_arm(&desc->job, job, &desc->armed, &desc->conflict, (unsigned int)(e->step_no + 1), e->prep)) return -1;
+	CMB_CHECK(cudaEventRecord(e->prep_done, e->prep));
+	CMB_CHECK(cudaStreamWaitEvent(e->st, e->prep_done, 0));
+	if (e->pend_head - e->pend_tail >= (uint64_t)cmb200_engine::RING) harvest_pending(e, true);
+	cudaEvent_t ev0 = e->p0[e->pend_head % cmb200_engine::RING], ev1 = e->p1[e->pend_head % cmb200_engine::RING];
+	e->pend_head++;
+	CMB_CHECK(cudaEventRecord(ev0, e->st));
+	if (launch_encode_kernel(job, e->st)) return -1;
+	CMB_CHECK(cudaEventRecord(ev1, e->st));
+	e->seq += (unsigned long long)n * e->seq_stride;
+	e->stats.kernel_launches += 2 + prep_kernels + (chain ? 1 : 0);
+	e->stats.put_chunks += n;
+	if (recs.out) {
+		if (launch_pack_records(d_addr, job.lens, job.rec_out, (uint32_t)n, seq0, e->seq_stride, recs.rank, recs.out, e->st)) return -1;
+		e->stats.kernel_launches++;
+	}
+	CMB_CHECK(cudaEventRecord(e->meta_free[mb], e->st));
+	if (lens_out) CMB_CHECK(cudaMemcpyAsync(lens_out, job.lens, n * 4, cudaMemcpyDeviceToHost, e->st));
+	CMB_CHECK(cudaEventRecord(e->ticket_ev[e->tickets % cmb200_engine::TICKETS], e->st));
+	*ticket = ++e->tickets;
+	e->step_no++;
+	e->step_call = e->mu.calls;
+	e->step_seq_lo = seq0; e->step_seq_hi = e->seq;
+	CMB_CHECK(cudaEventSynchronize(e->meta_done));
+	harvest_pending(e, false);
+	return 0;
+}
+
 static int check_dev_pages(const void *pages, const char *what) {
 	if (reinterpret_cast<uintptr_t>(pages) & 15u) {
 		snprintf(g_err, sizeof(g_err), "%s: device pages must be 16-byte aligned", what);
@@ -501,7 +620,7 @@
 
 static int put_impl(cmb200_engine *e, size_t n, const cmb200_addr *addr, const uint8_t *valid,
     const uint8_t *pages, bool pages_on_dev, const uint64_t *ts, int32_t *lens_out, uint64_t *ticket) {
-	std::lock_guard<std::mutex> g(e->mu);
+	std::lock_guard<CallLock> g(e->mu);
 	CMB_CHECK(cudaSetDevice(e->device));
 	if (ticket) *ticket = e->tickets;
 	for (size_t at = 0; at < n; at += cmb200_engine::META_CAP) {
@@ -530,17 +649,19 @@
 	if (multi_gpu_call(e, "cmb200_put_step")) return -1;
 	if (n > cmb200_engine::META_CAP) { set_error_msg("cmb200_put_step: more than 262144 chunks in one step"); return -1; }
 	if (pages_on_dev == 1 && check_dev_pages(pages, "cmb200_put_step")) return -1;
-	std::lock_guard<std::mutex> g(e->mu);
+	std::lock_guard<CallLock> g(e->mu);
 	CMB_CHECK(cudaSetDevice(e->device));
 	uint64_t t = e->tickets;
 	StepRecords r{rank, (unsigned long long *)records_dev_out, pages_on_dev == 2};
-	const int rc = n ? put_slice(e, n, addr, valid, (const uint8_t *)pages, pages_on_dev == 1, ts, lens_out, &t, &r) : 0;
+	const int rc = !n ? 0
+	    : pages_on_dev == 1 && n <= e->max_batch ? put_step_dev(e, n, addr, valid, (const uint8_t *)pages, ts, lens_out, &t, r)
+	    : put_slice(e, n, addr, valid, (const uint8_t *)pages, pages_on_dev == 1, ts, lens_out, &t, &r);
 	if (ticket) *ticket = t;
 	return rc;
 }
 
 extern "C" int cmb200_import_records_dev(cmb200_engine *e, size_t n_total, const void *records_dev, uint32_t my_rank) {
-	std::lock_guard<std::mutex> g(e->mu);
+	std::lock_guard<CallLock> g(e->mu);
 	if (multi_gpu_call(e, "cmb200_import_records_dev")) return -1;
 	CMB_CHECK(cudaSetDevice(e->device));
 	if (n_total == 0) return 0;
@@ -561,7 +682,7 @@
 extern "C" int cmb200_wait(cmb200_engine *e, uint64_t ticket) {
 	cudaEvent_t ev = nullptr;
 	{
-		std::lock_guard<std::mutex> g(e->mu);
+		std::lock_guard<CallLock> g(e->mu);
 		if (ticket == 0 || ticket > e->tickets) return 0;
 		ev = e->ticket_ev[(ticket - 1) % cmb200_engine::TICKETS];
 		if (cudaSetDevice(e->device) != cudaSuccess) return -1;
@@ -630,7 +751,7 @@
 
 static int get_impl(cmb200_engine *e, size_t n, const cmb200_addr *addr, const uint8_t *valid,
     uint8_t *pages_out, bool out_on_dev, int32_t *status_out) {
-	std::lock_guard<std::mutex> g(e->mu);
+	std::lock_guard<CallLock> g(e->mu);
 	CMB_CHECK(cudaSetDevice(e->device));
 	for (size_t at = 0; at < n; at += cmb200_engine::META_CAP) {
 		size_t m = n - at < cmb200_engine::META_CAP ? n - at : cmb200_engine::META_CAP;
@@ -657,7 +778,7 @@
 
 extern "C" int cmb200_locate_batch(cmb200_engine *e, size_t n, const cmb200_addr *addr, int32_t *status_out,
     uint64_t *owner_out) {
-	std::lock_guard<std::mutex> g(e->mu);
+	std::lock_guard<CallLock> g(e->mu);
 	CMB_CHECK(cudaSetDevice(e->device));
 	for (size_t at = 0; at < n; at += e->max_batch) {
 		uint32_t m = (uint32_t)((n - at < e->max_batch) ? n - at : e->max_batch);
@@ -673,7 +794,7 @@
 
 
 extern "C" int cmb200_set_stream_order(cmb200_engine *e, uint64_t next_seq, uint64_t stride) {
-	std::lock_guard<std::mutex> g(e->mu);
+	std::lock_guard<std::mutex> g(e->mu.m);
 	if (multi_gpu_call(e, "cmb200_set_stream_order")) return -1;
 	if (stride == 0) { set_error_msg("stream order: stride must be >= 1"); return -1; }
 	e->seq = next_seq; e->seq_stride = stride;
@@ -781,7 +902,7 @@
 
 extern "C" int cmb200_arena_ipc_handle(cmb200_engine *e, void *handle64, uint64_t *arena_bytes_out) {
 	{
-		std::lock_guard<std::mutex> g(e->mu);
+		std::lock_guard<CallLock> g(e->mu);
 		if (multi_gpu_call(e, "cmb200_arena_ipc_handle")) return -1;
 	}
 	CMB_CHECK(cudaSetDevice(e->device));
@@ -795,7 +916,7 @@
 
 extern "C" int cmb200_open_peer(cmb200_engine *e, uint32_t rank, const void *handle64, uint64_t arena_bytes) {
 	{
-		std::lock_guard<std::mutex> g(e->mu);
+		std::lock_guard<CallLock> g(e->mu);
 		if (multi_gpu_call(e, "cmb200_open_peer")) return -1;
 	}
 	if (rank >= GET_MAX_PEERS) { set_error_msg("cmb200_open_peer: rank out of range"); return -1; }
@@ -813,7 +934,7 @@
 
 
 extern "C" int cmb200_unset_batch(cmb200_engine *e, size_t n, const cmb200_addr *addr) {
-	std::lock_guard<std::mutex> g(e->mu);
+	std::lock_guard<CallLock> g(e->mu);
 	CMB_CHECK(cudaSetDevice(e->device));
 	for (size_t at = 0; at < n; at += e->max_batch) {
 		uint32_t m = (uint32_t)((n - at < e->max_batch) ? n - at : e->max_batch);
@@ -833,14 +954,14 @@
 }
 
 extern "C" uint64_t cmb200_entries(cmb200_engine *e) {
-	std::lock_guard<std::mutex> g(e->mu);
+	std::lock_guard<CallLock> g(e->mu);
 	unsigned long long c[8];
 	if (read_counters(e, c)) return 0;
 	return c[0];
 }
 
 extern "C" int cmb200_get_stats(cmb200_engine *e, cmb200_stats *out) {
-	std::lock_guard<std::mutex> g(e->mu);
+	std::lock_guard<CallLock> g(e->mu);
 	unsigned long long c[8];
 	if (read_counters(e, c)) return -1;
 	harvest_pending(e, true);
@@ -857,7 +978,7 @@
 
 extern "C" int cmb200_sample(cmb200_engine *e, size_t n, const uint64_t *r, cmb200_addr *addr_out,
     uint64_t *ts_out, int32_t *ok_out) {
-	std::lock_guard<std::mutex> g(e->mu);
+	std::lock_guard<CallLock> g(e->mu);
 	CMB_CHECK(cudaSetDevice(e->device));
 	for (size_t at = 0; at < n; at += e->max_batch) {
 		const uint32_t m = (uint32_t)((n - at < e->max_batch) ? n - at : e->max_batch);
@@ -874,7 +995,7 @@
 
 extern "C" int cmb200_read_records(cmb200_engine *e, size_t n, const cmb200_addr *addr, void *out_host,
     size_t stride, int32_t *len_out) {
-	std::lock_guard<std::mutex> g(e->mu);
+	std::lock_guard<CallLock> g(e->mu);
 	CMB_CHECK(cudaSetDevice(e->device));
 	std::vector<int32_t> st(e->max_batch);
 	std::vector<uint64_t> off(e->max_batch);
@@ -899,7 +1020,7 @@
 
 extern "C" int cmb200_read_fingerprints(cmb200_engine *e, size_t n, const cmb200_addr *addr, uint64_t *fp_out,
     int32_t *ok_out) {
-	std::lock_guard<std::mutex> g(e->mu);
+	std::lock_guard<CallLock> g(e->mu);
 	CMB_CHECK(cudaSetDevice(e->device));
 	if (!e->table.fp) { set_error_msg("engine created without CMB200_FINGERPRINT"); return -1; }
 	for (size_t at = 0; at < n; at += e->max_batch) {
@@ -922,7 +1043,7 @@
 
 extern "C" int cmb200_read_checkpoints(cmb200_engine *e, size_t n, const cmb200_addr *addr, uint32_t *words_out,
     int32_t *ok_out) {
-	std::lock_guard<std::mutex> g(e->mu);
+	std::lock_guard<CallLock> g(e->mu);
 	CMB_CHECK(cudaSetDevice(e->device));
 	if (!e->table.ckpt) {
 		memset(words_out, 0, n * CKPT_WORDS * 4);
@@ -1022,7 +1143,7 @@
 	bool ok = fwrite(&h, sizeof(h), 1, f) == 1;
 	int rc = 0;
 	for (int i = 0; i < g && ok && rc == 0; i++) {
-		std::lock_guard<std::mutex> lk(engines[i]->mu);
+		std::lock_guard<CallLock> lk(engines[i]->mu);
 		rc = save_engine(engines[i], f, win, &h.records, &h.bytes);
 	}
 	cudaFreeHost(win);
@@ -1075,7 +1196,7 @@
 static long long load_flush(LoadBatch &b, bool with_fp) {
 	if (b.m == 0) return 0;
 	cmb200_engine *e = b.e;
-	std::lock_guard<std::mutex> g(e->mu);
+	std::lock_guard<CallLock> g(e->mu);
 	CMB_CHECK(cudaSetDevice(e->device));
 	const size_t m = b.m;
 	if (e->tier.host) {
@@ -1171,7 +1292,7 @@
 	if (n == 0) return 0;
 	if (check_dev_pages(dst_dev, "cmb200_move_pages") || check_dev_pages(src_dev, "cmb200_move_pages")) return -1;
 	if (n > 0xffffffffu) { set_error_msg("cmb200_move_pages: too many pages"); return -1; }
-	std::lock_guard<std::mutex> g(e->mu);
+	std::lock_guard<CallLock> g(e->mu);
 	CMB_CHECK(cudaSetDevice(e->device));
 	if ((dst_idx || src_idx) && n > e->move_idx_cap) {
 		CMB_CHECK(cudaStreamSynchronize(e->st));
@@ -1193,7 +1314,7 @@
 
 extern "C" int cmb200_copy_peer(cmb200_engine *dst_e, void *dst_dev, cmb200_engine *src_e, const void *src_dev, size_t bytes) {
 	if (bytes == 0) return 0;
-	std::lock_guard<std::mutex> g(src_e->mu);
+	std::lock_guard<CallLock> g(src_e->mu);
 	CMB_CHECK(cudaSetDevice(src_e->device));
 	CMB_CHECK(cudaMemcpyPeerAsync(dst_dev, dst_e->device, src_dev, src_e->device, bytes, src_e->st));
 	CMB_CHECK(cudaStreamSynchronize(src_e->st));
@@ -1264,13 +1385,13 @@
 }
 
 extern "C" int cmb200_compact(cmb200_engine *e, uint64_t *reclaimed_out) {
-	std::lock_guard<std::mutex> g(e->mu);
+	std::lock_guard<CallLock> g(e->mu);
 	return compact_locked(e, reclaimed_out);
 }
 
 
 extern "C" int cmb200_host_tier_enable(cmb200_engine *e, uint64_t bytes) {
-	std::lock_guard<std::mutex> g(e->mu);
+	std::lock_guard<CallLock> g(e->mu);
 	if (e->tier.host) { set_error_msg("cmb200_host_tier_enable: the engine already has a host tier"); return -1; }
 	if (e->multi_gpu) { set_error_msg("cmb200_host_tier_enable: not available after a multi-GPU call"); return -1; }
 	if (e->seq != 1) { set_error_msg("cmb200_host_tier_enable: must be called before the first put"); return -1; }
@@ -1369,7 +1490,7 @@
 }
 
 extern "C" int cmb200_demote_batch(cmb200_engine *e, size_t n, const cmb200_addr *addr, uint64_t *demoted_out) {
-	std::lock_guard<std::mutex> g(e->mu);
+	std::lock_guard<CallLock> g(e->mu);
 	if (demoted_out) *demoted_out = 0;
 	if (!e->tier.host) { set_error_msg("cmb200_demote_batch: the engine has no host tier"); return -1; }
 	CMB_CHECK(cudaSetDevice(e->device));
@@ -1408,7 +1529,7 @@
 }
 
 extern "C" int cmb200_promote_batch(cmb200_engine *e, size_t n, const cmb200_addr *addr, uint64_t *promoted_out) {
-	std::lock_guard<std::mutex> g(e->mu);
+	std::lock_guard<CallLock> g(e->mu);
 	if (promoted_out) *promoted_out = 0;
 	cmb200_engine::HostTier &t = e->tier;
 	if (!t.host) { set_error_msg("cmb200_promote_batch: the engine has no host tier"); return -1; }
@@ -1451,7 +1572,7 @@
 }
 
 extern "C" int cmb200_host_tier_hot(cmb200_engine *e, size_t max, cmb200_addr *addr_out, size_t *n_out, uint64_t *lost_out) {
-	std::lock_guard<std::mutex> g(e->mu);
+	std::lock_guard<CallLock> g(e->mu);
 	*n_out = 0;
 	if (lost_out) *lost_out = 0;
 	cmb200_engine::HostTier &t = e->tier;
@@ -1479,7 +1600,7 @@
 }
 
 extern "C" int cmb200_host_tier_stats(cmb200_engine *e, struct cmb200_host_tier_stats *out) {
-	std::lock_guard<std::mutex> g(e->mu);
+	std::lock_guard<CallLock> g(e->mu);
 	memset(out, 0, sizeof(*out));
 	const cmb200_engine::HostTier &t = e->tier;
 	if (!t.host) return 0;
@@ -1570,7 +1691,7 @@
 }
 
 extern "C" int cmb200_fingerprint_dev(cmb200_engine *e, size_t n, const void *pages_dev, uint64_t *fp_out_host) {
-	std::lock_guard<std::mutex> g(e->mu);
+	std::lock_guard<CallLock> g(e->mu);
 	CMB_CHECK(cudaSetDevice(e->device));
 	DevBuf d_fps;
 	if (d_fps.alloc(n * 16)) return -1;
@@ -1593,7 +1714,7 @@
 }
 
 extern "C" int cmb200_gen_chunks_dev(cmb200_engine *e, uint64_t seed, const uint64_t *cids_host, size_t n, void *out_dev) {
-	std::lock_guard<std::mutex> g(e->mu);
+	std::lock_guard<CallLock> g(e->mu);
 	CMB_CHECK(cudaSetDevice(e->device));
 	DevBuf d_c;
 	if (d_c.alloc(n * 8)) return -1;
diff --git a/edge_fuse_b200/csrc/kernels.cu b/edge_fuse_b200/csrc/kernels.cu
--- a/edge_fuse_b200/csrc/kernels.cu
+++ b/edge_fuse_b200/csrc/kernels.cu
@@ -93,14 +93,18 @@
 }
 
 __global__ void k_upsert(TableView t, const unsigned long long *addr, const uint8_t *valid, uint32_t n,
-    unsigned long long seq0, unsigned long long seq_stride, uint32_t *slot_idx) {
+    unsigned long long seq0, unsigned long long seq_stride, uint32_t *slot_idx, unsigned long long busy_lo,
+    unsigned long long busy_hi, unsigned int *conflict) {
 	uint32_t i = blockIdx.x * blockDim.x + threadIdx.x;
 	if (i >= n) return;
 	uint32_t idx = 0xffffffffu;
 	if (!valid || valid[i]) {
 		unsigned long long key = fnv_addr(addr[2 * i], addr[2 * i + 1]);
 		idx = table_find_or_claim(t, key);
-		if (idx != 0xffffffffu) atomicMax(&t.slots[idx].seq, seq0 + seq_stride * i);
+		if (idx != 0xffffffffu) {
+			const unsigned long long old = atomicMax(&t.slots[idx].seq, seq0 + seq_stride * i);
+			if (conflict && old >= busy_lo && old < busy_hi) *conflict = 1u;
+		}
 	}
 	slot_idx[i] = idx;
 }
@@ -313,7 +317,7 @@
 	return need;
 }
 
-constexpr uint32_t COST_WARPS = 8, COST_TAB = 2048, COST_POS = 125;
+constexpr uint32_t COST_WARPS = 1, COST_TAB = 1024, COST_POS = 125;
 constexpr float COST_LIT = 1.0f / 14.0f;
 constexpr float COST_FULL = 160.0f;
 #ifdef CMB_ENC_TIMELINE
@@ -324,7 +328,7 @@
 	return t;
 }
 #endif
-__global__ void __launch_bounds__(COST_WARPS * 32, 4) k_cost(EncodeJob job) {
+__global__ void __launch_bounds__(COST_WARPS * 32) k_cost(EncodeJob job) {
 	__shared__ __align__(16) uint32_t smp[COST_WARPS][256 + 4];
 	__shared__ uint16_t tab[COST_WARPS][COST_TAB];
 	const int lane = threadIdx.x & 31, warp = threadIdx.x >> 5;
@@ -352,7 +356,7 @@
 			for (uint32_t k = 0; k < 32; k++) {
 				if (o0 + k >= COST_POS) break;
 				const uint32_t g = __funnelshift_r(w[k >> 2], w[(k >> 2) + 1], (k & 3u) * 8u);
-				h[(g * 2654435761u) >> 21] = (uint16_t)((uint32_t)lane * 32u + k);
+				h[(g * 2654435761u) >> 22] = (uint16_t)((uint32_t)lane * 32u + k);
 			}
 			__syncwarp();
 			uint32_t starts = 0, lits = 0;
@@ -361,7 +365,7 @@
 				if (o0 + k >= COST_POS) break;
 				const uint32_t p = (uint32_t)lane * 32u + k;
 				const uint32_t g = __funnelshift_r(w[k >> 2], w[(k >> 2) + 1], (k & 3u) * 8u);
-				const uint32_t q = h[(g * 2654435761u) >> 21] & 1023u;
+				const uint32_t q = h[(g * 2654435761u) >> 22] & 1023u;
 				const bool m = q != p && (q & 127u) < COST_POS && __funnelshift_r(s[q >> 2], s[(q >> 2) + 1], (q & 3u) * 8u) == g;
 				const bool cont = m && o0 + k > 0u && (q & 127u) > 0u && sb[p - 1] == sb[q - 1];
 				starts += m && !cont;
@@ -377,6 +381,7 @@
 			est = starts << 16 | lits;
 		}
 		if (lane == 0) {
+			if (job.live) job.live[i] = live;
 			const uint32_t pos = atomicAdd(&job.work[1 + bucket], 1u);
 			job.order[(size_t)bucket * job.n + pos] = i;
 #ifdef CMB_ENC_TIMELINE
@@ -384,6 +389,27 @@
 #endif
 		}
 	}
+}
+
+__global__ void k_live(EncodeJob job) {
+	const uint32_t i = blockIdx.x * blockDim.x + threadIdx.x;
+	if (i >= job.n) return;
+	const uint32_t idx = job.slot_idx[i];
+	job.live[i] = idx != 0xffffffffu && job.table.slots[idx].seq == job.seq0 + job.seq_stride * i;
+}
+
+__global__ void k_zero(unsigned int *p, uint32_t n) {
+	if (threadIdx.x < n) p[threadIdx.x] = 0u;
+}
+
+__global__ void k_arm(EncodeJob *dst, EncodeJob job, unsigned int *armed, const unsigned int *conflict, unsigned int stamp) {
+	*dst = job;
+	__threadfence();
+	if (!*conflict) asm volatile("st.release.gpu.global.u32 [%0], %1;" :: "l"(armed), "r"(stamp) : "memory");
+}
+
+__device__ __forceinline__ bool enc_warps_left(const EncodeJob &job) {
+	return 8u * *reinterpret_cast<volatile const unsigned int *>(&job.work[ENC_LEFT]) >= gridDim.x * (blockDim.x >> 5);
 }
 
 __device__ __noinline__ uint32_t enc_ticket_chunk(const unsigned int *work, const uint32_t *order, uint32_t n, uint32_t t, int lane) {
@@ -400,7 +426,7 @@
 
 constexpr int ENC_PLAIN_WARPS = 7, ENC_PLAIN_CTAS = 2, ENC_RING_WARPS = 13;
 template <bool WIDE, int ENC>
-__global__ void __launch_bounds__(ENC == 1 ? ENC_RING_WARPS * 32 : ENC_PLAIN_WARPS * 32, ENC == 1 ? 1 : ENC_PLAIN_CTAS) k_encode(EncodeJob job) {
+__global__ void __launch_bounds__(ENC == 1 ? ENC_RING_WARPS * 32 : ENC_PLAIN_WARPS * 32, ENC == 1 ? 1 : ENC_PLAIN_CTAS) k_encode(const __grid_constant__ EncodeJob job) {
 	extern __shared__ __align__(128) uint8_t smem[];
 	const int lane = threadIdx.x & 31, warp = threadIdx.x >> 5;
 	const uint32_t nwarps = blockDim.x >> 5;
@@ -417,36 +443,53 @@
 #ifdef CMB_ENC_TIMELINE
 	uint32_t prev = ~0u;
 #endif
+	const EncodeJob *jp = &job;
+	bool cont = false;
 	for (;;) {
+		const EncodeJob &J = *jp;
 		uint32_t i = 0;
-		if (lane == 0) i = atomicAdd(job.work, 1u);
+		if (lane == 0) i = cont && enc_warps_left(job) ? ~0u : atomicAdd(J.work, 1u);
 		i = __shfl_sync(CMB_FULL, i, 0);
-		if (i < job.n && job.order) i = enc_ticket_chunk(job.work, job.order, job.n, i, lane);
+		if (i < J.n && J.order) i = enc_ticket_chunk(J.work, J.order, J.n, i, lane);
 #ifdef CMB_ENC_TIMELINE
 		if (lane == 0 && g_enc_timeline) {
 			const unsigned long long t = enc_clock();
 			if (prev != ~0u) g_enc_timeline[4 * (size_t)prev + 2] = t;
-			if (i < job.n) { g_enc_timeline[4 * (size_t)i] = gw; g_enc_timeline[4 * (size_t)i + 1] = t; }
-			prev = i;
+			prev = ~0u;
+			if (i < J.n) {
+				prev = cont ? job.n + i : i;
+				g_enc_timeline[4 * (size_t)prev] = gw; g_enc_timeline[4 * (size_t)prev + 1] = t;
+			}
 		}
 #endif
-		if (i >= job.n) break;
-		const bool store = job.slot_idx != nullptr;
+		if (i >= J.n) {
+			if (cont || !job.next) break;
+			unsigned int a = 0;
+			if (lane == 0) {
+				asm volatile("ld.acquire.gpu.global.u32 %0, [%1];" : "=r"(a) : "l"(job.armed) : "memory");
+				if (enc_warps_left(job)) a = 0u;
+			}
+			if (__shfl_sync(CMB_FULL, a, 0) != job.stamp) break;
+			do asm volatile("ld.acquire.gpu.global.u32 %0, [%1];" : "=r"(a) : "l"(job.armed) : "memory"); while (a != job.stamp);
+			jp = job.next;
+			cont = true;
+			continue;
+		}
+		const bool store = J.slot_idx != nullptr;
 		uint32_t idx = 0;
 		if (store) {
-			idx = job.slot_idx[i];
-			bool live = idx != 0xffffffffu && job.table.slots[idx].seq == job.seq0 + job.seq_stride * i;
-			if (!live) { if (lane == 0) job.lens[i] = -1; continue; }
-		}
-		const uint8_t *src = job.pages + (size_t)i * job.page_stride;
+			idx = J.slot_idx[i];
+			if (!J.live[i]) { if (lane == 0) J.lens[i] = -1; continue; }
+		}
+		const uint8_t *src = J.pages + (size_t)i * J.page_stride;
 		uint64_t fp_hi = 0, fp_lo = 0;
 		if (job.accel == 0) {
-			if (job.fps) {
+			if (J.fps) {
 				warp_fingerprint128(src, job.nbytes, lane, fp_hi, fp_lo);
-				if (lane == 0) { job.fps[2 * (size_t)i] = fp_hi; job.fps[2 * (size_t)i + 1] = fp_lo; }
+				if (lane == 0) { J.fps[2 * (size_t)i] = fp_hi; J.fps[2 * (size_t)i + 1] = fp_lo; }
 			}
-			if (lane == 0) job.lens[i] = 0;
-			if (store) commit_record(job, i, idx, src, job.nbytes, 0, true, fp_hi, fp_lo, lane);
+			if (lane == 0) J.lens[i] = 0;
+			if (store) commit_record(J, i, idx, src, job.nbytes, 0, true, fp_hi, fp_lo, lane);
 			continue;
 		}
 		uint8_t *dst = job.stage + (size_t)(store ? gw : i) * job.stage_stride;
@@ -469,33 +512,34 @@
 		}
 		uint32_t clen, ck = 0xffffffffu;
 #ifdef CMB_ENC_PHASES
-		if (lane == 0) s_enc_phase_row[warp] = g_enc_phases && gw % 4u == 0u ? g_enc_phases + 2u * ENC_PH_N * (size_t)i : nullptr;
+		if (lane == 0) s_enc_phase_row[warp] = g_enc_phases && gw % 4u == 0u && !cont ? g_enc_phases + 2u * ENC_PH_N * (size_t)i : nullptr;
 		__syncwarp();
 #endif
 		if (job.fps) {
 			clen = lz4_encode_lean<WIDE, true, ENC == 1>(src, job.nbytes, dst, job.accel, wsm, ring, lane, fp_hi, fp_lo, ck);
-			if (lane == 0) { job.fps[2 * (size_t)i] = fp_hi; job.fps[2 * (size_t)i + 1] = fp_lo; }
+			if (lane == 0) { J.fps[2 * (size_t)i] = fp_hi; J.fps[2 * (size_t)i + 1] = fp_lo; }
 		} else {
 			clen = lz4_encode_lean<WIDE, false, ENC == 1>(src, job.nbytes, dst, job.accel, wsm, ring, lane, fp_hi, fp_lo, ck);
 		}
 		const bool raw = store && clen > job.nbytes + 1024u;
-		if (lane == 0) job.lens[i] = raw ? 0 : (int32_t)clen;
+		if (lane == 0) J.lens[i] = raw ? 0 : (int32_t)clen;
 		if (raw) {
 			__syncwarp();
-			commit_record(job, i, idx, src, job.nbytes, 0, true, fp_hi, fp_lo, lane);
+			commit_record(J, i, idx, src, job.nbytes, 0, true, fp_hi, fp_lo, lane);
 		} else if (store) {
 			__syncwarp();
 			if (in_arena) {
-				const uint32_t used = commit_direct(job, i, idx, base, clen, fp_hi, fp_lo, lane);
+				const uint32_t used = commit_direct(J, i, idx, base, clen, fp_hi, fp_lo, lane);
 				if (lane == 0) seg_cur += used;
-				ckpt_store(job, idx, base, clen, ck, lane);
+				ckpt_store(J, idx, base, clen, ck, lane);
 			} else {
-				const unsigned long long at = commit_record(job, i, idx, dst, clen, (int32_t)clen, false, fp_hi, fp_lo, lane);
-				if (at != ~0ull) ckpt_store(job, idx, at, clen, ck, lane);
+				const unsigned long long at = commit_record(J, i, idx, dst, clen, (int32_t)clen, false, fp_hi, fp_lo, lane);
+				if (at != ~0ull) ckpt_store(J, idx, at, clen, ck, lane);
 			}
 		}
 	}
 	if (direct && lane == 0) { job.arena.seg[2 * gw] = seg_cur; job.arena.seg[2 * gw + 1] = seg_end; }
+	if (job.next && lane == 0) atomicAdd(&job.work[ENC_LEFT], 1u);
 }
 
 static int g_sm_count = 0;
@@ -509,7 +553,13 @@
 	return g_sm_count;
 }
 
-static int launch_encode_kernel(const EncodeJob &job, bool ring, cudaStream_t st) {
+static bool encode_ring(const EncodeJob &job) {
+	return job.accel >= 1 && job.accel <= RING_MAX_ACCEL && job.nbytes < (1u << 24);
+}
+
+int launch_encode_kernel(const EncodeJob &job, cudaStream_t st) {
+	if (job.n == 0) return 0;
+	const bool ring = encode_ring(job);
 	const bool wide = job.nbytes >= LZ4_NARROW_LIMIT;
 	void (*const kern)(EncodeJob) = ring ? (wide ? k_encode<true, 1> : k_encode<false, 1>)
 	                                     : (wide ? k_encode<true, 0> : k_encode<false, 0>);
@@ -524,19 +574,54 @@
 	return 0;
 }
 
-int launch_encode(const EncodeJob &job_in, cudaStream_t st) {
-	if (job_in.n == 0) return 0;
-	EncodeJob job = job_in;
-	const bool ring = job.accel >= 1 && job.accel <= RING_MAX_ACCEL && job.nbytes < (1u << 24);
-	const uint32_t resident = (uint32_t)sm_count() * (ring ? ENC_RING_WARPS : ENC_PLAIN_CTAS * ENC_PLAIN_WARPS);
+static int prep_carveout() {
+	static bool done = false;
+	if (done) return 0;
+	const void *k[] = {(const void *)k_cost, (const void *)k_live, (const void *)k_zero, (const void *)k_arm, (const void *)k_upsert};
+	for (const void *f : k) CMB_CHECK(cudaFuncSetAttribute(f, cudaFuncAttributePreferredSharedMemoryCarveout, cudaSharedmemCarveoutMaxShared));
+	done = true;
+	return 0;
+}
+
+int launch_zero(unsigned int *p, uint32_t n, cudaStream_t st) {
+	if (prep_carveout()) return -1;
+	k_zero<<<1, 32, 0, st>>>(p, n);
+	CMB_CHECK(cudaGetLastError());
+	return 0;
+}
+
+int launch_encode_prep(EncodeJob &job, cudaStream_t st) {
+	if (job.n == 0) return 0;
+	if (prep_carveout()) return -1;
+	if (job.slot_idx && !job.live) return -1;
+	const uint32_t resident = (uint32_t)sm_count() * (encode_ring(job) ? ENC_RING_WARPS : ENC_PLAIN_CTAS * ENC_PLAIN_WARPS);
 	if (job.n <= resident || job.accel == 0 || job.nbytes < 1024u) job.order = nullptr;
-	CMB_CHECK(cudaMemsetAsync(job.work, 0, (job.order ? 1 + ENC_BUCKETS : 1) * sizeof(unsigned int), st));
+	if (launch_zero(job.work, ENC_WORK_WORDS, st)) return -1;
 	if (job.order) {
 		k_cost<<<(job.n + COST_WARPS - 1) / COST_WARPS, COST_WARPS * 32, 0, st>>>(job);
 		CMB_CHECK(cudaGetLastError());
-	}
-	if (launch_encode_kernel(job, ring, st) != 0) return -1;
-	return job.order ? 2 : 1;
+		return 1;
+	}
+	if (job.slot_idx) {
+		k_live<<<(job.n + 31u) / 32u, 32, 0, st>>>(job);
+		CMB_CHECK(cudaGetLastError());
+		return 1;
+	}
+	return 0;
+}
+
+int launch_encode(const EncodeJob &job_in, cudaStream_t st) {
+	EncodeJob job = job_in;
+	const int prep = launch_encode_prep(job, st);
+	if (prep < 0 || launch_encode_kernel(job, st) != 0) return -1;
+	return job.n ? 1 + prep : 0;
+}
+
+int launch_arm(EncodeJob *dst, const EncodeJob &job, unsigned int *armed, const unsigned int *conflict,
+    unsigned int stamp, cudaStream_t st) {
+	k_arm<<<1, 1, 0, st>>>(dst, job, armed, conflict, stamp);
+	CMB_CHECK(cudaGetLastError());
+	return 0;
 }
 
 #ifdef CMB_ENC_TIMELINE
@@ -1132,9 +1217,11 @@
 }
 
 int launch_upsert(TableView t, const unsigned long long *addr, const uint8_t *valid, uint32_t n,
-    unsigned long long seq0, unsigned long long seq_stride, uint32_t *slot_idx, cudaStream_t st) {
-	if (n == 0) return 0;
-	k_upsert<<<GRID1D(n), 0, st>>>(t, addr, valid, n, seq0, seq_stride, slot_idx);
+    unsigned long long seq0, unsigned long long seq_stride, uint32_t *slot_idx, cudaStream_t st,
+    unsigned long long busy_lo, unsigned long long busy_hi, unsigned int *conflict) {
+	if (n == 0) return 0;
+	if (conflict) k_upsert<<<(n + 31u) / 32u, 32, 0, st>>>(t, addr, valid, n, seq0, seq_stride, slot_idx, busy_lo, busy_hi, conflict);
+	else k_upsert<<<GRID1D(n), 0, st>>>(t, addr, valid, n, seq0, seq_stride, slot_idx, busy_lo, busy_hi, conflict);
 	CMB_CHECK(cudaGetLastError());
 	return 0;
 }
diff --git a/edge_fuse_b200/csrc/kernels.h b/edge_fuse_b200/csrc/kernels.h
--- a/edge_fuse_b200/csrc/kernels.h
+++ b/edge_fuse_b200/csrc/kernels.h
@@ -85,13 +85,23 @@
 	const unsigned long long *ts;
 	unsigned long long seq0;
 	unsigned long long seq_stride;
+	uint8_t *live;
+	const EncodeJob *next;
+	const unsigned int *armed;
+	unsigned int stamp;
 	TableView table;
 	ArenaView arena;
 };
 
 constexpr uint32_t ENC_BUCKETS = 8;
 inline size_t encode_order_words(uint32_t n) { return (size_t)ENC_BUCKETS * n; }
+constexpr uint32_t ENC_LEFT = 1 + ENC_BUCKETS, ENC_WORK_WORDS = ENC_LEFT + 1;
 int launch_encode(const EncodeJob &job, cudaStream_t st);
+int launch_encode_prep(EncodeJob &job, cudaStream_t st);
+int launch_encode_kernel(const EncodeJob &job, cudaStream_t st);
+int launch_zero(unsigned int *p, uint32_t n, cudaStream_t st);
+int launch_arm(EncodeJob *dst, const EncodeJob &job, unsigned int *armed, const unsigned int *conflict,
+    unsigned int stamp, cudaStream_t st);
 
 struct DecodeJob {
 	uint32_t n;
@@ -146,7 +156,8 @@
     uint32_t n, unsigned long long *addr, uint8_t *valid, unsigned long long *key, cudaStream_t st);
 
 int launch_upsert(TableView t, const unsigned long long *addr, const uint8_t *valid, uint32_t n,
-    unsigned long long seq0, unsigned long long seq_stride, uint32_t *slot_idx, cudaStream_t st);
+    unsigned long long seq0, unsigned long long seq_stride, uint32_t *slot_idx, cudaStream_t st,
+    unsigned long long busy_lo = 0, unsigned long long busy_hi = 0, unsigned int *conflict = nullptr);
 
 #define XREC_LEN_BITS 22
 #define XREC_OFF_BITS 34
```

Result: no change. 139.4, median of 6 (+0.9%).
